# Chanuk-Yang/Deep_Continuous_Fusion_for_Multi-Sensor_3D_Object_Detection

Hardware: AMD Instinct MI355X
Metric: frames/sec (train step) 100k-pt LiDAR + 1242x375 RGB (higher is better)
Workload: dtype bf16; 1 GPU; cfg2: grid 32x704x800, 100000 pts/frame, 1242x375 RGB, ResNet-18 image stream, K=3 fusion x4 sites, eval-mode BN (reference F4), batch 2/GPU; global_batch=2, parallelism=dp1, loss_sampling=compat, conv_chain=False

## Files before the change

### deep_continuous_fusion_for_multi-sensor_3d_object_detection_amd/_hip.py

```python
import ctypes
import os
import subprocess

import numpy as np
import torch

_HERE = os.path.dirname(os.path.abspath(__file__))
LIB_PATH = os.environ.get("DCF_HIP_LIB") or os.path.join(_HERE, "libdcf_hip.so")
CSRC = os.path.join(_HERE, "csrc")

F32, BF16, F16 = 0, 1, 2
VOXEL_COMPAT, VOXEL_ACCUM, VOXEL_COMPAT_ROUNDS, VOXEL_OCCUPANCY = 0, 1, 2, 3
PROJ_COMPAT, PROJ_CORRECT = 0, 1

c_int, c_float, c_i64, c_size_t, c_void_p = ctypes.c_int, ctypes.c_float, ctypes.c_int64, ctypes.c_size_t, ctypes.c_void_p
P = c_void_p

SIGNATURES = {
    "dcf_last_error": (ctypes.c_char_p, []),
    "dcf_version": (c_int, []),
    "dcf_set_option": (c_int, [ctypes.c_char_p, ctypes.c_char_p]),
    "dcf_prof_enable": (c_int, [c_int]),
    "dcf_prof_reset": (c_int, []),
    "dcf_prof_calibrate": (c_int, [P, c_int]),
    "dcf_prof_read": (c_int, [P, P, P, P, c_int]),
    "dcf_prof_read2": (c_int, [P, P, P, P, P, c_int]),
    "dcf_compact_workspace_bytes": (c_size_t, [c_int]),
    "dcf_range_filter": (c_int, [P, c_int, P, P, P, P, P, P]),
    "dcf_voxelize_workspace_bytes": (c_size_t, [c_int, c_int, c_int]),
    "dcf_voxelize": (c_int, [P, c_int, P, P, c_int, c_int, c_int, c_int, P, P, P]),
    "dcf_voxelize_batch": (c_int, [P, P, c_int, P, P, c_int, c_int, c_int, P, P, P]),
    "dcf_voxelize_batch_nhwc": (c_int, [c_int, P, P, c_int, P, P, c_int, c_int, c_int, P, P, P]),
    "dcf_project_filter": (c_int, [P, c_int, P, P, c_float, c_float, c_int, P, P, P, P, P, P]),
    "dcf_project_filter_batch": (c_int, [P, P, c_int, P, P, c_float, c_float, c_int, P, P, c_int, P, P, P]),
    "dcf_knn_workspace_bytes": (c_size_t, [c_int, c_int, c_int]),
    "dcf_knn_bev": (c_int, [P, P, c_int, c_int, c_int, c_int, c_int, c_float, c_float, c_float, c_float, c_float, P, P, P]),
    "dcf_knn_bev_batch": (c_int, [P, P, c_int, c_int, c_int, c_int, c_int, c_int, c_float, c_float, c_float, c_float, c_float, P, P, c_size_t, P]),
    "dcf_knn_bev_sites": (c_int, [P, P, c_int, c_int, c_int, P, c_int, c_float, c_float, c_float, c_float, c_float, P]),
    "dcf_knn_bev_batch_shared": (c_int, [P, P, c_int, c_int, c_int, c_int, c_int, c_int, c_int, c_int, c_int, c_float, c_float, c_float, c_float, c_float, P, P, c_size_t, P, c_size_t, P]),
    "dcf_nchw_to_nhwc": (c_int, [c_int, P, P, c_int, c_int, c_int, c_int, P]),
    "dcf_nhwc_to_nchw": (c_int, [c_int, P, P, c_int, c_int, c_int, c_int, P]),
    "dcf_image_to_nhwc4": (c_int, [c_int, P, P, c_int, c_int, c_int, P]),
    "dcf_conv2d_fwd": (c_int, [c_int, P, P, P, P, P] + [c_int] * 12 + [P]),
    "dcf_conv2d_fwd_rowscale": (c_int, [c_int, P, P, P, P, P, P] + [c_int] * 12 + [P]),
    "dcf_conv2d_dgrad": (c_int, [c_int, P, P, P, P, P] + [c_int] * 11 + [P]),
    "dcf_conv2d_dgrad_halfres": (c_int, [c_int, P, P, P, P, P, P] + [c_int] * 11 + [P]),
    "dcf_conv3x3_chain_supported": (c_int, [c_int] * 6),
    "dcf_conv3x3_chain_workspace_bytes": (c_size_t, [c_int] * 6),
    "dcf_conv3x3_chain": (c_int, [c_int, P, c_int, c_int, c_int, c_int, c_int, c_int, P, P]),
    "dcf_fp8_act_scale": (c_int, [c_float, P]),
    "dcf_cast_fp8": (c_int, [c_int, P, P, P, P, c_i64, P]),
    "dcf_weight_prep_fp8": (c_int, [P, P, c_int, c_int, P, P, P, P, P, c_float, P]),
    "dcf_conv2d_fwd_fp8": (c_int, [c_int, P, P, P, P, P, P, P, P, P, P] + [c_int] * 12 + [P]),
    "dcf_conv2d_wgrad_splits": (c_int, [c_int] * 8),
    "dcf_conv2d_wgrad": (c_int, [c_int, P, P, P, P, c_int] + [c_int] * 11 + [P]),
    "dcf_conv2d_wgrad_groupable": (c_int, [c_int] * 10),
    "dcf_conv2d_wgrad_group": (c_int, [P, c_int, P]),
    "dcf_stem7x7_fwd": (c_int, [c_int, P, P, P, P] + [c_int] * 7 + [P]),
    "dcf_stem7x7_wgrad": (c_int, [c_int, P, P, P, P, c_int] + [c_int] * 6 + [P]),
    "dcf_weight_prep": (c_int, [c_int, P, c_int, P, P, P, P, c_float, P]),
    "dcf_wgrad_finalize": (c_int, [P, c_int, c_int, P, P, P, P, P, P, c_float, P]),
    "dcf_eval_score_filter": (c_int, [P, c_int, c_int, c_int, c_float, c_int, P, P, P]),
    "dcf_eval_nms_workspace_bytes": (c_size_t, [c_int]),
    "dcf_eval_nms": (c_int, [P, P, c_int, c_int, ctypes.c_double, P, P, P, P]),
    "dcf_eval_match": (c_int, [P, c_int, P, c_int, P, c_int, P, P]),
    "dcf_eval_rank_workspace_bytes": (c_size_t, [c_int, c_int, c_int]),
    "dcf_eval_rank_filter": (c_int, [P, c_int, c_int, c_int, c_float, c_int, P, P, P, P, P, P]),
    "dcf_eval_match_ranked_workspace_bytes": (c_size_t, [c_int, c_int]),
    "dcf_eval_match_ranked": (c_int, [P, P, P, c_int, P, c_int, P, c_int, P, P, P]),
    "dcf_eval_accumulate": (c_int, [P, P, P, P, P, c_int, P, c_int, P, P, c_i64, P, P]),
    "dcf_eval_ap_workspace_bytes": (c_size_t, [c_i64]),
    "dcf_eval_ap": (c_int, [P, P, P, c_i64, c_int, P, P, P, P]),
    "dcf_wgrad_finalize_rows": (c_int, [P, c_int, P, P, P, P, P, P, P, c_float, P]),
    "dcf_bn_workspace_bytes": (c_size_t, [c_int]),
    "dcf_bn_train_fwd": (c_int, [c_int, P, P, P, P, P, P, P, P, P, c_i64, c_int, c_float, c_float, c_int, P, P]),
    "dcf_bn_train_bwd": (c_int, [c_int, P, P, P, P, P, P, P, P, c_i64, c_int, P, P]),
    "dcf_relu_bwd_chansum": (c_int, [c_int, P, P, P, c_i64, c_int, c_int, P]),
    "dcf_resize_bilinear_fwd": (c_int, [c_int, P, P, P] + [c_int] * 7 + [P]),
    "dcf_resize_bilinear_bwd": (c_int, [c_int, P, P] + [c_int] * 7 + [P]),
    "dcf_maxpool3x3s2_fwd": (c_int, [c_int, P, P] + [c_int] * 6 + [P]),
    "dcf_maxpool3x3s2_bwd": (c_int, [c_int, P, P, P, P] + [c_int] * 6 + [P]),
    "dcf_maxpool3x3s2_fwd_idx": (c_int, [c_int, P, P, P] + [c_int] * 6 + [P]),
    "dcf_maxpool3x3s2_bwd_idx": (c_int, [c_int, P, P, P] + [c_int] * 6 + [P]),
    "dcf_head_fwd": (c_int, [c_int, P, c_int, P, P, c_int, c_int, c_int, P]),
    "dcf_head_bwd": (c_int, [c_int, P, c_int, P, P, P, P, c_int, c_int, c_int, P]),
    "dcf_point_sample_fwd": (c_int, [c_int, P, c_int, c_int, c_int, P, P, c_int, P, P]),
    "dcf_point_sample_bwd": (c_int, [c_int, P, c_int, c_int, c_int, P, P, c_int, P, P]),
    "dcf_point_sample_fwd_batch": (c_int, [c_int, P, c_int, c_int, c_int, P, c_i64, P, c_int, P, c_int, P]),
    "dcf_point_sample_bwd_batch": (c_int, [c_int, P, c_int, c_int, c_int, P, c_i64, P, c_int, P, c_int, P]),
    "dcf_fusion_gather_fwd_batch": (c_int, [c_int, P, c_i64, P, c_i64, P, c_int, c_int, c_int, c_int, c_float, c_float, c_float, c_float, P, P, c_int, P, P, c_int, P]),
    "dcf_fusion_gather_bwd_inv_batch": (c_int, [c_int, P, c_i64, P, c_i64, P, P, c_i64, P, P, c_int, c_int, c_int, c_int, c_float, c_float, c_float, c_float, P, P, c_int, P, P, P, P, P, c_int, P]),
    "dcf_fusion_gather_fwd": (c_int, [c_int, P, P, P, c_int, c_int, c_int, c_int, c_float, c_float, c_float, c_float, P, P, c_int, P, P, P]),
    "dcf_fusion_gather_bwd": (c_int, [c_int, P, P, P, c_int, c_int, c_int, c_int, c_float, c_float, c_float, c_float, P, P, c_int, P, P, P, P, P]),
    "dcf_fusion_invert_workspace_bytes": (c_size_t, [c_int, c_int]),
    "dcf_fusion_invert": (c_int, [P, c_int, c_int, c_int, P, P, P, P, P]),
    "dcf_fusion_gather_bwd_pts": (c_int, [c_int, P, P, P, c_int, P, P, c_int, c_int, c_int, c_int, c_float, c_float, c_float, c_float, P, P, c_int, P, P, P, P, P]),
    "dcf_fusion_gather_bwd_workspace_bytes": (c_size_t, [c_int]),
    "dcf_fusion_gather_bwd_direct_workspace_bytes": (c_size_t, [c_int, c_int, c_int]),
    "dcf_fusion_gather_bwd_direct_batch": (c_int, [c_int, P, c_i64, P, c_i64, P, P, c_i64, P, P, c_int, c_int, c_int, c_int, c_float, c_float, c_float, c_float, P, P, c_int, P, P, P, P, P, P, c_int, P]),
    "dcf_fusion_gather_bwd_inv": (c_int, [c_int, P, P, P, P, P, P, c_int, c_int, c_int, c_int, c_float, c_float, c_float, c_float, P, P, c_int, P, P, P, P, P, P]),
    "dcf_rowscale_bias_fwd": (c_int, [c_int, P, P, P, c_i64, c_int, P]),
    "dcf_rowscale_bias_bwd": (c_int, [c_int, P, P, P, c_i64, c_int, P]),
    "dcf_relu_mask_rowscale_bwd": (c_int, [c_int, P, P, P, P, P, c_i64, c_int, P]),
    "dcf_cast": (c_int, [c_int, P, c_int, P, c_i64, P]),
    "dcf_loss_fwd_bwd": (c_int, [P, c_i64, P, c_i64, P, P, P, c_int, c_int, c_float, c_int, P, P, c_i64, P, c_i64, P]),
    "dcf_loss_sample_rand": (ctypes.c_uint32, [ctypes.c_uint64, c_int, c_int, c_int, c_int]),
    "dcf_loss_sample_fwd_bwd": (c_int, [P, c_i64, P, c_i64, P, P, P, c_int, c_int, c_int, c_int, c_int, c_float, c_float, c_float, c_float, c_float,
                                        c_int, c_int, c_int, c_int, ctypes.c_uint64, c_float, c_int, P, P, c_i64, P, c_i64, P, P, P, P]),
    "dcf_inv_sort_segments": (c_int, [P, c_int, P, P, P]),
    "dcf_cam_invert_workspace_bytes": (c_size_t, [c_int, c_int, c_int]),
    "dcf_cam_invert": (c_int, [P, c_i64, P, c_int, c_int, c_int, c_int, P, P, P, P, P]),
    "dcf_point_sample_bwd_det": (c_int, [c_int, P, c_i64, c_int, c_int, c_int, P, c_i64, P, P, P, c_int, P]),
    "dcf_fusion_gather_bwd_det_workspace_bytes": (c_size_t, [c_int, c_int, c_int]),
    "dcf_fusion_gather_bwd_det": (c_int, [c_int, P, c_i64, P, c_i64, P, c_int, P, P, c_int, c_int, c_int, c_int, c_float, c_float, c_float, c_float,
                                          P, P, c_int, P, P, P, P, P, c_int, P]),
    "dcf_rowscale_bias_bwd_det_workspace_bytes": (c_size_t, [c_int]),
    "dcf_rowscale_bias_bwd_det": (c_int, [c_int, P, P, P, P, P, c_i64, c_int, P, P]),
    "dcf_rows_fold": (c_int, [P, c_int, c_int, P, P]),
    "dcf_loss_fwd_bwd_det": (c_int, [P, c_i64, P, c_i64, P, P, P, c_int, c_int, c_float, c_int, P, P, c_i64, P, c_i64, P, P]),
    "dcf_loss_sample_fwd_bwd_det": (c_int, [P, c_i64, P, c_i64, P, P, P, c_int, c_int, c_int, c_int, c_int, c_float, c_float, c_float, c_float, c_float,
                                            c_int, c_int, c_int, c_int, ctypes.c_uint64, c_float, c_int, P, P, c_i64, P, c_i64, P, P, P, P, P]),
    "dcf_loss_hard_workspace_bytes": (c_size_t, [c_int, c_int, c_int]),
    "dcf_loss_hard_fwd_bwd": (c_int, [P, c_i64, P, c_i64, P, P, P, c_int, c_int, c_int, c_int, c_int, c_float, c_float, c_float, c_float, c_float,
                                      c_int, c_int, c_int, c_int, ctypes.c_uint64, c_float, c_int, P, P, c_i64, P, c_i64, P, P, P, P, P]),
    "dcf_loss_hard_fwd_bwd_det": (c_int, [P, c_i64, P, c_i64, P, P, P, c_int, c_int, c_int, c_int, c_int, c_float, c_float, c_float, c_float, c_float,
                                          c_int, c_int, c_int, c_int, ctypes.c_uint64, c_float, c_int, P, P, c_i64, P, c_i64, P, P, P, P, P, P]),
    "dcf_adam_step": (c_int, [P, P, P, P, c_i64, c_float, c_float, c_float, c_float, c_int, c_float, P]),
    "dcf_grad_stats": (c_int, [P, c_i64, P, P]),
    "dcf_amp_update": (c_int, [P, c_float, c_int, ctypes.c_double, ctypes.c_double, c_int, c_float, c_float, c_float, c_float, P]),
    "dcf_adam_step_guarded": (c_int, [P, P, P, P, c_i64, c_float, c_float, c_float, P, P]),
}


class ConvParam(ctypes.Structure):
    _fields_ = [("w_off", c_i64), ("gamma_off", c_i64), ("beta_off", c_i64), ("mean_off", c_i64), ("var_off", c_i64),
                ("wfwd_off", c_i64), ("wdgrad_off", c_i64), ("shift_off", c_i64), ("slab_off", c_i64), ("gsum_off", c_i64),
                ("cout", ctypes.c_int32), ("cin", ctypes.c_int32), ("taps", ctypes.c_int32), ("cout_pad", ctypes.c_int32),
                ("nsplit", ctypes.c_int32), ("flags", ctypes.c_int32), ("pad0", ctypes.c_int32), ("pad1", ctypes.c_int32)]


F8_AMAX_STRIDE = 80


class F8Param(ctypes.Structure):
    _fields_ = [("w8_off", c_i64), ("wscale_off", c_i64)]


class WgradItem(ctypes.Structure):
    _fields_ = [("dtype", ctypes.c_int32), ("nsplit", ctypes.c_int32), ("x", c_void_p), ("gy", c_void_p), ("slabs", c_void_p),
                ("gsum", c_void_p), ("B", ctypes.c_int32), ("H", ctypes.c_int32), ("W", ctypes.c_int32), ("Cin", ctypes.c_int32),
                ("Cout", ctypes.c_int32), ("kh", ctypes.c_int32), ("kw", ctypes.c_int32), ("stride", ctypes.c_int32), ("pad", ctypes.c_int32),
                ("pad_", ctypes.c_int32)]


CHAIN_MAX_LAYERS = 24


class ChainLayer(ctypes.Structure):
    _fields_ = [("x", c_void_p), ("w", c_void_p), ("shift", c_void_p), ("res", c_void_p), ("mask", c_void_p), ("y", c_void_p),
                ("relu", ctypes.c_int32), ("pad_", ctypes.c_int32)]


class KnnMap(ctypes.Structure):
    _fields_ = [("idx", c_void_p), ("h", ctypes.c_int32), ("w", ctypes.c_int32)]


class KnnSite(ctypes.Structure):
    _fields_ = [("h", ctypes.c_int32), ("w", ctypes.c_int32), ("stride", ctypes.c_int32), ("fine", ctypes.c_int32), ("idx_out", c_void_p),
                ("ws", c_void_p), ("ws_stride_bytes", ctypes.c_size_t)]


AMP_PARTS = 1024


class AmpState(ctypes.Structure):
    _fields_ = [("scale_in", c_float), ("scale_next", c_float), ("growth_tracker", ctypes.c_int32), ("found_inf", ctypes.c_int32),
                ("applied_steps", c_i64), ("skipped_steps", c_i64), ("grad_norm", c_float), ("clip_coef", c_float),
                ("gscale", c_float), ("lr_over_bc1", c_float), ("inv_sqrt_bc2", c_float), ("pad_", ctypes.c_int32 * 3),
                ("part_sum", c_float * AMP_PARTS), ("part_flag", ctypes.c_int32 * AMP_PARTS)]


class DcfError(RuntimeError):
    pass


_LIB = None


def build(force=False):
    if force:
        subprocess.check_call(["make", "-s", "-C", CSRC, "clean"])
    subprocess.check_call(["make", "-s", "-j8", "-C", CSRC])
    return LIB_PATH


def lib():
    global _LIB
    if _LIB is None:
        if not os.path.exists(LIB_PATH):
            raise DcfError("libdcf_hip.so is not built (%s). Run __graft_entry__.build() / make -C %s; "
                           "there is no CPU fallback for the HIP hot path." % (LIB_PATH, CSRC))
        L = ctypes.CDLL(LIB_PATH)
        for name, (res, args) in SIGNATURES.items():
            fn = getattr(L, name)
            fn.restype = res
            fn.argtypes = args
        _LIB = L
    return _LIB


_Tensor = torch.Tensor
_Param = torch.nn.Parameter


def _ptr(t):
    tt = type(t)
    if tt is int or tt is float or t is None:
        return t
    if tt is _Tensor or tt is _Param:
        return t.data_ptr()
    if isinstance(t, torch.Tensor):
        return t.data_ptr()
    if isinstance(t, np.ndarray):
        return t.ctypes.data
    return t


_raw_stream = getattr(torch._C, "_cuda_getCurrentRawStream", None)
_get_device = torch._C._cuda_getDevice if hasattr(torch._C, "_cuda_getDevice") else None


def stream_ptr():
    if _raw_stream is not None:
        return _raw_stream(_get_device())
    return torch.cuda.current_stream().cuda_stream


_FN = {}
_NO_RAISE = ("dcf_version", "dcf_conv2d_wgrad_splits", "dcf_prof_read", "dcf_conv2d_wgrad_groupable", "dcf_conv3x3_chain_supported")


def call(name, *args):
    ent = _FN.get(name)
    if ent is None:
        fn = getattr(lib(), name)
        ent = _FN[name] = (fn, fn.restype is c_int and name not in _NO_RAISE)
    rc = ent[0](*[_ptr(a) for a in args])
    if rc != 0 and ent[1]:
# ... 50 lines not shown
```

### deep_continuous_fusion_for_multi-sensor_3d_object_detection_amd/csrc/geometry.hip

```cpp
#include <stdlib.h>
#include "dcf_common.h"

namespace {

struct Lim6 { float v[6]; };
struct Aff6 { float v[6]; };
struct Crt12 { float v[12]; };

__device__ __forceinline__ bool in_range(float x, float y, float z, const Lim6 &l)
{
    return x > l.v[0] && x < l.v[1] && y > l.v[2] && y < l.v[3] && z > l.v[4] && z < l.v[5];
}

constexpr int CP_THREADS = 256;
constexpr int CP_ITEMS = 4;
constexpr int CP_TILE = CP_THREADS * CP_ITEMS;

__device__ __forceinline__ int block_excl_scan(int v, int *total)
{
    __shared__ int wsum[4];
    const int lane = threadIdx.x & 63, wid = threadIdx.x >> 6;
    int inc = v;
#pragma unroll
    for (int o = 1; o < 64; o <<= 1) {
// ... 308 lines not shown
        for (int c = 0; c < 8; ++c) contrib[k][c] = 0.f;
    const int cell = (zl * L + xl) * W + yl;
#pragma unroll
    for (int oz = -1; oz <= 1; ++oz)
#pragma unroll
        for (int ox = -1; ox <= 1; ++ox)
#pragma unroll
            for (int oy = -1; oy <= 1; ++oy) {
                const int nc = cell + (oz * L + ox) * W + oy;
                if (nc < 0 || nc >= nvox) continue;
                const int j1 = last[nc];
                if (j1 <= 0) continue;
                const float *q = pts + 3 * (size_t)(j1 - 1);
                const float fx = __fadd_rn(__fmul_rn(q[0], aff.v[0]), aff.v[1]);
                const float fy = __fadd_rn(__fmul_rn(q[1], aff.v[2]), aff.v[3]);
                const float fz = __fadd_rn(__fmul_rn(q[2], aff.v[4]), aff.v[5]);
                const float dx = __fsub_rn(fx, (float)(int)fx), dy = __fsub_rn(fy, (float)(int)fy), dz = __fsub_rn(fz, (float)(int)fz);
                const float wxs[2] = {__fsub_rn(1.0f, dx), dx}, wys[2] = {__fsub_rn(1.0f, dy), dy}, wzs[2] = {__fsub_rn(1.0f, dz), dz};
#pragma unroll
                for (int k = 0; k < 8; ++k) {
                    const int ez = (k & 1) - oz, ex = ((k >> 1) & 1) - ox, ey = ((k >> 2) & 1) - oy;
                    if (ez < 0 || ez > 1 || ex < 0 || ex > 1 || ey < 0 || ey > 1) continue;
                    contrib[k][ez | (ex << 1) | (ey << 2)] = __fmul_rn(__fmul_rn(wxs[ex], wys[ey]), wzs[ez]);
                }
            }
#pragma unroll
    for (int k = 0; k < 8; ++k) {
        float sum = 0.f;
#pragma unroll
        for (int c = 0; c < 8; ++c) sum = __fadd_rn(sum, contrib[k][c]);
        const int v = cell + ((k & 1) * L + ((k >> 1) & 1)) * W + ((k >> 2) & 1);
        if (v >= nvox) continue;
        if (NHWC) {
            const int vz = v / (L * W), r = v - vz * (L * W);
            DT<TO>::st(grid + (size_t)r * Cz + vz, sum);
        } else {
            DT<TO>::st(grid + v, sum);
        }
    }
}

__global__ void __launch_bounds__(256) k_voxel_accum(const float *pts, int n, Lim6 lim, Aff6 aff, int L, int W, float *grid)
{
    const int i = blockIdx.x * blockDim.x + threadIdx.x;
    if (i >= n) return;
    const float x = pts[3 * i], y = pts[3 * i + 1], z = pts[3 * i + 2];
    if (!in_range(x, y, z, lim)) return;
    Corner8 c8;
    corners(x, y, z, aff, L, W, c8);
#pragma unroll
    for (int c = 0; c < 8; ++c) atomicAdd(&grid[c8.vox[c]], c8.w[c]);
}

__global__ void __launch_bounds__(256) k_voxel_occupancy(const float *pts, int n, Lim6 lim, Aff6 aff, int L, int W, float *grid)
{
    const int i = blockIdx.x * blockDim.x + threadIdx.x;
    if (i >= n) return;
    const float x = pts[3 * i], y = pts[3 * i + 1], z = pts[3 * i + 2];
    if (!in_range(x, y, z, lim)) return;
    Corner8 c8;
    corners(x, y, z, aff, L, W, c8);
    grid[c8.vox[0]] = 1.0f;
}

struct KnnGrid {
    int h, w, h8, w8, stride;
    float xs, xo, ys, yo;
    int fs_xyz, fs_cnt, fs_ws, fs_out;
};

__device__ __forceinline__ int cell_key(int ci, int cj, const KnnGrid &g)
{
    return (((ci >> 3) * g.w8 + (cj >> 3)) << 6) + ((ci & 7) << 3) + (cj & 7);
}

__device__ __forceinline__ void point_cell(float x, float y, const KnnGrid &g, int &ci, int &cj)
{
    const float fx = __fadd_rn(__fmul_rn(x, g.xs), g.xo), fy = __fadd_rn(__fmul_rn(y, g.ys), g.yo);
    ci = (int)floorf(fx / (float)g.stride);
    cj = (int)floorf(fy / (float)g.stride);
    ci = min(max(ci, 0), g.h - 1);
    cj = min(max(cj, 0), g.w - 1);
}

__global__ void __launch_bounds__(256) k_knn_hist(const float *xyz, const int *count, int n_max, KnnGrid g, int *cellcnt,
                                                  int *pkey)
{
    const int i = blockIdx.x * blockDim.x + threadIdx.x;
    xyz += (size_t)blockIdx.y * g.fs_xyz; count += blockIdx.y * g.fs_cnt; cellcnt += (size_t)blockIdx.y * g.fs_ws; pkey += (size_t)blockIdx.y * g.fs_ws;
    const int n = min(*count, n_max);
    if (i >= n) return;
    int ci, cj;
    point_cell(xyz[3 * i], xyz[3 * i + 1], g, ci, cj);
    const int key = cell_key(ci, cj, g);
    pkey[i] = key;
    atomicAdd(&cellcnt[key], 1);
}

__global__ void __launch_bounds__(CP_THREADS) k_scan_blocksum(const int *in, int n, int *blocksum, int fstride = 0)
{
    in += (size_t)blockIdx.y * fstride; blocksum += (size_t)blockIdx.y * fstride;
    const int base = blockIdx.x * CP_TILE + threadIdx.x * CP_ITEMS;
    int c = 0;
#pragma unroll
    for (int k = 0; k < CP_ITEMS; ++k)
        if (base + k < n) c += in[base + k];
    int tot;
    block_excl_scan(c, &tot);
    if (threadIdx.x == 0) blocksum[blockIdx.x] = tot;
}

__global__ void __launch_bounds__(CP_THREADS) k_scan_apply(const int *in, int n, const int *blockoff, int *out, int *cursor, int fstride = 0)
{
    in += (size_t)blockIdx.y * fstride; blockoff += (size_t)blockIdx.y * fstride; out += (size_t)blockIdx.y * fstride; cursor += (size_t)blockIdx.y * fstride;
    const int base = blockIdx.x * CP_TILE + threadIdx.x * CP_ITEMS;
    int v[CP_ITEMS];
    int c = 0;
#pragma unroll
    for (int k = 0; k < CP_ITEMS; ++k) {
        v[k] = (base + k < n) ? in[base + k] : 0;
        c += v[k];
    }
    int tot;
    int pos = blockoff[blockIdx.x] + block_excl_scan(c, &tot);
#pragma unroll
    for (int k = 0; k < CP_ITEMS; ++k) {
        if (base + k < n) {
            out[base + k] = pos;
            cursor[base + k] = pos;
            pos += v[k];
        }
    }
}

__global__ void __launch_bounds__(256) k_knn_fill(const float *xyz, const int *count, int n_max, const int *pkey, int *cursor,
                                                  float4 *sorted, int fs_xyz = 0, int fs_cnt = 0, int fs_ws = 0)
{
    xyz += (size_t)blockIdx.y * fs_xyz; count += blockIdx.y * fs_cnt; pkey += (size_t)blockIdx.y * fs_ws; cursor += (size_t)blockIdx.y * fs_ws;
    sorted = reinterpret_cast<float4 *>(reinterpret_cast<int *>(sorted) + (size_t)blockIdx.y * fs_ws);
    const int i = blockIdx.x * blockDim.x + threadIdx.x;
    const int n = min(*count, n_max);
    if (i >= n) return;
    const int pos = atomicAdd(&cursor[pkey[i]], 1);
    sorted[pos] = make_float4(xyz[3 * i], xyz[3 * i + 1], __int_as_float(i), 0.f);
}

#define DCF_MAX_KNN_SITES 4
struct KnnSortSites {
    KnnGrid g[DCF_MAX_KNN_SITES];
    int *ws[DCF_MAX_KNN_SITES];
    int nscan[DCF_MAX_KNN_SITES], nsb[DCF_MAX_KNN_SITES];
    int pkey_off[DCF_MAX_KNN_SITES], sorted_off[DCF_MAX_KNN_SITES];
    int n, B;
};

__global__ void __launch_bounds__(256) k_knn_zero_ms(KnnSortSites S)
{
    const int site = blockIdx.y / S.B, frame = blockIdx.y - site * S.B;
    int *p = S.ws[site] + (size_t)frame * S.g[site].fs_ws;
    const int n = S.nscan[site], n4 = n >> 2;
    int4 *row = reinterpret_cast<int4 *>(p);
    for (int i = blockIdx.x * blockDim.x + threadIdx.x; i < n4; i += gridDim.x * blockDim.x) row[i] = make_int4(0, 0, 0, 0);
    if (blockIdx.x == 0 && threadIdx.x < (n & 3)) p[(n4 << 2) + threadIdx.x] = 0;
}

__global__ void __launch_bounds__(256) k_knn_hist_ms(const float *xyz, const int *count, int n_max, KnnSortSites S)
{
    const int site = blockIdx.y / S.B, frame = blockIdx.y - site * S.B;
    const KnnGrid &g = S.g[site];
    const int i = blockIdx.x * blockDim.x + threadIdx.x;
    xyz += (size_t)frame * g.fs_xyz; count += frame * g.fs_cnt;
    int *cellcnt = S.ws[site] + (size_t)frame * g.fs_ws, *pkey = cellcnt + S.pkey_off[site];
    const int n = min(*count, n_max);
    if (i >= n) return;
    int ci, cj;
    point_cell(xyz[3 * i], xyz[3 * i + 1], g, ci, cj);
    const int key = cell_key(ci, cj, g);
    pkey[i] = key;
    atomicAdd(&cellcnt[key], 1);
}

__global__ void __launch_bounds__(CP_THREADS) k_scan_blocksum_ms(KnnSortSites S)
{
    const int site = blockIdx.y / S.B, frame = blockIdx.y - site * S.B;
    if ((int)blockIdx.x >= S.nsb[site]) return;
    const int n = S.nscan[site];
    const int *in = S.ws[site] + (size_t)frame * S.g[site].fs_ws;
    int *blocksum = const_cast<int *>(in) + 3 * n;
    const int base = blockIdx.x * CP_TILE + threadIdx.x * CP_ITEMS;
    int c = 0;
#pragma unroll
    for (int k = 0; k < CP_ITEMS; ++k)
        if (base + k < n) c += in[base + k];
    int tot;
    block_excl_scan(c, &tot);
    if (threadIdx.x == 0) blocksum[blockIdx.x] = tot;
}

__global__ void __launch_bounds__(CP_THREADS) k_compact_scan_ms(KnnSortSites S)
{
    const int site = blockIdx.y / S.B, frame = blockIdx.y - site * S.B;
    const int nb = S.nsb[site];
    int *blocksum = S.ws[site] + (size_t)frame * S.g[site].fs_ws + 3 * S.nscan[site];
    int carry = 0;
    for (int b0 = 0; b0 < nb; b0 += CP_THREADS) {
        int i = b0 + threadIdx.x;
        int v = i < nb ? blocksum[i] : 0;
        int tot;
        int ex = block_excl_scan(v, &tot);
        if (i < nb) blocksum[i] = carry + ex;
        carry += tot;
    }
    if (threadIdx.x == 0) blocksum[nb] = carry;
}

__global__ void __launch_bounds__(CP_THREADS) k_scan_apply_ms(KnnSortSites S)
{
    const int site = blockIdx.y / S.B, frame = blockIdx.y - site * S.B;
    if ((int)blockIdx.x >= S.nsb[site]) return;
    const int n = S.nscan[site];
    const int *in = S.ws[site] + (size_t)frame * S.g[site].fs_ws;
    int *out = const_cast<int *>(in) + n, *cursor = out + n;
    const int *blockoff = cursor + n;
    const int base = blockIdx.x * CP_TILE + threadIdx.x * CP_ITEMS;
    int v[CP_ITEMS];
    int c = 0;
#pragma unroll
    for (int k = 0; k < CP_ITEMS; ++k) {
        v[k] = (base + k < n) ? in[base + k] : 0;
        c += v[k];
    }
    int tot;
    int pos = blockoff[blockIdx.x] + block_excl_scan(c, &tot);
#pragma unroll
    for (int k = 0; k < CP_ITEMS; ++k) {
        if (base + k < n) {
            out[base + k] = pos;
            cursor[base + k] = pos;
            pos += v[k];
        }
    }
}

__global__ void __launch_bounds__(256) k_knn_fill_ms(const float *xyz, const int *count, int n_max, KnnSortSites S)
{
    const int site = blockIdx.y / S.B, frame = blockIdx.y - site * S.B;
    const KnnGrid &g = S.g[site];
    xyz += (size_t)frame * g.fs_xyz; count += frame * g.fs_cnt;
    int *ws = S.ws[site] + (size_t)frame * g.fs_ws;
    const int *pkey = ws + S.pkey_off[site];
    int *cursor = ws + 2 * S.nscan[site];
    float4 *sorted = reinterpret_cast<float4 *>(ws + S.sorted_off[site]);
    const int i = blockIdx.x * blockDim.x + threadIdx.x;
    const int n = min(*count, n_max);
    if (i >= n) return;
    const int pos = atomicAdd(&cursor[pkey[i]], 1);
    sorted[pos] = make_float4(xyz[3 * i], xyz[3 * i + 1], __int_as_float(i), 0.f);
}

template <int K>
struct TopK {
    float d[K];
    int id[K];
    __device__ __forceinline__ void clear()
    {
#pragma unroll
        for (int q = 0; q < K; ++q) { d[q] = 3.0e38f; id[q] = 0x7fffffff; }
    }
    __device__ __forceinline__ float kth() const { return d[K - 1]; }
    __device__ __forceinline__ bool full() const { return id[K - 1] != 0x7fffffff; }
    __device__ __forceinline__ int count() const
    {
        int c = 0;
#pragma unroll
        for (int q = 0; q < K; ++q) c += id[q] != 0x7fffffff;
        return c;
    }
    static __device__ __forceinline__ unsigned long long key(float dd, int ii)
    {
        return ((unsigned long long)__float_as_uint(dd) << 32) | (unsigned)ii;
    }
    __device__ __forceinline__ void insert(float dd, int ii)
    {
        unsigned long long x = key(dd, ii);
#pragma unroll
        for (int q = 0; q < K; ++q) {
            const unsigned long long kq = key(d[q], id[q]);
            const bool lt = x < kq;
            const unsigned long long lo = lt ? x : kq;
            x = lt ? kq : x;
            d[q] = __uint_as_float((unsigned)(lo >> 32));
            id[q] = (int)(unsigned)lo;
        }
    }
    __device__ __forceinline__ void insert_unique(unsigned long long x)
    {
#pragma unroll
        for (int q = 0; q < K; ++q) {
            const unsigned long long kq = key(d[q], id[q]);
            if (x == kq) x = ~0ull;
            const bool lt = x < kq;
            const unsigned long long lo = lt ? x : kq;
            x = lt ? kq : x;
            d[q] = __uint_as_float((unsigned)(lo >> 32));
            id[q] = (int)(unsigned)lo;
        }
    }
};

#ifdef KNN_STAMP
#define KNN_STAMP_TILES 4096
__device__ long long g_knn_stamps[KNN_STAMP_TILES][16];
#define KNN_ST(k, v) do { if (blockIdx.y == 0 && tile < KNN_STAMP_TILES && lane == 0 && wv == 0) g_knn_stamps[tile][k] = (v); } while (0)
#define KNN_CNT(var, n) (var) += (n)
#define KNN_T(k) KNN_ST(k, __builtin_amdgcn_s_memtime() - st_t0)
#else
#define KNN_ST(k, v) do { } while (0)
#define KNN_CNT(var, n) do { } while (0)
#define KNN_T(k) do { } while (0)
#endif

constexpr int KNN_MERGE_POINTS = 256;
template <int K, int NW>
__device__ __forceinline__ void knn_search_tile(const int *count, int n_max, const KnnGrid &g, const int *cellstart,
                                                const float4 *sorted, float rmax2, int *out, const int tile, const int wv)
{
    count += blockIdx.y * g.fs_cnt; cellstart += (size_t)blockIdx.y * g.fs_ws; out += (size_t)blockIdx.y * g.fs_out;
    sorted = reinterpret_cast<const float4 *>(reinterpret_cast<const int *>(sorted) + (size_t)blockIdx.y * g.fs_ws);
    const int lane = threadIdx.x & 63;
    const int TI = tile / g.w8, TJ = tile - TI * g.w8;
    const int i = TI * 8 + (lane >> 3), j = TJ * 8 + (lane & 7);
    const bool inside = (i < g.h) && (j < g.w);
    __shared__ unsigned long long s_keys[NW][K][64];
    const float s = (float)g.stride;
    const float X = __fdiv_rn(__fsub_rn(__fmul_rn((float)i + 0.5f, s), g.xo), g.xs);
    const float Y = __fdiv_rn(__fsub_rn(__fmul_rn((float)j + 0.5f, s), g.yo), g.ys);
    const float cwx = s / g.xs, cwy = s / g.ys;
    const float cwmin = fminf(cwx, cwy);
    const int n = min(*count, n_max);

    TopK<K> top;
    top.clear();
    bool done = !inside;
#ifdef KNN_STAMP
    long long st_pts = 0, st_rings = 0, st_blocks = 0;
    const long long st_t0 = __builtin_amdgcn_s_memtime();
#endif

    const float d2lim = rmax2 >= 0.0f ? rmax2 : __int_as_float(0x7f800000);
    const float4 nopoint = make_float4(__int_as_float(0x7fc00000), __int_as_float(0x7fc00000), 0.f, 0.f);
    auto offer = [&](const float4 &mine, int n, bool take) {
        const float lim = take ? d2lim : -1.0f;
        for (int u0 = wv; u0 < n; u0 += 4 * NW) {
#pragma unroll
            for (int v = 0; v < 4; ++v) {
                const int u = u0 + NW * v;
                const float qx = __int_as_float(__builtin_amdgcn_readlane(__float_as_int(mine.x), u));
                const float qy = __int_as_float(__builtin_amdgcn_readlane(__float_as_int(mine.y), u));
                const int qi = __builtin_amdgcn_readlane(__float_as_int(mine.z), u);
                const float dx = __fsub_rn(qx, X), dy = __fsub_rn(qy, Y);
                const float d2 = __fadd_rn(__fmul_rn(dx, dx), __fmul_rn(dy, dy));
                top.insert(d2 <= lim ? d2 : __int_as_float(0x7f800000), qi);
            }
        }
    };
    auto merge = [&]() {
        if constexpr (NW > 1) {
#pragma unroll
            for (int q = 0; q < K; ++q) s_keys[wv][q][lane] = TopK<K>::key(top.d[q], top.id[q]);
            __syncthreads();
#pragma unroll
            for (int o = 1; o < NW; ++o) {
#pragma unroll
                for (int q = 0; q < K; ++q) top.insert_unique(s_keys[(wv + o) % NW][q][lane]);
            }
            __syncthreads();
        }
    };
    auto scan_range = [&](int b, int e, bool take) {
        KNN_CNT(st_pts, e - b);
        for (int p0 = b; p0 < e; p0 += 64) {
            const int n = min(64, e - p0);
            const float4 mine = lane < n ? sorted[p0 + lane] : nopoint;
            offer(mine, n, take);
        }
    };

    KNN_T(8);
    if (n > 0) {
        const int H8 = g.h8 * 8, W8 = g.w8 * 8;
        {
            const int row = lane / 3, seg = lane - row * 3;
            const int ci = TI * 8 - 2 + row;
            int c0 = TJ * 8 + (seg == 0 ? -2 : (seg == 1 ? 0 : 8));
            int c1 = TJ * 8 + (seg == 0 ? -1 : (seg == 1 ? 7 : 9));
            c0 = max(c0, 0); c1 = min(c1, W8 - 1);
            int ps = 0, pe = 0;
            if (lane < 36 && ci >= 0 && ci <= H8 - 1 && c0 <= c1) {
                ps = cellstart[cell_key(ci, c0, g)];
                pe = cellstart[cell_key(ci, c1, g) + 1];
            }
            const int len = pe - ps;
            int inc = len;
#ifdef KNN_STAMP
            if (__any(len > 1 << 30)) return;
            KNN_T(9);
#endif
#pragma unroll
            for (int o = 1; o < 64; o <<= 1) {
                const int v = __shfl_up(inc, o, 64);
                if (lane >= o) inc += v;
            }
            const int total = __builtin_amdgcn_readlane(inc, 63);
            const int exc = inc - len;
            KNN_ST(2, (long long)total);
            for (int base = 0; base < total; base += 64) {
                const int t = base + lane;
                int lo = 0, hi = 63;
#pragma unroll
                for (int it = 0; it < 6; ++it) {
                    const int mid = (lo + hi) >> 1;
                    const bool right = __shfl(inc, mid, 64) <= t;
                    lo = right ? mid + 1 : lo;
                    hi = right ? hi : mid;
                }
                const int src = __shfl(ps, lo, 64) + (t - __shfl(exc, lo, 64));
                const int n = min(64, total - base);
                const float4 mine = lane < n ? sorted[src] : nopoint;
#ifdef KNN_STAMP
                if (base == 0) {
                    KNN_T(10);
                    if (__any(mine.z == 123456.f)) return;
                    KNN_T(11);
                }
#endif
                offer(mine, n, !done);
            }
        }
        merge();
        {
            const float bound = 2.5f * cwmin - 1e-3f;
            if (!done && top.full() && top.kth() < bound * bound) done = true;
            if (rmax2 >= 0.0f && bound > 0.f && bound * bound > rmax2) done = true;
        }
        KNN_ST(0, __builtin_amdgcn_s_memtime() - st_t0);
#ifdef KNN_STAMP
        { const long long left = __popcll(__ballot(!done)); KNN_ST(6, left); }
#endif
        if (!__all(done)) {
            if (!done) top.clear();
            const int Rmax = max(g.h8, g.w8);
            for (int R = 0; R <= Rmax; ++R) {
                const int nblk = R == 0 ? 1 : 8 * R;
                for (int t0 = 0; t0 < nblk; t0 += 64) {
                    const int t = t0 + lane;
                    int a = 0, b = 0;
                    if (R > 0) {
                        if (t < 2 * R + 1) { a = -R; b = -R + t; }
                        else if (t < 4 * R + 2) { a = R; b = -R + (t - (2 * R + 1)); }
                        else if (t < 6 * R + 1) { b = -R; a = -R + 1 + (t - (4 * R + 2)); }
                        else { b = R; a = -R + 1 + (t - (6 * R + 1)); }
                    }
                    const int bi = TI + a, bj = TJ + b;
                    int ps = 0, pe = 0;
                    if (t < nblk && bi >= 0 && bi < g.h8 && bj >= 0 && bj < g.w8) {
                        const int k0 = (bi * g.w8 + bj) << 6;
                        ps = cellstart[k0];
                        pe = cellstart[k0 + 64];
                    }
                    unsigned long long live = __ballot(pe > ps);
                    while (live) {
                        const int l = __ffsll((long long)live) - 1;
                        live &= live - 1;
                        const int cbi = __builtin_amdgcn_readlane(bi, l), cbj = __builtin_amdgcn_readlane(bj, l);
                        const int cps = __builtin_amdgcn_readlane(ps, l), cpe = __builtin_amdgcn_readlane(pe, l);
                        bool visit = !done;
                        if (visit && top.full()) {
                            const float lox = ((float)(cbi * 8) * s - g.xo) / g.xs, hix = ((float)(cbi * 8 + 8) * s - g.xo) / g.xs;
                            const float loy = ((float)(cbj * 8) * s - g.yo) / g.ys, hiy = ((float)(cbj * 8 + 8) * s - g.yo) / g.ys;
                            const float ddx = fmaxf(0.f, fmaxf(lox - X, X - hix) - 1e-3f);
                            const float ddy = fmaxf(0.f, fmaxf(loy - Y, Y - hiy) - 1e-3f);
                            visit = (ddx * ddx + ddy * ddy) <= top.kth();
                        }
                        if (__any(visit)) { KNN_CNT(st_blocks, 1); scan_range(cps, cpe, visit); }
                        if (cpe - cps > KNN_MERGE_POINTS) merge();
                    }
                }
                merge();
                KNN_CNT(st_rings, 1);
                const float bound = (8.0f * (float)R + 0.5f) * cwmin - 1e-3f;
                if (!done && top.full() && top.kth() < bound * bound) done = true;
                if (rmax2 >= 0.0f && bound > 0.f && bound * bound > rmax2) done = true;
                if (__all(done)) break;
            }
        }
    }
#ifdef KNN_STAMP
    KNN_ST(1, __builtin_amdgcn_s_memtime() - st_t0);
    KNN_ST(3, st_pts); KNN_ST(4, st_rings); KNN_ST(5, st_blocks);
#endif
    if (inside) {
        const int hw = g.h * g.w, pix = i * g.w + j;
#pragma unroll
        for (int q = 0; q < K; ++q) out[q * hw + pix] = top.id[q] != 0x7fffffff ? top.id[q] : -1;
    }
}

template <int K, int NW>
__global__ void __launch_bounds__(64 * NW) k_knn_search(const int *count, int n_max, KnnGrid g, const int *cellstart,
                                                       const float4 *sorted, float rmax2, int *out)
{
    knn_search_tile<K, NW>(count, n_max, g, cellstart, sorted, rmax2, out, blockIdx.x, __builtin_amdgcn_readfirstlane(threadIdx.x >> 6));
}

template <int K>
__device__ __forceinline__ void wave_merge(const TopK<K> &mine, float (&gd)[K], int (&gi)[K], int &gcnt)
{
    TopK<K> t = mine;
    gcnt = 0;
#pragma unroll
    for (int q = 0; q < K; ++q) {
        float d = t.d[0];
        int id = t.id[0];
#pragma unroll
        for (int o = 1; o < 64; o <<= 1) {
            const float od = __shfl_xor(d, o, 64);
            const int oi = __shfl_xor(id, o, 64);
            if (od < d || (od == d && oi < id)) { d = od; id = oi; }
        }
        gd[q] = d; gi[q] = id;
        if (id != 0x7fffffff) ++gcnt;
        if (t.id[0] == id && id != 0x7fffffff) {
#pragma unroll
            for (int k = 0; k + 1 < K; ++k) { t.d[k] = t.d[k + 1]; t.id[k] = t.id[k + 1]; }
            t.d[K - 1] = 3.0e38f; t.id[K - 1] = 0x7fffffff;
        }
    }
}

template <int K>
__device__ __forceinline__ void knn_search_wave(const int *count, int n_max, const KnnGrid &g, const int *cellstart,
                                                const float4 *sorted, float rmax2, int *out, const int bx)
{
    count += blockIdx.y * g.fs_cnt; cellstart += (size_t)blockIdx.y * g.fs_ws; out += (size_t)blockIdx.y * g.fs_out;
    sorted = reinterpret_cast<const float4 *>(reinterpret_cast<const int *>(sorted) + (size_t)blockIdx.y * g.fs_ws);
    const int lane = threadIdx.x & 63;
    const int pix = __builtin_amdgcn_readfirstlane(bx * 4 + (threadIdx.x >> 6));
    const int hw = g.h * g.w;
    if (pix >= hw) return;
    const int i = pix / g.w, j = pix - i * g.w;
    const float s = (float)g.stride;
    const float X = __fdiv_rn(__fsub_rn(__fmul_rn((float)i + 0.5f, s), g.xo), g.xs);
    const float Y = __fdiv_rn(__fsub_rn(__fmul_rn((float)j + 0.5f, s), g.yo), g.ys);
    const float cwmin = fminf(s / g.xs, s / g.ys);
    const int n = min(*count, n_max);

    TopK<K> top;
    top.clear();
    float gd[K];
    int gi[K];
    int gcnt = 0;
#pragma unroll
    for (int q = 0; q < K; ++q) { gd[q] = 3.0e38f; gi[q] = 0x7fffffff; }

    auto scan_range = [&](int b, int e) {
        for (int p = b + lane; p < e; p += 64) {
            const float4 q = sorted[p];
            const float dx = __fsub_rn(q.x, X), dy = __fsub_rn(q.y, Y);
            const float d2 = __fadd_rn(__fmul_rn(dx, dx), __fmul_rn(dy, dy));
            if (!(rmax2 >= 0.0f && d2 > rmax2)) top.insert(d2, __float_as_int(q.z));
        }
    };

    bool done = (n == 0);
    if (!done) {
        const int H8 = g.h8 * 8, W8 = g.w8 * 8;
        {
            const int row = lane >> 1, part = lane & 1;
            const int ci = i - 2 + row;
            const int cbeg = max(j - 2, 0), cend = min(j + 2, W8 - 1);
            const int split = min(cend, (cbeg | 7));
            const int c0 = part == 0 ? cbeg : split + 1;
            const int c1 = part == 0 ? split : cend;
            int ps = 0, pe = 0;
            if (lane < 10 && ci >= 0 && ci <= H8 - 1 && c0 <= c1) {
                ps = cellstart[cell_key(ci, c0, g)];
                pe = cellstart[cell_key(ci, c1, g) + 1];
            }
            unsigned long long live = __ballot(pe > ps);
            while (live) {
                const int l = __ffsll((long long)live) - 1;
                live &= live - 1;
                scan_range(__builtin_amdgcn_readlane(ps, l), __builtin_amdgcn_readlane(pe, l));
            }
        }
        wave_merge<K>(top, gd, gi, gcnt);
        const float bound = 2.5f * cwmin - 1e-3f;
        if (gcnt >= K && gd[K - 1] < bound * bound) done = true;
        if (rmax2 >= 0.0f && bound > 0.f && bound * bound > rmax2) done = true;
    }
    if (!done) {
        top.clear();
        gcnt = 0;
#pragma unroll
        for (int q = 0; q < K; ++q) { gd[q] = 3.0e38f; gi[q] = 0x7fffffff; }
        const int I = i >> 3, J = j >> 3;
        const int Rmax = max(g.h8, g.w8);
        for (int R = 0; R <= Rmax && !done; ++R) {
            const int nblk = R == 0 ? 1 : 8 * R;
            for (int t0 = 0; t0 < nblk; t0 += 64) {
                const int t = t0 + lane;
                int a = 0, b = 0;
                if (R > 0) {
                    if (t < 2 * R + 1) { a = -R; b = -R + t; }
                    else if (t < 4 * R + 2) { a = R; b = -R + (t - (2 * R + 1)); }
                    else if (t < 6 * R + 1) { b = -R; a = -R + 1 + (t - (4 * R + 2)); }
                    else { b = R; a = -R + 1 + (t - (6 * R + 1)); }
                }
                const int bi = I + a, bj = J + b;
                int ps = 0, pe = 0;
                if (t < nblk && bi >= 0 && bi < g.h8 && bj >= 0 && bj < g.w8) {
                    const int k0 = (bi * g.w8 + bj) << 6;
                    ps = cellstart[k0];
                    pe = cellstart[k0 + 64];
                }
                unsigned long long live = __ballot(pe > ps);
                while (live) {
                    const int l = __ffsll((long long)live) - 1;
                    live &= live - 1;
                    const int cbi = __builtin_amdgcn_readlane(bi, l), cbj = __builtin_amdgcn_readlane(bj, l);
                    const int cps = __builtin_amdgcn_readlane(ps, l), cpe = __builtin_amdgcn_readlane(pe, l);
                    bool visit = true;
                    if (gcnt >= K) {
                        const float lox = ((float)(cbi * 8) * s - g.xo) / g.xs, hix = ((float)(cbi * 8 + 8) * s - g.xo) / g.xs;
                        const float loy = ((float)(cbj * 8) * s - g.yo) / g.ys, hiy = ((float)(cbj * 8 + 8) * s - g.yo) / g.ys;
                        const float ddx = fmaxf(0.f, fmaxf(lox - X, X - hix) - 1e-3f);
                        const float ddy = fmaxf(0.f, fmaxf(loy - Y, Y - hiy) - 1e-3f);
                        visit = (ddx * ddx + ddy * ddy) <= gd[K - 1];
                    }
                    if (visit) scan_range(cps, cpe);
                }
            }
            wave_merge<K>(top, gd, gi, gcnt);
            const float bound = (8.0f * (float)R + 0.5f) * cwmin - 1e-3f;
            if (gcnt >= K && gd[K - 1] < bound * bound) done = true;
            if (rmax2 >= 0.0f && bound > 0.f && bound * bound > rmax2) done = true;
        }
    }
    if (lane == 0) {
#pragma unroll
        for (int q = 0; q < K; ++q) out[q * hw + pix] = (q < gcnt) ? gi[q] : -1;
    }
}

template <int K>
__global__ void __launch_bounds__(256) k_knn_search_wave(const int *count, int n_max, KnnGrid g, const int *cellstart,
                                                         const float4 *sorted, float rmax2, int *out)
{
    knn_search_wave<K>(count, n_max, g, cellstart, sorted, rmax2, out, blockIdx.x);
}

constexpr int KNN_FINE_MIN_POINTS = 192;

__device__ __forceinline__ float open_edge_distance(const KnnGrid &gf, float X, float Y, int i0, int i1, int j0, int j1)
{
    const float s = (float)gf.stride;
    float b = 3.0e38f;
    if (i0 > 0) b = fminf(b, X - ((float)i0 * s - gf.xo) / gf.xs);
    if (i1 < gf.h - 1) b = fminf(b, ((float)(i1 + 1) * s - gf.xo) / gf.xs - X);
    if (j0 > 0) b = fminf(b, Y - ((float)j0 * s - gf.yo) / gf.ys);
    if (j1 < gf.w - 1) b = fminf(b, ((float)(j1 + 1) * s - gf.yo) / gf.ys - Y);
    return b - 1e-3f;
}

template <int K>
__device__ __forceinline__ void knn_search_fine(const int *count, int n_max, const KnnGrid &g, const KnnGrid &gf, const int *cellstart_c,
                                                const float4 *sorted_c, const int *cellstart, const float4 *sorted, float rmax2,
                                                int *out, int dense_min, const int bx)
{
    count += blockIdx.y * g.fs_cnt; out += (size_t)blockIdx.y * g.fs_out;
    cellstart_c += (size_t)blockIdx.y * g.fs_ws;
    sorted_c = reinterpret_cast<const float4 *>(reinterpret_cast<const int *>(sorted_c) + (size_t)blockIdx.y * g.fs_ws);
    cellstart += (size_t)blockIdx.y * gf.fs_ws;
    sorted = reinterpret_cast<const float4 *>(reinterpret_cast<const int *>(sorted) + (size_t)blockIdx.y * gf.fs_ws);
    const int lane = threadIdx.x & 63;
    const int pix = __builtin_amdgcn_readfirstlane(bx * 4 + (threadIdx.x >> 6));
    const int hw = g.h * g.w;
    if (pix >= hw) return;
    const int i = pix / g.w, j = pix - i * g.w;
    const float s = (float)g.stride;
    const float X = __fdiv_rn(__fsub_rn(__fmul_rn((float)i + 0.5f, s), g.xo), g.xs);
    const float Y = __fdiv_rn(__fsub_rn(__fmul_rn((float)j + 0.5f, s), g.yo), g.ys);
    const int n = min(*count, n_max);
    int ci, cj;
    point_cell(X, Y, gf, ci, cj);

    TopK<K> top;
    top.clear();
    float gd[K];
    int gi[K];
    int gcnt = 0;
#pragma unroll
    for (int q = 0; q < K; ++q) { gd[q] = 3.0e38f; gi[q] = 0x7fffffff; }
    auto scan_own = [&](int b, int e) {
        for (int p = b; p < e; ++p) {
            const float4 q = sorted[p];
            const float dx = __fsub_rn(q.x, X), dy = __fsub_rn(q.y, Y);
            const float d2 = __fadd_rn(__fmul_rn(dx, dx), __fmul_rn(dy, dy));
            if (!(rmax2 >= 0.0f && d2 > rmax2)) top.insert(d2, __float_as_int(q.z));
        }
    };
    auto scan_range = [&](int b, int e) {
        for (int p = b + lane; p < e; p += 64) {
            const float4 q = sorted_c[p];
            const float dx = __fsub_rn(q.x, X), dy = __fsub_rn(q.y, Y);
            const float d2 = __fadd_rn(__fmul_rn(dx, dx), __fmul_rn(dy, dy));
            if (!(rmax2 >= 0.0f && d2 > rmax2)) top.insert(d2, __float_as_int(q.z));
        }
    };
    bool done = (n == 0);
    bool dense = false;
    if (!done) {
        const int H8 = g.h8 * 8, W8 = g.w8 * 8;
        const int row = lane >> 1, part = lane & 1;
        const int wi = i - 2 + row;
        const int cbeg = max(j - 2, 0), cend = min(j + 2, W8 - 1);
        const int split = min(cend, (cbeg | 7));
        const int c0 = part == 0 ? cbeg : split + 1;
        const int c1 = part == 0 ? split : cend;
        int ps = 0, pe = 0;
        if (lane < 10 && wi >= 0 && wi <= H8 - 1 && c0 <= c1) {
            ps = cellstart_c[cell_key(wi, c0, g)];
            pe = cellstart_c[cell_key(wi, c1, g) + 1];
        }
        const int total = wave_sum_i(pe - ps);
        dense = total > dense_min;
        if (!dense) {
            unsigned long long live = __ballot(pe > ps);
            while (live) {
                const int l = __ffsll((long long)live) - 1;
                live &= live - 1;
                scan_range(__builtin_amdgcn_readlane(ps, l), __builtin_amdgcn_readlane(pe, l));
            }
            wave_merge<K>(top, gd, gi, gcnt);
            const float cw = fminf(s / g.xs, s / g.ys);
            const float bound = 2.5f * cw - 1e-3f;
            if (gcnt >= K && gd[K - 1] < bound * bound) done = true;
            if (rmax2 >= 0.0f && bound > 0.f && bound * bound > rmax2) done = true;
        }
    }
    int rprev = -1;
    for (int r = 2; r <= 8 && !done && dense; r += 2) {
        const int side = 2 * r + 1, ncell = side * side;
        for (int t0 = 0; t0 < ncell; t0 += 64) {
            const int t = t0 + lane;
            const int a = t / side - r, b = t - (t / side) * side - r;
            const int fi = ci + a, fj = cj + b;
            if (t < ncell && max(abs(a), abs(b)) > rprev && fi >= 0 && fi < gf.h && fj >= 0 && fj < gf.w) {
                const int key = cell_key(fi, fj, gf);
                scan_own(cellstart[key], cellstart[key + 1]);
            }
        }
        rprev = r;
        wave_merge<K>(top, gd, gi, gcnt);
        const float bound = open_edge_distance(gf, X, Y, ci - r, ci + r, cj - r, cj + r);
        if (gcnt >= K && bound > 0.f && gd[K - 1] < bound * bound) done = true;
        if (rmax2 >= 0.0f && bound > 0.f && bound * bound > rmax2) done = true;
    }
    if (!done) {
        top.clear();
        gcnt = 0;
#pragma unroll
        for (int q = 0; q < K; ++q) { gd[q] = 3.0e38f; gi[q] = 0x7fffffff; }
        const float cwmin = fminf(s / g.xs, s / g.ys);
        const int I = i >> 3, J = j >> 3;
        const int Rmax = max(g.h8, g.w8);
        for (int R = 0; R <= Rmax && !done; ++R) {
            const int nblk = R == 0 ? 1 : 8 * R;
            for (int t0 = 0; t0 < nblk; t0 += 64) {
                const int t = t0 + lane;
                int a = 0, b = 0;
                if (R > 0) {
                    if (t < 2 * R + 1) { a = -R; b = -R + t; }
                    else if (t < 4 * R + 2) { a = R; b = -R + (t - (2 * R + 1)); }
                    else if (t < 6 * R + 1) { b = -R; a = -R + 1 + (t - (4 * R + 2)); }
                    else { b = R; a = -R + 1 + (t - (6 * R + 1)); }
                }
                const int bi = I + a, bj = J + b;
                int ps = 0, pe = 0;
                if (t < nblk && bi >= 0 && bi < g.h8 && bj >= 0 && bj < g.w8) {
                    const int k0 = (bi * g.w8 + bj) << 6;
                    ps = cellstart_c[k0];
                    pe = cellstart_c[k0 + 64];
                }
                unsigned long long live = __ballot(pe > ps);
                while (live) {
                    const int l = __ffsll((long long)live) - 1;
                    live &= live - 1;
                    const int cbi = __builtin_amdgcn_readlane(bi, l), cbj = __builtin_amdgcn_readlane(bj, l);
                    const int cps = __builtin_amdgcn_readlane(ps, l), cpe = __builtin_amdgcn_readlane(pe, l);
                    bool visit = true;
                    if (gcnt >= K) {
                        const float lox = ((float)(cbi * 8) * s - g.xo) / g.xs, hix = ((float)(cbi * 8 + 8) * s - g.xo) / g.xs;
                        const float loy = ((float)(cbj * 8) * s - g.yo) / g.ys, hiy = ((float)(cbj * 8 + 8) * s - g.yo) / g.ys;
                        const float ddx = fmaxf(0.f, fmaxf(lox - X, X - hix) - 1e-3f);
                        const float ddy = fmaxf(0.f, fmaxf(loy - Y, Y - hiy) - 1e-3f);
                        visit = (ddx * ddx + ddy * ddy) <= gd[K - 1];
                    }
                    if (visit) scan_range(cps, cpe);
                }
            }
            wave_merge<K>(top, gd, gi, gcnt);
            const float bound = (8.0f * (float)R + 0.5f) * cwmin - 1e-3f;
            if (gcnt >= K && gd[K - 1] < bound * bound) done = true;
            if (rmax2 >= 0.0f && bound > 0.f && bound * bound > rmax2) done = true;
        }
    }
    if (lane == 0) {
#pragma unroll
        for (int q = 0; q < K; ++q) out[q * hw + pix] = (q < gcnt) ? gi[q] : -1;
    }
}

template <int K>
__global__ void __launch_bounds__(256) k_knn_search_fine(const int *count, int n_max, KnnGrid g, KnnGrid gf, const int *cellstart_c,
                                                         const float4 *sorted_c, const int *cellstart, const float4 *sorted, float rmax2,
                                                         int *out, int dense_min)
{
    knn_search_fine<K>(count, n_max, g, gf, cellstart_c, sorted_c, cellstart, sorted, rmax2, out, dense_min, blockIdx.x);
}

struct KnnSearchSites {
    KnnGrid g[DCF_MAX_KNN_SITES], gf[DCF_MAX_KNN_SITES];
    const int *cellstart[DCF_MAX_KNN_SITES], *cellstart_f[DCF_MAX_KNN_SITES];
    const float4 *sorted[DCF_MAX_KNN_SITES], *sorted_f[DCF_MAX_KNN_SITES];
    int *out[DCF_MAX_KNN_SITES];
    int kind[DCF_MAX_KNN_SITES];
    int first[DCF_MAX_KNN_SITES + 1];
    int n, dense_min;
};

template <int K>
__global__ void __launch_bounds__(256) k_knn_search_ms(const int *count, int n_max, KnnSearchSites S, float rmax2)
{
    int i = 0;
#pragma unroll
    for (int k = 1; k < DCF_MAX_KNN_SITES; ++k) i += (k < S.n && (int)blockIdx.x >= S.first[k]);
    const int lb = (int)blockIdx.x - S.first[i];
    const int wave = __builtin_amdgcn_readfirstlane(threadIdx.x >> 6);
    const KnnGrid &g = S.g[i];
    const int kind = S.kind[i];
    if (kind == 0) {
        const int tile = lb * 4 + wave;
        if (tile >= g.h8 * g.w8) return;
        knn_search_tile<K, 1>(count, n_max, g, S.cellstart[i], S.sorted[i], rmax2, S.out[i], tile, 0);
    } else if (kind == 1) {
        knn_search_tile<K, 4>(count, n_max, g, S.cellstart[i], S.sorted[i], rmax2, S.out[i], lb, wave);
    } else if (kind == 2) {
        knn_search_wave<K>(count, n_max, g, S.cellstart[i], S.sorted[i], rmax2, S.out[i], lb);
    } else {
        knn_search_fine<K>(count, n_max, g, S.gf[i], S.cellstart[i], S.sorted[i], S.cellstart_f[i], S.sorted_f[i], rmax2, S.out[i], S.dense_min, lb);
    }
}

struct InvMaps {
    const int *idx[DCF_MAX_KNN_MAPS];
    int first[DCF_MAX_KNN_MAPS + 1];
    int hw[DCF_MAX_KNN_MAPS], w[DCF_MAX_KNN_MAPS];
    int n;
};

__device__ __forceinline__ int inv_map_of(const InvMaps &m, int e)
{
    int g = 0;
#pragma unroll
    for (int i = 1; i < DCF_MAX_KNN_MAPS; ++i) g += (i < m.n && e >= m.first[i]);
    return g;
}

struct InvRun { int head, len; };
__device__ __forceinline__ InvRun inv_run(int key, int lane)
{
    const int prev = __shfl_up(key, 1, 64);
    const unsigned long long heads = __ballot(lane == 0 || key != prev);
    const unsigned long long below = heads & ((2ull << lane) - 1ull);
    InvRun r;
    r.head = 63 - __clzll(below);
    const unsigned long long above = lane == 63 ? 0ull : (heads >> (lane + 1));
    r.len = (above ? lane + 1 + (__ffsll((long long)above) - 1) : 64) - r.head;
    return r;
}

__global__ void __launch_bounds__(256) k_zero_rows(int *p, int n, int64_t stride)
{
    int4 *row = reinterpret_cast<int4 *>(p + blockIdx.y * stride);
    const int n4 = n >> 2;
    for (int i = blockIdx.x * blockDim.x + threadIdx.x; i < n4; i += gridDim.x * blockDim.x) row[i] = make_int4(0, 0, 0, 0);
    if (blockIdx.x == 0 && threadIdx.x < (n & 3)) p[blockIdx.y * stride + (n4 << 2) + threadIdx.x] = 0;
}

__device__ __forceinline__ int inv_load(const InvMaps &m, int e, int &g)
{
    const int e0 = blockIdx.x * blockDim.x;
    const int gA = __builtin_amdgcn_readfirstlane(inv_map_of(m, e0));
    const int gB = __builtin_amdgcn_readfirstlane(inv_map_of(m, min(e0 + (int)blockDim.x, m.first[m.n]) - 1));
    if (gA == gB) {
        g = gA;
        return m.idx[gA][e - m.first[gA]];
    }
    g = inv_map_of(m, e);
    return m.idx[g][e - m.first[g]];
}

__global__ void __launch_bounds__(256) k_inv_hist(InvMaps m, int n_max, int *cnt)
{
    const int e = blockIdx.x * blockDim.x + threadIdx.x;
    const int lane = threadIdx.x & 63;
    int key = -1;
    if (e < m.first[m.n]) {
        int g;
        const int id = inv_load(m, e, g);
        if (id >= 0 && id < n_max) key = g * (n_max + 1) + id;
    }
    const InvRun r = inv_run(key, lane);
    if (key >= 0 && r.head == lane) atomicAdd(&cnt[key], r.len);
}

__global__ void __launch_bounds__(256) k_inv_fill(InvMaps m, int n_max, int *cursor, int *ent_pix, int *ent_pt)
{
    const int e = blockIdx.x * blockDim.x + threadIdx.x;
    const int lane = threadIdx.x & 63;
    int key = -1, g = 0, id = 0;
    if (e < m.first[m.n]) {
        id = inv_load(m, e, g);
        if (id >= 0 && id < n_max) key = g * (n_max + 1) + id;
    }
    const InvRun r = inv_run(key, lane);
    int base = 0;
    if (key >= 0 && r.head == lane) base = atomicAdd(&cursor[key], r.len);
    base = __shfl(base, r.head, 64);
    if (key < 0) return;
    const int pos = base + (lane - r.head);
    const int p = (e - m.first[g]) % m.hw[g];
    ent_pix[pos] = ((p / m.w[g]) << 16) | (p % m.w[g]);
    ent_pt[pos] = id;
}

}

extern "C" size_t dcf_compact_workspace_bytes(int n) { return sizeof(int) * (size_t)(cdiv(n > 0 ? n : 1, CP_TILE) + 8); }

extern "C" int dcf_range_filter(const float *pts, int n, const float *lim, float *out_pts, int32_t *out_src,
                                int32_t *count_dev, void *ws, dcf_stream_t stream)
{
    DCF_REQUIRE(n >= 0 && lim && count_dev && ws, "dcf_range_filter: bad arguments");
    hipStream_t s = S(stream);
    if (n == 0) { DCF_HIP(hipMemsetAsync(count_dev, 0, sizeof(int), s)); return DCF_OK; }
    RangePred p;
    memcpy(p.lim.v, lim, sizeof(p.lim.v));
    int nb = cdiv(n, CP_TILE);
    int *bs = (int *)ws;
    DCF_LAUNCH_B("compact_count", (double)n * 12.0, s, hipLaunchKernelGGL(k_compact_count<RangePred>, dim3(nb), dim3(CP_THREADS), 0, s, pts, n, p, bs));
    DCF_LAUNCH("compact_scan", s, hipLaunchKernelGGL(k_compact_scan, dim3(1), dim3(CP_THREADS), 0, s, bs, nb, count_dev));
    DCF_LAUNCH_B("compact_scatter", (double)n * (12.0 + 16.0), s, hipLaunchKernelGGL((k_compact_scatter<RangePred, false>), dim3(nb), dim3(CP_THREADS), 0, s, pts, n, p, bs,
                                                         (float *)nullptr, out_pts, out_src));
    return DCF_OK;
}

extern "C" int dcf_project_filter(const float *pts, int n, const float *lim, const float *crt, float ulim, float vlim,
                                  int mode, float *uv_out, float *xyz_out, int32_t *src_out, int32_t *count_dev,
                                  void *ws, dcf_stream_t stream)
{
    DCF_REQUIRE(n >= 0 && lim && crt && count_dev && ws && uv_out && xyz_out, "dcf_project_filter: bad arguments");
    hipStream_t s = S(stream);
    if (n == 0) { DCF_HIP(hipMemsetAsync(count_dev, 0, sizeof(int), s)); return DCF_OK; }
    ProjPred p;
    memcpy(p.lim.v, lim, sizeof(p.lim.v));
    memcpy(p.c.v, crt, sizeof(p.c.v));
    p.ulim = ulim; p.vlim = vlim; p.mode = mode;
    int nb = cdiv(n, CP_TILE);
    int *bs = (int *)ws;
    DCF_LAUNCH_B("project_count", (double)n * 12.0, s, hipLaunchKernelGGL(k_compact_count<ProjPred>, dim3(nb), dim3(CP_THREADS), 0, s, pts, n, p, bs));
    DCF_LAUNCH("compact_scan", s, hipLaunchKernelGGL(k_compact_scan, dim3(1), dim3(CP_THREADS), 0, s, bs, nb, count_dev));
    DCF_LAUNCH_B("project_scatter", (double)n * (12.0 + 20.0), s, hipLaunchKernelGGL((k_compact_scatter<ProjPred, true>), dim3(nb), dim3(CP_THREADS), 0, s, pts, n, p, bs,
                                                         uv_out, xyz_out, src_out));
    return DCF_OK;
}

extern "C" int dcf_project_filter_batch(const float *const *pts, const int *n, int B, const float *lim, const float *crt, float ulim, float vlim,
                                        int mode, float *uv_out, float *xyz_out, int rows, int32_t *count_dev, void *ws, dcf_stream_t stream)
{
    const char *who = "dcf_project_filter_batch";
    DCF_REQUIRE(pts && n && lim && crt && count_dev && ws && uv_out && xyz_out, "%s: bad arguments", who);
    DCF_REQUIRE(B >= 1 && B <= DCF_PROJ_BATCH_MAX, "%s: 1..%d frames per call", who, DCF_PROJ_BATCH_MAX);
    hipStream_t s = S(stream);
    ProjBatch pb;
    int nmax = 0;
    for (int b = 0; b < DCF_PROJ_BATCH_MAX; ++b) {
        pb.pts[b] = b < B ? pts[b] : nullptr;
        pb.n[b] = b < B ? n[b] : 0;
        DCF_REQUIRE(b >= B || (n[b] >= 0 && n[b] <= rows && (n[b] == 0 || pts[b])), "%s: frame %d: bad point count / null points", who, b);
        memcpy(pb.c[b].v, crt + 12 * (b < B ? b : 0), sizeof(pb.c[b].v));
        if (b < B && n[b] > nmax) nmax = n[b];
    }
    if (nmax == 0) { DCF_HIP(hipMemsetAsync(count_dev, 0, sizeof(int) * B, s)); return DCF_OK; }
    Lim6 l;
    memcpy(l.v, lim, sizeof(l.v));
    const int nb = cdiv(nmax, CP_TILE);
    const int bstride = (int)(dcf_compact_workspace_bytes(nmax) / sizeof(int));
    int *bs = (int *)ws;
    DCF_LAUNCH_B("project_count", (double)nmax * B * 12.0, s, hipLaunchKernelGGL(k_proj_count_b, dim3(nb, B), dim3(CP_THREADS), 0, s, pb, l, ulim, vlim, mode, bs, bstride));
    DCF_LAUNCH("compact_scan", s, hipLaunchKernelGGL(k_proj_scan_b, dim3(1, B), dim3(CP_THREADS), 0, s, bs, nb, bstride, count_dev));
    DCF_LAUNCH_B("project_scatter", (double)nmax * B * (12.0 + 20.0), s, hipLaunchKernelGGL(k_proj_scatter_b, dim3(nb, B), dim3(CP_THREADS), 0, s, pb, l, ulim, vlim, mode, bs, bstride,
                                                                                    uv_out, xyz_out, rows));
    return DCF_OK;
}

extern "C" size_t dcf_voxelize_workspace_bytes(int Cz, int L, int W) { return sizeof(int) * 2 * (size_t)Cz * L * W; }


extern "C" int dcf_voxelize(const float *pts, int n, const float *lim, const float *aff, int Cz, int L, int W,
                            int mode, float *grid, void *owner_ws, dcf_stream_t stream)
{
    DCF_REQUIRE(n >= 0 && lim && aff && grid && Cz > 0 && L > 0 && W > 0, "dcf_voxelize: bad arguments");
    DCF_REQUIRE((int64_t)Cz * L * W < (1ll << 31), "dcf_voxelize: grid too large for int32 voxel ids");
    hipStream_t s = S(stream);
    const int nvox = Cz * L * W;
    DCF_HIP(hipMemsetAsync(grid, 0, sizeof(float) * (size_t)nvox, s));
    if (n == 0) return DCF_OK;
    Lim6 l; Aff6 a;
    memcpy(l.v, lim, sizeof(l.v));
    memcpy(a.v, aff, sizeof(a.v));
    const int nb = cdiv(n, 256);
    if (mode == DCF_VOXEL_COMPAT) {
        DCF_REQUIRE(owner_ws != nullptr, "dcf_voxelize: compat mode needs the zeroed owner workspace");
        VoxBatch vb;
        for (int b = 0; b < DCF_MAX_VOXEL_BATCH; ++b) { vb.pts[b] = b == 0 ? pts : nullptr; vb.n[b] = b == 0 ? n : 0; }
        const dim3 g1(nb, 1);
        DCF_LAUNCH("voxel_cell_claim", s, hipLaunchKernelGGL(k_voxel_cell_claim, g1, dim3(256), 0, s, vb, l, a, L, W, nvox, (int *)owner_ws, 0));
        DCF_LAUNCH("voxel_cell_gather", s, hipLaunchKernelGGL((k_voxel_cell_gather<float, false>), g1, dim3(256), 0, s, vb, l, a, Cz, L, W, nvox, grid, (const int *)owner_ws));
        DCF_LAUNCH("voxel_cell_claim", s, hipLaunchKernelGGL(k_voxel_cell_claim, g1, dim3(256), 0, s, vb, l, a, L, W, nvox, (int *)owner_ws, 1));
    } else if (mode == DCF_VOXEL_COMPAT_ROUNDS) {
        DCF_REQUIRE(owner_ws != nullptr, "dcf_voxelize: compat mode needs the zeroed owner workspace");
        for (int r = 0; r <= 8; ++r)
            DCF_LAUNCH("voxel_compat_round", s, hipLaunchKernelGGL(k_voxel_compat_round, dim3(nb), dim3(256), 0, s, pts, n, l, a, L, W, nvox, r,
                                                                   grid, (int *)owner_ws));
    } else if (mode == DCF_VOXEL_ACCUM) {
        DCF_LAUNCH("voxel_accum", s, hipLaunchKernelGGL(k_voxel_accum, dim3(nb), dim3(256), 0, s, pts, n, l, a, L, W, grid));
    } else if (mode == DCF_VOXEL_OCCUPANCY) {
        DCF_LAUNCH("voxel_occupancy", s, hipLaunchKernelGGL(k_voxel_occupancy, dim3(nb), dim3(256), 0, s, pts, n, l, a, L, W, grid));
    } else {
        dcf_set_error("dcf_voxelize: unknown mode %d", mode);
        return DCF_EINVAL;
    }
    return DCF_OK;
}

static int voxelize_batch_impl(const char *who, int dtype, bool nhwc, const float *const *pts, const int *n, int B, const float *lim, const float *aff,
                               int Cz, int L, int W, void *grids, void *owner_ws, hipStream_t s)
{
    DCF_REQUIRE(pts && n && lim && aff && grids && owner_ws && Cz > 0 && L > 0 && W > 0, "%s: bad arguments", who);
    DCF_REQUIRE(B >= 1 && B <= DCF_MAX_VOXEL_BATCH, "%s: 1..%d frames per call", who, DCF_MAX_VOXEL_BATCH);
    DCF_REQUIRE((int64_t)Cz * L * W < (1ll << 31), "%s: grid too large for int32 voxel ids", who);
    const int nvox = Cz * L * W;
    const size_t es = dtype == DCF_F32 ? 4 : 2;
    DCF_HIP(hipMemsetAsync(grids, 0, es * (size_t)nvox * B, s));
    VoxBatch vb;
    int nmax = 0;
    for (int b = 0; b < DCF_MAX_VOXEL_BATCH; ++b) {
        vb.pts[b] = b < B ? pts[b] : nullptr;
        vb.n[b] = b < B ? n[b] : 0;
        DCF_REQUIRE(b >= B || (n[b] >= 0 && (n[b] == 0 || pts[b])), "%s: frame %d: null points", who, b);
        if (b < B && n[b] > nmax) nmax = n[b];
    }
    if (nmax == 0) return DCF_OK;
    Lim6 l; Aff6 a;
    memcpy(l.v, lim, sizeof(l.v));
    memcpy(a.v, aff, sizeof(a.v));
    const dim3 grid(cdiv(nmax, 256), B);
    DCF_LAUNCH_B("voxel_cell_claim", (double)nmax * B * 16.0, s, hipLaunchKernelGGL(k_voxel_cell_claim, grid, dim3(256), 0, s, vb, l, a, L, W, nvox, (int *)owner_ws, 0));
    if (!nhwc) {
        DCF_LAUNCH_B("voxel_cell_gather", (double)nmax * B * (12.0 + 27 * 4.0 + 8 * 4.0), s, hipLaunchKernelGGL((k_voxel_cell_gather<float, false>), grid, dim3(256), 0, s, vb, l, a, Cz, L, W, nvox, (float *)grids, (const int *)owner_ws));
    } else {
        DCF_DISPATCH_DTYPE(dtype, { DCF_LAUNCH_B("voxel_cell_gather", (double)nmax * B * (12.0 + 27 * 4.0 + 8.0 * sizeof(T)), s, hipLaunchKernelGGL((k_voxel_cell_gather<T, true>), grid, dim3(256), 0, s, vb, l, a, Cz, L, W, nvox, (T *)grids, (const int *)owner_ws)); })
    }
    DCF_LAUNCH_B("voxel_cell_claim", (double)nmax * B * 16.0, s, hipLaunchKernelGGL(k_voxel_cell_claim, grid, dim3(256), 0, s, vb, l, a, L, W, nvox, (int *)owner_ws, 1));
    return DCF_OK;
}

extern "C" int dcf_voxelize_batch(const float *const *pts, const int *n, int B, const float *lim, const float *aff, int Cz, int L, int W,
                                  float *grids, void *owner_ws, dcf_stream_t stream)
{
    return voxelize_batch_impl("dcf_voxelize_batch", DCF_F32, false, pts, n, B, lim, aff, Cz, L, W, grids, owner_ws, S(stream));
}

extern "C" int dcf_voxelize_batch_nhwc(int dtype, const float *const *pts, const int *n, int B, const float *lim, const float *aff, int Cz, int L,
                                       int W, void *x_nhwc, void *owner_ws, dcf_stream_t stream)
{
    DCF_REQUIRE(dtype == DCF_F32 || dtype == DCF_BF16 || dtype == DCF_F16, "dcf_voxelize_batch_nhwc: unsupported dtype %d", dtype);
    return voxelize_batch_impl("dcf_voxelize_batch_nhwc", dtype, true, pts, n, B, lim, aff, Cz, L, W, x_nhwc, owner_ws, S(stream));
}

static inline void knn_dims(int h, int w, int &h8, int &w8, int &ncell) { h8 = (h + 7) / 8; w8 = (w + 7) / 8; ncell = h8 * w8 * 64; }

extern "C" size_t dcf_knn_workspace_bytes(int n_max, int h, int w)
{
    int h8, w8, ncell;
    knn_dims(h, w, h8, w8, ncell);
    size_t ints = 3 * (size_t)(ncell + 1) + (size_t)cdiv(ncell + 1, CP_TILE) + 8 + (size_t)n_max;
    ints = (ints + 3) & ~(size_t)3;
    return ints * sizeof(int) + sizeof(float4) * (size_t)n_max + 64;
}

struct KnnFine {
    int h, w, stride;
    const void *ws;
    size_t ws_stride_bytes;
};

struct KnnSearchPlan {
    KnnGrid g, gf;
    const int *cellstart, *cellstart_f;
    const float4 *sorted, *sorted_f;
    int kind;
    int tile_waves, dense_min;
};

static KnnSearchPlan knn_search_plan(const KnnGrid &g, int B, int n_max, int K, const int *cellstart, const float4 *sorted, const KnnFine *fine, bool merged)
{
    KnnSearchPlan pl;
    pl.g = g; pl.gf = g; pl.cellstart = cellstart; pl.sorted = sorted; pl.cellstart_f = nullptr; pl.sorted_f = nullptr;
    pl.tile_waves = 1; pl.dense_min = KNN_FINE_MIN_POINTS;
    static DcfOpt force_o("KNN_KERNEL"); const char *force = force_o.str();
    const bool per_wave = force && force[0] == 'w' ? true : (force && force[0] == 't' ? false : (g.h * g.w <= 20000));
    static DcfOpt tw_o("KNN_TILE_WAVES"); const char *tw = tw_o.str();
    pl.tile_waves = tw && (tw[0] == '1' || tw[0] == '2' || tw[0] == '4') ? tw[0] - '0' : (!merged && g.h8 * g.w8 * B <= 1500 ? 4 : 1);
    if (fine) {
        KnnGrid gf = g;
        gf.h = fine->h; gf.w = fine->w; gf.stride = fine->stride;
        int ncf;
        knn_dims(fine->h, fine->w, gf.h8, gf.w8, ncf);
        gf.fs_ws = B > 1 ? (int)(fine->ws_stride_bytes / 4) : 0;
        const int nscf = ncf + 1, nsbf = cdiv(nscf, CP_TILE);
        size_t intsf = 3 * (size_t)nscf + (size_t)nsbf + 8 + (size_t)n_max;
        intsf = (intsf + 3) & ~(size_t)3;
        static DcfOpt dm_o("KNN_FINE_MIN"); const char *dm = dm_o.str();
        pl.gf = gf;
        pl.cellstart_f = (const int *)fine->ws + nscf;
        pl.sorted_f = (const float4 *)((const char *)fine->ws + intsf * sizeof(int));
        pl.dense_min = dm ? atoi(dm) : KNN_FINE_MIN_POINTS;
        pl.kind = 3;
    } else if (per_wave) pl.kind = 2;
    else pl.kind = pl.tile_waves == 4 ? 1 : 0;
    (void)K;
    return pl;
}

static int knn_bev_impl(const char *who, const float *xyz, const int32_t *count_dev, int B, int n_max, int K, int h, int w, int stride,
                        float xs, float xo, float ys, float yo, float rmax2, int32_t *idx_out, void *ws, size_t ws_stride_bytes, hipStream_t s,
                        const KnnFine *fine = nullptr, bool presorted = false, KnnSearchPlan *defer = nullptr)
{
    DCF_REQUIRE(xyz && count_dev && idx_out && ws, "%s: null pointer", who);
    DCF_REQUIRE(K >= 1 && K <= 8, "%s: K must be 1..8 (got %d)", who, K);
    DCF_REQUIRE(h > 0 && w > 0 && stride > 0 && n_max >= 0 && B >= 1 && B <= 65535, "%s: bad dims", who);
    DCF_REQUIRE(B == 1 || (ws_stride_bytes % 16 == 0 && ws_stride_bytes >= dcf_knn_workspace_bytes(n_max, h, w) && ws_stride_bytes / 4 < (1ull << 31)),
                "%s: workspace stride must be a multiple of 16 bytes and hold one frame's workspace", who);
    KnnGrid g;
    g.h = h; g.w = w; g.stride = stride; g.xs = xs; g.xo = xo; g.ys = ys; g.yo = yo;
    g.fs_xyz = B > 1 ? n_max * 3 : 0; g.fs_cnt = B > 1 ? 1 : 0; g.fs_ws = B > 1 ? (int)(ws_stride_bytes / 4) : 0; g.fs_out = B > 1 ? K * h * w : 0;
    int ncell;
    knn_dims(h, w, g.h8, g.w8, ncell);
    const int nscan = ncell + 1;
    const int nsb = cdiv(nscan, CP_TILE);
    int *cellcnt = (int *)ws;
    int *cellstart = cellcnt + nscan;
    int *cursor = cellstart + nscan;
    int *blocksum = cursor + nscan;
    int *pkey = blocksum + nsb + 8;
    size_t ints = 3 * (size_t)nscan + (size_t)nsb + 8 + (size_t)n_max;
    ints = (ints + 3) & ~(size_t)3;
    float4 *sorted = (float4 *)((char *)ws + ints * sizeof(int));
    const double fB = (double)B;
    if (!presorted) {
        if (B == 1) DCF_HIP(hipMemsetAsync(cellcnt, 0, sizeof(int) * (size_t)nscan, s));
        else if ((ws_stride_bytes & 15) == 0 && ((uintptr_t)cellcnt & 15) == 0)
            DCF_LAUNCH_B("knn_zero", (double)B * nscan * 4.0, s, hipLaunchKernelGGL(k_zero_rows, dim3(std::min(cdiv(nscan, 1024), 256), B), dim3(256), 0, s, cellcnt, nscan, (int64_t)(ws_stride_bytes / 4)));
        else DCF_HIP(hipMemset2DAsync(cellcnt, ws_stride_bytes, 0, sizeof(int) * (size_t)nscan, B, s));
        if (n_max > 0) {
            const int nb = cdiv(n_max, 256);
            DCF_LAUNCH_B("knn_hist", fB * n_max * 16.0, s, hipLaunchKernelGGL(k_knn_hist, dim3(nb, B), dim3(256), 0, s, xyz, count_dev, n_max, g, cellcnt, pkey));
        }
        int *total = blocksum + nsb;
        DCF_LAUNCH("scan_blocksum", s, hipLaunchKernelGGL(k_scan_blocksum, dim3(nsb, B), dim3(CP_THREADS), 0, s, cellcnt, nscan, blocksum, g.fs_ws));
        DCF_LAUNCH("compact_scan", s, hipLaunchKernelGGL(k_compact_scan, dim3(1, B), dim3(CP_THREADS), 0, s, blocksum, nsb, total, g.fs_ws));
        DCF_LAUNCH("scan_apply", s, hipLaunchKernelGGL(k_scan_apply, dim3(nsb, B), dim3(CP_THREADS), 0, s, cellcnt, nscan, blocksum, cellstart, cursor, g.fs_ws));
        if (n_max > 0) {
            const int nb = cdiv(n_max, 256);
            DCF_LAUNCH_B("knn_fill", fB * n_max * (12.0 + 4.0 + 16.0), s, hipLaunchKernelGGL(k_knn_fill, dim3(nb, B), dim3(256), 0, s, xyz, count_dev, n_max, pkey, cursor, sorted, g.fs_xyz, g.fs_cnt, g.fs_ws));
        }
    }
    const KnnSearchPlan pl = knn_search_plan(g, B, n_max, K, cellstart, sorted, fine, defer != nullptr);
    if (defer) { *defer = pl; return DCF_OK; }
    const int nbp = g.h8 * g.w8;
    const int nbw = cdiv(h * w, 4);
    if (pl.kind == 3) {
#define KNN_FCASE(KK)                                                                                                                       \
    case KK:                                                                                                                                \
        DCF_LAUNCH_B("knn_search_fine", fB * ((double)h * w * K * 4.0 + (double)n_max * 16.0), s,                                           \
                     hipLaunchKernelGGL(k_knn_search_fine<KK>, dim3(nbw, B), dim3(256), 0, s, count_dev, n_max, g, pl.gf, cellstart, sorted,   \
                                        pl.cellstart_f, pl.sorted_f, rmax2, idx_out, pl.dense_min));                                        \
        break;
        switch (K) {
            KNN_FCASE(1) KNN_FCASE(2) KNN_FCASE(3) KNN_FCASE(4) KNN_FCASE(5) KNN_FCASE(6) KNN_FCASE(7) KNN_FCASE(8)
        }
#undef KNN_FCASE
        return DCF_OK;
    }
#define KNN_CASE(KK)                                                                                                     \
    case KK:                                                                                                             \
        if (pl.kind == 2)                                                                                                \
            DCF_LAUNCH_B("knn_search_wave", fB * ((double)h * w * K * 4.0 + (double)n_max * 16.0), s, hipLaunchKernelGGL(k_knn_search_wave<KK>, dim3(nbw, B), dim3(256), 0, s, count_dev, n_max, g, \
                                                                cellstart, sorted, rmax2, idx_out));                     \
        else if (pl.tile_waves == 4)                                                                                     \
            DCF_LAUNCH_B("knn_search", fB * ((double)h * w * K * 4.0 + (double)n_max * 16.0), s, hipLaunchKernelGGL((k_knn_search<KK, 4>), dim3(nbp, B), dim3(256), 0, s, count_dev, n_max, g, \
                                                           cellstart, sorted, rmax2, idx_out));                          \
        else if (pl.tile_waves == 2)                                                                                     \
            DCF_LAUNCH_B("knn_search", fB * ((double)h * w * K * 4.0 + (double)n_max * 16.0), s, hipLaunchKernelGGL((k_knn_search<KK, 2>), dim3(nbp, B), dim3(128), 0, s, count_dev, n_max, g, \
                                                           cellstart, sorted, rmax2, idx_out));                          \
        else                                                                                                             \
            DCF_LAUNCH_B("knn_search", fB * ((double)h * w * K * 4.0 + (double)n_max * 16.0), s, hipLaunchKernelGGL((k_knn_search<KK, 1>), dim3(nbp, B), dim3(64), 0, s, count_dev, n_max, g, \
                                                           cellstart, sorted, rmax2, idx_out));                          \
        break;
    switch (K) {
        KNN_CASE(1) KNN_CASE(2) KNN_CASE(3) KNN_CASE(4) KNN_CASE(5) KNN_CASE(6) KNN_CASE(7) KNN_CASE(8)
    }
#undef KNN_CASE
    return DCF_OK;
}

extern "C" int dcf_knn_bev(const float *xyz, const int32_t *count_dev, int n_max, int K, int h, int w, int stride,
                           float xs, float xo, float ys, float yo, float rmax2, int32_t *idx_out, void *ws,
                           dcf_stream_t stream)
{
    return knn_bev_impl("dcf_knn_bev", xyz, count_dev, 1, n_max, K, h, w, stride, xs, xo, ys, yo, rmax2, idx_out, ws, 0, S(stream));
}

extern "C" int dcf_knn_bev_batch(const float *xyz, const int32_t *count_dev, int B, int n_max, int K, int h, int w, int stride,
                                 float xs, float xo, float ys, float yo, float rmax2, int32_t *idx_out, void *ws, size_t ws_stride_bytes,
                                 dcf_stream_t stream)
{
    return knn_bev_impl("dcf_knn_bev_batch", xyz, count_dev, B, n_max, K, h, w, stride, xs, xo, ys, yo, rmax2, idx_out, ws, ws_stride_bytes, S(stream));
}

extern "C" int dcf_knn_bev_batch_shared(const float *xyz, const int32_t *count_dev, int B, int n_max, int K, int h, int w, int stride,
                                        int fine_h, int fine_w, int fine_stride, float xs, float xo, float ys, float yo, float rmax2,
                                        int32_t *idx_out, void *ws, size_t ws_stride_bytes, const void *ws_fine, size_t ws_fine_stride_bytes,
                                        dcf_stream_t stream)
{
    const char *who = "dcf_knn_bev_batch_shared";
    DCF_REQUIRE(ws_fine && fine_h > 0 && fine_w > 0 && fine_stride > 0, "%s: bad fine-site arguments", who);
    DCF_REQUIRE(stride % fine_stride == 0 && h * stride <= fine_h * fine_stride && w * stride <= fine_w * fine_stride,
                "%s: the coarse site must lie on the fine site's grid", who);
    DCF_REQUIRE(B == 1 || (ws_fine_stride_bytes % 16 == 0 && ws_fine_stride_bytes >= dcf_knn_workspace_bytes(n_max, fine_h, fine_w) &&
                           ws_fine_stride_bytes / 4 < (1ull << 31)), "%s: fine workspace stride must be that of the fine site's call", who);
    const KnnFine fine = {fine_h, fine_w, fine_stride, ws_fine, ws_fine_stride_bytes};
    return knn_bev_impl(who, xyz, count_dev, B, n_max, K, h, w, stride, xs, xo, ys, yo, rmax2, idx_out, ws, ws_stride_bytes, S(stream), &fine);
}

extern "C" int dcf_knn_bev_sites(const float *xyz, const int32_t *count_dev, int B, int n_max, int K, const dcf_knn_site *sites, int nsites,
                                 float xs, float xo, float ys, float yo, float rmax2, dcf_stream_t stream)
{
    const char *who = "dcf_knn_bev_sites";
    DCF_REQUIRE(xyz && count_dev && sites && nsites >= 1 && nsites <= DCF_MAX_KNN_SITES, "%s: 1..%d sites", who, DCF_MAX_KNN_SITES);
    DCF_REQUIRE(K >= 1 && K <= 8 && n_max >= 0 && B >= 1 && B * nsites <= 65535, "%s: bad dims", who);
    hipStream_t s = S(stream);
    KnnSortSites ss;
    ss.n = nsites; ss.B = B;
    int max_nsb = 1, max_nscan = 1;
    for (int i = 0; i < DCF_MAX_KNN_SITES; ++i) {
        const dcf_knn_site &t = sites[i < nsites ? i : 0];
        DCF_REQUIRE(t.idx_out && t.ws && t.h > 0 && t.w > 0 && t.stride > 0, "%s: site %d: bad arguments", who, i);
        DCF_REQUIRE(((uintptr_t)t.ws & 15) == 0 && t.ws_stride_bytes % 16 == 0 && t.ws_stride_bytes >= dcf_knn_workspace_bytes(n_max, t.h, t.w) &&
                    t.ws_stride_bytes / 4 < (1ull << 31), "%s: site %d: workspace must be 16-byte aligned, its stride a multiple of 16 bytes that holds one frame's workspace", who, i);
        DCF_REQUIRE(t.fine < i && t.fine >= -1, "%s: site %d: `fine` must name an earlier site of the call (or -1)", who, i);
        KnnGrid &g = ss.g[i];
        g.h = t.h; g.w = t.w; g.stride = t.stride; g.xs = xs; g.xo = xo; g.ys = ys; g.yo = yo;
        g.fs_xyz = B > 1 ? n_max * 3 : 0; g.fs_cnt = B > 1 ? 1 : 0; g.fs_ws = B > 1 ? (int)(t.ws_stride_bytes / 4) : 0; g.fs_out = B > 1 ? K * t.h * t.w : 0;
        int ncell;
        knn_dims(t.h, t.w, g.h8, g.w8, ncell);
        ss.ws[i] = (int *)t.ws;
        ss.nscan[i] = ncell + 1;
        ss.nsb[i] = cdiv(ncell + 1, CP_TILE);
        ss.pkey_off[i] = 3 * ss.nscan[i] + ss.nsb[i] + 8;
        size_t ints = 3 * (size_t)ss.nscan[i] + (size_t)ss.nsb[i] + 8 + (size_t)n_max;
        ints = (ints + 3) & ~(size_t)3;
        ss.sorted_off[i] = (int)ints;
        if (i < nsites) { max_nsb = std::max(max_nsb, ss.nsb[i]); max_nscan = std::max(max_nscan, ss.nscan[i]); }
    }
    const int gy = nsites * B;
    DCF_LAUNCH_B("knn_zero", (double)B * max_nscan * 4.0, s, hipLaunchKernelGGL(k_knn_zero_ms, dim3(std::min(cdiv(max_nscan, 1024), 256), gy), dim3(256), 0, s, ss));
    if (n_max > 0)
        DCF_LAUNCH_B("knn_hist", (double)gy * n_max * 16.0, s, hipLaunchKernelGGL(k_knn_hist_ms, dim3(cdiv(n_max, 256), gy), dim3(256), 0, s, xyz, count_dev, n_max, ss));
    DCF_LAUNCH("scan_blocksum", s, hipLaunchKernelGGL(k_scan_blocksum_ms, dim3(max_nsb, gy), dim3(CP_THREADS), 0, s, ss));
    DCF_LAUNCH("compact_scan", s, hipLaunchKernelGGL(k_compact_scan_ms, dim3(1, gy), dim3(CP_THREADS), 0, s, ss));
    DCF_LAUNCH("scan_apply", s, hipLaunchKernelGGL(k_scan_apply_ms, dim3(max_nsb, gy), dim3(CP_THREADS), 0, s, ss));
    if (n_max > 0)
        DCF_LAUNCH_B("knn_fill", (double)gy * n_max * (12.0 + 4.0 + 16.0), s, hipLaunchKernelGGL(k_knn_fill_ms, dim3(cdiv(n_max, 256), gy), dim3(256), 0, s, xyz, count_dev, n_max, ss));
    static DcfOpt ms_o("KNN_MERGED_SEARCH"); const char *ms = ms_o.str();
    const bool merged = !(ms && ms[0] == '0');
    KnnSearchSites S;
    S.n = nsites; S.dense_min = KNN_FINE_MIN_POINTS;
    int blocks = 0;
    double bytes = 0.0;
    for (int i = 0; i < nsites; ++i) {
        const dcf_knn_site &t = sites[i];
        KnnFine fine;
        if (t.fine >= 0) {
            const dcf_knn_site &f = sites[t.fine];
            DCF_REQUIRE(t.stride % f.stride == 0 && t.h * t.stride <= f.h * f.stride && t.w * t.stride <= f.w * f.stride,
                        "%s: site %d must lie on the grid of its fine site", who, i);
            fine = {f.h, f.w, f.stride, f.ws, f.ws_stride_bytes};
        }
        KnnSearchPlan pl;
        int rc = knn_bev_impl(who, xyz, count_dev, B, n_max, K, t.h, t.w, t.stride, xs, xo, ys, yo, rmax2, t.idx_out, t.ws, t.ws_stride_bytes, s,
                              t.fine >= 0 ? &fine : nullptr, true, merged ? &pl : nullptr);
        if (rc) return rc;
        if (!merged) continue;
        S.g[i] = pl.g; S.gf[i] = pl.gf; S.cellstart[i] = pl.cellstart; S.sorted[i] = pl.sorted; S.cellstart_f[i] = pl.cellstart_f;
        S.sorted_f[i] = pl.sorted_f; S.out[i] = t.idx_out; S.kind[i] = pl.kind; S.dense_min = pl.dense_min;
        S.first[i] = blocks;
        const int tiles = pl.g.h8 * pl.g.w8;
        blocks += pl.kind == 0 ? cdiv(tiles, 4) : (pl.kind == 1 ? tiles : cdiv(t.h * t.w, 4));
        bytes += (double)B * ((double)t.h * t.w * K * 4.0 + (double)n_max * 16.0);
    }
    if (!merged) return DCF_OK;
    for (int i = nsites; i < DCF_MAX_KNN_SITES; ++i) {
        S.g[i] = S.g[0]; S.gf[i] = S.gf[0]; S.cellstart[i] = S.cellstart[0]; S.sorted[i] = S.sorted[0]; S.cellstart_f[i] = S.cellstart_f[0];
        S.sorted_f[i] = S.sorted_f[0]; S.out[i] = S.out[0]; S.kind[i] = S.kind[0];
    }
    for (int i = nsites; i <= DCF_MAX_KNN_SITES; ++i) S.first[i] = blocks;
#define KNN_MCASE(KK)                                                                                                                  \
    case KK:                                                                                                                           \
        DCF_LAUNCH_B("knn_search_sites", bytes, s, hipLaunchKernelGGL(k_knn_search_ms<KK>, dim3(blocks, B), dim3(256), 0, s, count_dev, n_max, S, rmax2)); \
        break;
    switch (K) {
        KNN_MCASE(1) KNN_MCASE(2) KNN_MCASE(3) KNN_MCASE(4) KNN_MCASE(5) KNN_MCASE(6) KNN_MCASE(7) KNN_MCASE(8)
    }
#undef KNN_MCASE
    return DCF_OK;
}

extern "C" size_t dcf_fusion_invert_workspace_bytes(int n_max, int nmaps)
{
    const size_t nscan = (size_t)nmaps * (n_max + 1);
    return sizeof(int) * (2 * nscan + (size_t)cdiv(nscan, CP_TILE) + 8);
}

extern "C" int dcf_fusion_invert(const dcf_knn_map *maps, int nmaps, int K, int n_max, int32_t *start, int32_t *ent_pix, int32_t *ent_pt,
                                 void *ws, dcf_stream_t stream)
{
    DCF_REQUIRE(maps && start && ent_pix && ent_pt && ws && K >= 1 && n_max >= 1, "dcf_fusion_invert: bad arguments");
    DCF_REQUIRE(nmaps >= 1 && nmaps <= DCF_MAX_KNN_MAPS, "dcf_fusion_invert: 1..%d maps per call", DCF_MAX_KNN_MAPS);
    InvMaps m;
    m.n = nmaps;
    int64_t tot = 0;
    for (int i = 0; i < DCF_MAX_KNN_MAPS; ++i) {
        m.idx[i] = nullptr; m.hw[i] = 1; m.w[i] = 1; m.first[i] = (int)tot;
        if (i < nmaps) {
            DCF_REQUIRE(maps[i].idx && maps[i].h >= 1 && maps[i].w >= 1 && maps[i].h < 65536 && maps[i].w < 65536,
                        "dcf_fusion_invert: map %d: null or pixel coordinates beyond 16 bits", i);
            m.idx[i] = maps[i].idx; m.hw[i] = maps[i].h * maps[i].w; m.w[i] = maps[i].w;
            tot += (int64_t)K * m.hw[i];
        }
    }
    m.first[DCF_MAX_KNN_MAPS] = (int)tot;
    for (int i = nmaps; i <= DCF_MAX_KNN_MAPS; ++i) m.first[i] = (int)tot;
    DCF_REQUIRE(tot < (1ll << 31), "dcf_fusion_invert: too many pairs");
    hipStream_t s = S(stream);
    const int total = (int)tot, nscan = nmaps * (n_max + 1), nsb = cdiv(nscan, CP_TILE);
    int *cnt = (int *)ws, *cursor = cnt + nscan, *blocksum = cursor + nscan, *totp = blocksum + nsb;
    DCF_HIP(hipMemsetAsync(cnt, 0, sizeof(int) * (size_t)nscan, s));
    DCF_LAUNCH_B("inv_hist", (double)total * 4.0, s, hipLaunchKernelGGL(k_inv_hist, dim3(cdiv(total, 256)), dim3(256), 0, s, m, n_max, cnt));
    DCF_LAUNCH("scan_blocksum", s, hipLaunchKernelGGL(k_scan_blocksum, dim3(nsb), dim3(CP_THREADS), 0, s, cnt, nscan, blocksum));
    DCF_LAUNCH("compact_scan", s, hipLaunchKernelGGL(k_compact_scan, dim3(1), dim3(CP_THREADS), 0, s, blocksum, nsb, totp));
    DCF_LAUNCH("scan_apply", s, hipLaunchKernelGGL(k_scan_apply, dim3(nsb), dim3(CP_THREADS), 0, s, cnt, nscan, blocksum, start, cursor));
    DCF_LAUNCH_B("inv_fill", (double)total * 12.0, s, hipLaunchKernelGGL(k_inv_fill, dim3(cdiv(total, 256)), dim3(256), 0, s, m, n_max, cursor, ent_pix, ent_pt));
    return DCF_OK;
}

#ifdef KNN_STAMP
extern "C" int dcf_knn_stamps_read(long long *dst, int *dims)
{
    dims[0] = KNN_STAMP_TILES; dims[1] = 16;
    DCF_HIP(hipMemcpyFromSymbol(dst, HIP_SYMBOL(g_knn_stamps), sizeof(long long) * KNN_STAMP_TILES * 16));
    return DCF_OK;
}
#endif
```

### deep_continuous_fusion_for_multi-sensor_3d_object_detection_amd/model.py

```python
import math
import os

import numpy as np
import torch
import torch.nn as nn

from . import _hip as H
from .engine import ParamTable, Plan, StackPlan


class AnchorBoundingBoxFeature(nn.Module):

    def __init__(self, config):
        super(AnchorBoundingBoxFeature, self).__init__()
        self.config = config
        a = config["anchor_bbox_feature"]
        self.f_height = int(config["voxel_length"] / a["reduced_scale"])
        self.f_width = int(config["voxel_width"] / a["reduced_scale"])
        self.width, self.length, self.height = a["width"], a["length"], a["height"]

    def forward(self):
        h, w, c = self.f_height, self.f_width, self.config
        xs = torch.linspace(c["lidar_x_min"], c["lidar_x_max"], h).view(h, 1).expand(h, w)
        ys = torch.linspace(c["lidar_y_min"], c["lidar_y_max"], w).view(1, w).expand(h, w)
# ... 262 lines not shown
                if len(shape) >= 2:
                    bound = 1.0 / math.sqrt(float(np.prod(shape[1:])))
                    p.uniform_(-bound, bound)
            for (key, shape, off, n, layout), p in zip(self._table.entries, self._param_list):
                leaf = key.split(".")[-1]
                if len(shape) == 1 and leaf == "weight":
                    p.fill_(1.0)
                elif len(shape) == 1 and "fusion" in key:
                    p.uniform_(-0.05, 0.05)
                if zero_init_last and "fusion" in key and ".fc2." in key:
                    p.zero_()
            for key, shape, off, n in self._buf_meta:
                self._bufflat[off:off + n].fill_(1.0 if key.endswith("running_var") else 0.0)

    def _apply(self, fn, recurse=True):
        new_flat = fn(self._flat)
        if new_flat.dtype != torch.float32:
            raise TypeError("master parameters stay fp32; choose the compute dtype with config['dtype']")
        if new_flat.device == self._flat.device:
            return self
        self._flat = new_flat.contiguous()
        self._gradflat = torch.zeros_like(self._flat)
        self._bufflat = fn(self._bufflat).contiguous()
        for p, (shape, off, n, layout) in zip(self._param_list, self._param_meta):
            p.data = ParamTable.view(self._flat, shape, off, n, layout)
            p.grad = None
        for key, shape, off, n in self._buf_meta:
            node, leaf = self._resolve(key)
            node._buffers[leaf] = self._bufflat[off:off + n].view(shape)
        self._nbtflat = fn(self._nbtflat).contiguous()
        for i, key in enumerate(self._nbt_keys):
            node, leaf = self._resolve(key)
            node._buffers[leaf] = self._nbtflat[i]
        self._on_moved()
        return self

    @property
    def _nbt(self):
        out = []
        for key in self._nbt_keys:
            node, leaf = self._resolve(key)
            out.append(node._buffers[leaf])
        return out

    def _bind_grads(self):
        for p, (shape, off, n, layout) in zip(self._param_list, self._param_meta):
            p.grad = ParamTable.view(self._gradflat, shape, off, n, layout)

    @property
    def flat_params(self):
        return self._flat

    @property
    def flat_grads(self):
        return self._gradflat


class ObjectDetection_DCF(_FlatParamModule):
    def __init__(self, config):
        super(ObjectDetection_DCF, self).__init__()
        self.config = config
        fu = dict(config.get("fusion") or {})
        self.fusion_enabled = bool(fu.get("enabled", False))
        self.K = int(fu.get("K", 3))
        self.r_max = fu.get("r_max", None)
        self.cf = int(fu.get("image_channels", 64))
        dt = config.get("dtype", "f32")
        self.fp8 = dt in ("fp8", "f8", "e4m3")
        self.dtype = H.dtype_code("bf16" if self.fp8 else dt)
        self.bn_mode = config.get("bn_mode", "eval")
        if self.bn_mode not in ("eval", "train", "module"):
            raise ValueError("bn_mode must be eval, train or module (got %r)" % (self.bn_mode,))
        stream = fu.get("image_stream", "resnet18")
        from .engine import IMAGE_ARCHS
        if self.fusion_enabled and stream not in IMAGE_ARCHS:
            raise NotImplementedError("image_stream=%r (one of %s)" % (stream, sorted(IMAGE_ARCHS)))
        self.deterministic = parse_deterministic_config(config)
        hg = config.get("hip_graphs", False)
        self.use_graphs = "auto" if str(hg).lower() == "auto" else bool(hg)
        self._graphs = None
        self._plan = Plan(config, with_image=self.fusion_enabled, cf=self.cf, image_arch=str(fu.get("image_stream", "resnet18")))
        self._backend = None
        if self.deterministic and self.fusion_enabled:
            bad = [f["cb"] for f in self._plan.fusion if f["cb"] not in DET_CHANNELS]
            if bad:
                raise ValueError("deterministic: true needs fusion sites of %s channels (got %s)" % (list(DET_CHANNELS), bad))
        self._build_parameters()
        self.reset_parameters(zero_init_last=bool(fu.get("zero_init_last", False)))
        from .ops import GridSpec
        self._grid = GridSpec(config)

    def _on_moved(self):
        self._backend = None
        self._graphs = None
        self._plan._anc_key = None

    def set_grid(self, voxel_length, voxel_width):
        L, W = int(voxel_length), int(voxel_width)
        if (L, W) == (self.config["voxel_length"], self.config["voxel_width"]):
            return
        if L % 16 or W % 16:
            raise ValueError("voxel_length and voxel_width must be multiples of 16 (FPN add, model.py:151)")
        cfg = dict(self.config, voxel_length=L, voxel_width=W)
        from .ops import GridSpec
        grid = GridSpec(cfg)
        self.config = cfg
        self._plan.cfg = cfg
        self._plan._anc_key = None
        self._grid = grid
        self._graphs = None

    def load_state_dict(self, state_dict, strict=True):
        sd = {(k[7:] if k.startswith("module.") else k): v for k, v in state_dict.items()}
        return super(ObjectDetection_DCF, self).load_state_dict(sd, strict=strict)

    def _ensure_backend(self, device):
        if self._backend is None or self._backend.dev != device:
            if device.type != "cuda":
                raise H.DcfError("ObjectDetection_DCF runs on the HIP device only: move the module with .cuda() "
                                 "(no CPU fallback exists for the hot path)")
            from .backend_hip import HipBackend
            self._backend = HipBackend(self._plan, self._flat, self._gradflat, self._bufflat, self.dtype,
                                       fp8_min_cin=int(self.config.get("fp8_min_cin", 128)) if self.fp8 else 0,
                                       fp8_min_blocks=int(self.config.get("fp8_min_blocks", 512)))
            self._backend.deterministic = self.deterministic
            if self.config.get("conv_chain") is not None:
                self._backend.chain_enabled = bool(self.config["conv_chain"])
        return self._backend

    KNN_SHARED_MAX_PIXELS = 20000
    knn_shared = True
    knn_merged = os.environ.get("DCF_KNN_MERGED", "1") != "0"

    def fusion_geometry(self, points, uv, n_valid, bufs=None):
        from . import ops
        B = points.shape[0]
        dev = points.device
        cnt = n_valid.to(device=dev, dtype=torch.int32).contiguous() if isinstance(n_valid, torch.Tensor) else \
            torch.tensor([int(v) for v in n_valid], dtype=torch.int32, device=dev)
        L, W = self.config["voxel_length"], self.config["voxel_width"]
        idx = []
        batched = points.is_contiguous() and cnt.is_contiguous()
        if batched and self.knn_shared and self.knn_merged:
            sites, first = [], None
            for si in range(1, 5):
                s = 2 ** si
                h, w = L // s, W // s
                out = bufs["idx"][si - 1] if bufs is not None else torch.empty((B, self.K, h, w), dtype=torch.int32, device=dev)
                ws = bufs["ws"][si - 1] if bufs is not None else torch.empty((B, ops.knn_ws_stride(points.shape[1], h, w)), dtype=torch.uint8, device=dev)
                fine = first if (first is not None and h * w <= self.KNN_SHARED_MAX_PIXELS) else -1
                if first is None:
                    first = si - 1
                sites.append((h, w, s, fine, ws, out))
            idx = ops.knn_bev_sites(points, cnt, self.K, sites, self._grid.aff, self.r_max)
            return dict(xyz=points.contiguous(), uv=uv.contiguous(), cnt=cnt, idx=idx, aff=self._grid.aff)
        fine = None
        for si in range(1, 5):
            s = 2 ** si
            h, w = L // s, W // s
            if bufs is not None:
                site = bufs["idx"][si - 1]
            else:
                site = torch.empty((B, self.K, h, w), dtype=torch.int32, device=dev)
            ws = None if bufs is None else bufs["ws"][si - 1]
            if batched and fine is not None and h * w <= self.KNN_SHARED_MAX_PIXELS and self.knn_shared:
                ops.knn_bev_batch_shared(points, cnt, self.K, h, w, s, fine[:3], fine[3], self._grid.aff, self.r_max, ws=ws, out=site)
            elif batched and (B > 1 or self.knn_shared):
                if ws is None:
                    ws = torch.empty((B, ops.knn_ws_stride(points.shape[1], h, w)), dtype=torch.uint8, device=dev)
                ops.knn_bev_batch(points, cnt, self.K, h, w, s, self._grid.aff, self.r_max, ws=ws, out=site)
                if fine is None:
                    fine = (h, w, s, ws)
            else:
                for b in range(B):
                    ops.knn_bev(points[b], cnt[b:b + 1], self.K, h, w, s, self._grid.aff, self.r_max, ws=None if ws is None else ws[0], out=site[b])
            idx.append(site)
        return dict(xyz=points.contiguous(), uv=uv.contiguous(), cnt=cnt, idx=idx, aff=self._grid.aff)

    def fusion_buffers(self, B, n_max, device):
        from . import ops
        L, W = self.config["voxel_length"], self.config["voxel_width"]
        idx, ws = [], []
        for si in range(1, 5):
            s = 2 ** si
            idx.append(torch.empty((B, self.K, L // s, W // s), dtype=torch.int32, device=device))
            ws.append(torch.empty((B, ops.knn_ws_stride(n_max, L // s, W // s)), dtype=torch.uint8, device=device))
        maps = [t[b] for t in idx for b in range(B)]
        ns, ne, nw = ops.fusion_invert_sizes(maps, n_max)
        inv = (torch.empty((ns,), dtype=torch.int32, device=device), torch.empty((2, ne), dtype=torch.int32, device=device),
               torch.empty((nw,), dtype=torch.uint8, device=device))
        out = dict(idx=idx, ws=ws, inv=inv)
        if self.deterministic:
            out["inv_scratch"] = torch.empty((ne,), dtype=torch.int32, device=device)
            Hf, Wf = self._cam_hw()
            out["cam"] = ops.cam_invert_buffers(B, n_max, Hf, Wf, device)
        return out

    def _cam_hw(self):
        Hi, Wi = int(self.config["image_height"]), int(self.config["image_width"])
        return ((Hi + 1) // 2 + 1) // 2, ((Wi + 1) // 2 + 1) // 2

    def fusion_inverse(self, geom, bufs=None):
        from . import ops
        from .engine import FUSION_INV
        if FUSION_INV == "0":
            return geom
        n_max = geom["xyz"].shape[1]
        maps = [t[b] for t in geom["idx"] for b in range(t.shape[0])]
        if self.deterministic:
            geom["inv"] = ops.fusion_invert_sorted(maps, n_max, out=None if bufs is None else bufs["inv"],
                                                   scratch=None if bufs is None else bufs["inv_scratch"])
            Hf, Wf = self._cam_hw()
            geom["cam_inv"] = ops.cam_invert(geom["uv"], geom["cnt"], n_max, Hf, Wf, out=None if bufs is None else bufs["cam"])
        else:
            geom["inv"] = ops.fusion_invert(maps, n_max, out=None if bufs is None else bufs["inv"])
        geom["inv_nmax"] = n_max
        return geom

    def forward(self, x_lidar, x_image, points=None, uv=None, n_valid=None, geom=None):
        K = self._ensure_backend(x_lidar.device)
        if not self.fusion_enabled:
            if geom is not None and geom.get("voxel_event") is not None:
                torch.cuda.current_stream().wait_event(geom["voxel_event"])
            geom = None
        elif geom is None and points is not None:
            geom = self.fusion_geometry(points, uv, n_valid)
            if torch.is_grad_enabled():
                self.fusion_inverse(geom)
        bn_train = self.bn_mode == "train" or (self.bn_mode == "module" and self.training)
        if K.set_bn_mode(bn_train):
            self._graphs = None
        if bn_train:
            self._nbtflat += 1
        need = torch.is_grad_enabled() and self._param_list[0].requires_grad
        if self.graphs_wanted(x_lidar.shape[0]) and need and not self._profiling():
            if self._graphs is None:
                self._graphs = _StepGraphs(self)
            if self._graphs.misses > self._graphs.MAX_MISSES and not self._graphs.disabled:
                import warnings
                warnings.warn("hip_graphs: more than %d input signatures captured -- falling back to eager launches" % self._graphs.MAX_MISSES)
                self._graphs.disabled = True
                self._graphs.sets.clear()
            if not self._graphs.disabled:
                return _RunGraphs.apply(self._param_list[0], self, x_lidar, x_image, geom)
        K.prepare()
        return _RunPlan.apply(self._param_list[0], self, x_lidar, x_image, geom, need)

    def graphs_wanted(self, batch):
        if self.use_graphs == "auto":
            import torch.distributed as dist
            multi = dist.is_available() and dist.is_initialized() and dist.get_world_size() > 1
            return batch == 1 and not multi
        return bool(self.use_graphs)

    graphs_off = False

    def _profiling(self):
        return self.graphs_off


class _RunStack(torch.autograd.Function):

    @staticmethod
    def forward(ctx, x, token, module, need):
        ctx.module, ctx.saved_graph = module, need
        outs = module._plan.forward(module._backend, x, save=need)
        module._fwd_serial = ctx.serial = getattr(module, "_fwd_serial", 0) + 1
        return tuple(outs)

    @staticmethod
    def backward(ctx, *gouts):
        m = ctx.module
        if not ctx.saved_graph:
            raise RuntimeError("backward through a forward that ran without saving activations")
        if ctx.serial != m._fwd_serial:
            raise RuntimeError("backward of a stale forward: this module keeps the activations of its LAST forward only "
                               "(call backward before the next forward; gradients are overwritten, not accumulated)")
        gx = m._plan.backward(m._backend, list(gouts))
        m._bind_grads()
        return gx, None, None, None


class _ResidualStack(_FlatParamModule):
    dtype = "f32"
    bn_mode = "module"

    def _setup(self, stages, taps, dtype=None, bn_mode=None):
        if dtype is not None:
            self.dtype = dtype
        if bn_mode is not None:
            self.bn_mode = bn_mode
        self._plan = StackPlan(stages, taps)
        self._backend = None
        self._build_parameters()
        self.reset_parameters()

    def _ensure_backend(self, device):
        if self._backend is None or self._backend.dev != device:
            if device.type != "cuda":
                raise H.DcfError("%s runs on the HIP device only: move the module with .cuda() (no CPU fallback exists "
                                 "for the hot path)" % type(self).__name__)
            from .backend_hip import HipBackend
            self._backend = HipBackend(self._plan, self._flat, self._gradflat, self._bufflat, H.dtype_code(self.dtype))
        return self._backend

    def _run(self, x):
        K = self._ensure_backend(x.device)
        bn_train = self.bn_mode == "train" or (self.bn_mode == "module" and self.training)
        K.set_bn_mode(bn_train)
        if bn_train:
            self._nbtflat += 1
        need = torch.is_grad_enabled() and (self._param_list[0].requires_grad or x.requires_grad)
        K.prepare()
        return _RunStack.apply(x.contiguous(), self._param_list[0], self, need)


class ResidualBlock(_ResidualStack):

    def __init__(self, in_channels, out_channels, dtype=None, bn_mode=None):
        super(ResidualBlock, self).__init__()
        self.in_channels, self.out_channels = in_channels, out_channels
        self._setup([[("", in_channels, out_channels)]], [0], dtype, bn_mode)

    @property
    def should_apply_shortcut(self):
        return self.in_channels != self.out_channels

    def forward(self, x):
        return self._run(x)[0]


class ResidualBlockModule(_ResidualStack):

    def __init__(self, first_in_channel, last_out_channel, num_resblock, dtype=None, bn_mode=None):
        super(ResidualBlockModule, self).__init__()
        blocks = [("sequential.resblock_%d." % i, first_in_channel if i == 0 else last_out_channel, last_out_channel)
                  for i in range(num_resblock)]
        self._setup([blocks], [0], dtype, bn_mode)

    def forward(self, x):
        return self._run(x)[0]


class ResnetCustomed(_ResidualStack):

    def __init__(self, out_feature=(32, 64, 128, 192, 256), num_res_block=(1, 2, 4, 6, 6), dtype=None, bn_mode=None):
        super(ResnetCustomed, self).__init__()
        stages = []
        for k in range(5):
            cin = out_feature[0] if k == 0 else out_feature[k - 1]
            stages.append([("layer%d.sequential.resblock_%d." % (k + 1, i), cin if i == 0 else out_feature[k], out_feature[k])
                           for i in range(num_res_block[k])])
        self._setup(stages, [4, 3, 2], dtype, bn_mode)

    def forward(self, x):
        x4, x3, x2 = self._run(x)
        return x4, x3, x2


class OffsettoBbox(nn.Module):

    def __init__(self, config):
        super(OffsettoBbox, self).__init__()
        self.anchor_bbox_feature = AnchorBoundingBoxFeature(config)

    def forward(self, x):
        from . import ops
        B, C, h, w = x.shape
# ... 34 lines not shown
```

### deep_continuous_fusion_for_multi-sensor_3d_object_detection_amd/ops.py

```python
import ctypes

import numpy as np
import torch

from . import _hip as H


def _chk(t, name):
    if not (isinstance(t, torch.Tensor) and t.is_cuda and t.is_contiguous()):
        raise H.DcfError("%s must be a contiguous CUDA tensor" % name)
    return t


def conv_out_size(n, k, s, p):
    return (n + 2 * p - k) // s + 1


def nchw_to_nhwc(x, dtype):
    B, C, Hh, W = x.shape
    _chk(x, "x")
    y = torch.empty((B, Hh, W, C), dtype=H.torch_dtype(dtype), device=x.device)
    H.call("dcf_nchw_to_nhwc", dtype, x, y, B, C, Hh, W, H.stream_ptr())
    return y

# ... 269 lines not shown
def adam_step_guarded(params, grads, m, v, beta1, beta2, eps, state):
    H.call("dcf_adam_step_guarded", params, grads, m, v, params.numel(), beta1, beta2, eps, state.raw, H.stream_ptr())


class GridSpec(object):

    def __init__(self, cfg):
        L, W, Cz = cfg["voxel_length"], cfg["voxel_width"], cfg["voxel_channel"]
        self.dims = (Cz, L, W)
        self.xs = int(L / (cfg["lidar_x_max"] - cfg["lidar_x_min"]))
        self.ys = int(W / (cfg["lidar_y_max"] - cfg["lidar_y_min"]))
        self.zs = int(Cz / (cfg["lidar_z_max"] - cfg["lidar_z_min"]))
        self.xo = int(-cfg["lidar_x_min"] * self.xs)
        self.yo = int(-cfg["lidar_y_min"] * self.ys)
        self.zo = int(-cfg["lidar_z_min"] * self.zs)
        d = cfg["delta"]
        self.lim = np.array([cfg["lidar_x_min"], cfg["lidar_x_max"] - d, cfg["lidar_y_min"], cfg["lidar_y_max"] - d,
                             cfg["lidar_z_min"], cfg["lidar_z_max"] - d], dtype=np.float64).astype(np.float32)
        self.aff = np.array([self.xs, self.xo, self.ys, self.yo, self.zs, self.zo], dtype=np.float32)
        self.image_height = cfg["image_height"]
        self.image_width = cfg["image_width"]


def range_filter(pts, lim):
    n = pts.shape[0]
    dev = pts.device
    out = torch.empty((max(n, 1), 3), dtype=torch.float32, device=dev)
    src = torch.empty((max(n, 1),), dtype=torch.int32, device=dev)
    cnt = torch.zeros((1,), dtype=torch.int32, device=dev)
    ws = torch.empty((H.lib().dcf_compact_workspace_bytes(n),), dtype=torch.uint8, device=dev)
    H.call("dcf_range_filter", _chk(pts, "pts"), n, H.host_f32(lim), out, src, cnt, ws, H.stream_ptr())
    return out, src, cnt


def voxelize(pts, lim, aff, dims, mode=H.VOXEL_COMPAT, owner_ws=None, out=None):
    Cz, L, W = dims
    dev = pts.device
    grid = torch.empty((Cz, L, W), dtype=torch.float32, device=dev) if out is None else _chk(out, "out")
    if mode in (H.VOXEL_COMPAT, H.VOXEL_COMPAT_ROUNDS) and owner_ws is None:
        owner_ws = torch.zeros((2, Cz * L * W), dtype=torch.int32, device=dev)
    H.call("dcf_voxelize", _chk(pts, "pts"), pts.shape[0], H.host_f32(lim), H.host_f32(aff), Cz, L, W, mode, grid, owner_ws,
           H.stream_ptr())
    return grid


def voxelize_batch(pts_list, lim, aff, dims, owner_ws, out):
    Cz, L, W = dims
    B = len(pts_list)
    ptrs = (ctypes.c_void_p * B)(*[_chk(p, "pts").data_ptr() for p in pts_list])
    ns = (ctypes.c_int * B)(*[p.shape[0] for p in pts_list])
    H.call("dcf_voxelize_batch", ctypes.addressof(ptrs), ctypes.addressof(ns), B, H.host_f32(lim), H.host_f32(aff), Cz, L, W, _chk(out, "out"),
           owner_ws, H.stream_ptr())
    return out


def voxelize_batch_nhwc(dtype, pts_list, lim, aff, dims, owner_ws, out):
    Cz, L, W = dims
    B = len(pts_list)
    ptrs = (ctypes.c_void_p * B)(*[_chk(p, "pts").data_ptr() for p in pts_list])
    ns = (ctypes.c_int * B)(*[p.shape[0] for p in pts_list])
    H.call("dcf_voxelize_batch_nhwc", dtype, ctypes.addressof(ptrs), ctypes.addressof(ns), B, H.host_f32(lim), H.host_f32(aff), Cz, L, W,
           _chk(out, "out"), owner_ws, H.stream_ptr())
    return out


def project_filter(pts, lim, crt, ulim, vlim, mode=H.PROJ_COMPAT, n_out=None, want_src=False, out=None):
    n = pts.shape[0]
    dev = pts.device
    n_out = n if n_out is None else n_out
    if n_out < n:
        raise H.DcfError("project_filter: output rows (%d) < input points (%d)" % (n_out, n))
    if out is not None:
        uv, xyz, cnt = out
        if uv.shape[0] < n or xyz.shape[0] < n or not (uv.is_contiguous() and xyz.is_contiguous()):
            raise H.DcfError("project_filter: out tensors must be contiguous with at least %d rows" % n)
    else:
        uv = torch.zeros((max(n_out, 1), 2), dtype=torch.float32, device=dev)
        xyz = torch.zeros((max(n_out, 1), 3), dtype=torch.float32, device=dev)
        cnt = torch.zeros((1,), dtype=torch.int32, device=dev)
    src = torch.empty((max(n, 1),), dtype=torch.int32, device=dev) if want_src else None
    ws = torch.empty((H.lib().dcf_compact_workspace_bytes(n),), dtype=torch.uint8, device=dev)
    H.call("dcf_project_filter", _chk(pts, "pts"), n, H.host_f32(lim), H.host_f32(crt).reshape(-1), float(ulim), float(vlim), mode,
           uv, xyz, src, cnt, ws, H.stream_ptr())
    return uv, xyz, cnt, src


def project_filter_batch(pts_list, lim, crts, ulim, vlim, mode, uv_all, xyz_all, cnt_all, ws=None):
    import ctypes
    B = len(pts_list)
    rows = xyz_all.shape[1]
    ns = [int(p.shape[0]) for p in pts_list]
    if max(ns) > rows or uv_all.shape[1] != rows or not (uv_all.is_contiguous() and xyz_all.is_contiguous() and cnt_all.is_contiguous()):
        raise H.DcfError("project_filter_batch: contiguous outputs with at least %d rows per frame" % max(ns))
    ptrs = (ctypes.c_void_p * B)(*[_chk(p, "pts").data_ptr() if p.shape[0] else None for p in pts_list])
    cnts = (ctypes.c_int32 * B)(*ns)
    crt = np.ascontiguousarray(np.asarray(crts, dtype=np.float32).reshape(B, 12))
    need = B * H.lib().dcf_compact_workspace_bytes(max(max(ns), 1))
    if ws is None or ws.numel() < need:
        ws = torch.empty((need,), dtype=torch.uint8, device=xyz_all.device)
    H.call("dcf_project_filter_batch", ctypes.addressof(ptrs), ctypes.addressof(cnts), B, H.host_f32(lim), crt, float(ulim), float(vlim), int(mode),
           uv_all, xyz_all, rows, cnt_all, ws, H.stream_ptr())
    return ws


def knn_bev(xyz, cnt, K, h, w, stride, aff, rmax=None, ws=None, out=None):
    n_max = xyz.shape[0]
    dev = xyz.device
    idx = torch.empty((K, h, w), dtype=torch.int32, device=dev) if out is None else _chk(out, "out")
    if ws is None:
        ws = torch.empty((H.lib().dcf_knn_workspace_bytes(n_max, h, w),), dtype=torch.uint8, device=dev)
    r2 = -1.0 if rmax is None else float(np.float32(rmax) * np.float32(rmax))
    H.call("dcf_knn_bev", _chk(xyz, "xyz"), cnt, n_max, K, h, w, stride, float(aff[0]), float(aff[1]), float(aff[2]), float(aff[3]),
           r2, idx, ws, H.stream_ptr())
    return idx


def knn_ws_stride(n_max, h, w):
    return (H.lib().dcf_knn_workspace_bytes(n_max, h, w) + 255) // 256 * 256


def knn_bev_batch(xyz, cnt, K, h, w, stride, aff, rmax=None, ws=None, out=None):
    B, n_max = xyz.shape[0], xyz.shape[1]
    dev = xyz.device
    st = knn_ws_stride(n_max, h, w)
    idx = torch.empty((B, K, h, w), dtype=torch.int32, device=dev) if out is None else _chk(out, "out")
    if ws is None:
        ws = torch.empty((B, st), dtype=torch.uint8, device=dev)
    if ws.shape[0] < B or ws.stride(0) != st:
        raise H.DcfError("knn_bev_batch: workspace must be [B, %d] bytes" % st)
    r2 = -1.0 if rmax is None else float(np.float32(rmax) * np.float32(rmax))
    H.call("dcf_knn_bev_batch", _chk(xyz, "xyz"), _chk(cnt, "cnt"), B, n_max, K, h, w, stride, float(aff[0]), float(aff[1]), float(aff[2]), float(aff[3]),
           r2, idx, ws, st, H.stream_ptr())
    return idx


def knn_bev_batch_shared(xyz, cnt, K, h, w, stride, fine, ws_fine, aff, rmax=None, ws=None, out=None):
    B, n_max = xyz.shape[0], xyz.shape[1]
    fh, fw, fs = fine
    stf = knn_ws_stride(n_max, fh, fw)
    if ws_fine.shape[0] < B or ws_fine.stride(0) != stf:
        raise H.DcfError("knn_bev_batch_shared: the fine site's workspace must be [B, %d] bytes" % stf)
    st = knn_ws_stride(n_max, h, w)
    if ws is None:
        ws = torch.empty((B, st), dtype=torch.uint8, device=xyz.device)
    if ws.shape[0] < B or ws.stride(0) != st:
        raise H.DcfError("knn_bev_batch_shared: workspace must be [B, %d] bytes" % st)
    idx = torch.empty((B, K, h, w), dtype=torch.int32, device=xyz.device) if out is None else _chk(out, "out")
    r2 = -1.0 if rmax is None else float(np.float32(rmax) * np.float32(rmax))
    H.call("dcf_knn_bev_batch_shared", _chk(xyz, "xyz"), _chk(cnt, "cnt"), B, n_max, K, h, w, stride, fh, fw, fs, float(aff[0]), float(aff[1]),
           float(aff[2]), float(aff[3]), r2, idx, ws, st, ws_fine, stf, H.stream_ptr())
    return idx


def knn_bev_sites(xyz, cnt, K, sites, aff, rmax=None):
    B, n_max = xyz.shape[0], xyz.shape[1]
    arr = (H.KnnSite * len(sites))()
    for i, (h, w, stride, fine, ws, out) in enumerate(sites):
        st = knn_ws_stride(n_max, h, w)
        if ws.shape[0] < B or ws.stride(0) != st or ws.dtype != torch.uint8:
            raise H.DcfError("knn_bev_sites: site %d: workspace must be uint8 [B, %d]" % (i, st))
        if tuple(out.shape) != (B, K, h, w) or out.dtype != torch.int32 or not out.is_contiguous():
            raise H.DcfError("knn_bev_sites: site %d: out must be a contiguous int32 [B, K, h, w]" % i)
        arr[i] = H.KnnSite(h, w, stride, fine, out.data_ptr(), ws.data_ptr(), st)
    r2 = -1.0 if rmax is None else float(np.float32(rmax) * np.float32(rmax))
    H.call("dcf_knn_bev_sites", _chk(xyz, "xyz"), _chk(cnt, "cnt"), B, n_max, K, ctypes.addressof(arr), len(sites), float(aff[0]), float(aff[1]),
           float(aff[2]), float(aff[3]), r2, H.stream_ptr())
    return [t[5] for t in sites]


def point_sample_fwd(dtype, fmap, uv, cnt, n_max, out=None):
    Hf, Wf, Cf = fmap.shape
    fp = (torch.empty if n_max > 0 else torch.zeros)((max(n_max, 1), Cf), dtype=fmap.dtype, device=fmap.device) if out is None else _chk(out, "out")
    H.call("dcf_point_sample_fwd", dtype, fmap, Hf, Wf, Cf, uv, cnt, n_max, fp, H.stream_ptr())
    return fp


def point_sample_bwd(dtype, gfp, uv, cnt, n_max, gfmap):
    Hf, Wf, Cf = gfmap.shape
    H.call("dcf_point_sample_bwd", dtype, gfp, Hf, Wf, Cf, uv, cnt, n_max, gfmap, H.stream_ptr())
    return gfmap


def point_sample_fwd_batch(dtype, fmap, uv, cnt, n_max, out):
    B, Hf, Wf, Cf = fmap.shape
    H.call("dcf_point_sample_fwd_batch", dtype, _chk(fmap, "fmap"), Hf, Wf, Cf, _chk(uv, "uv"), uv.stride(0), cnt, n_max, _chk(out, "out"), B, H.stream_ptr())
    return out


def point_sample_bwd_batch(dtype, gfp, uv, cnt, n_max, gfmap):
    B, Hf, Wf, Cf = gfmap.shape
    H.call("dcf_point_sample_bwd_batch", dtype, _chk(gfp, "gfp"), Hf, Wf, Cf, _chk(uv, "uv"), uv.stride(0), cnt, n_max, _chk(gfmap, "gfmap"), B, H.stream_ptr())
    return gfmap


def fusion_gather_fwd_batch(dtype, P, xyz, idx, stride, aff, w1d, b1, hsum, cnt):
    B, K, h, w = idx.shape
    Cb = P.shape[2]
    H.call("dcf_fusion_gather_fwd_batch", dtype, _chk(P, "P"), P.shape[1], _chk(xyz, "xyz"), xyz.stride(0), _chk(idx, "idx"), K, h, w, stride,
           float(aff[0]), float(aff[1]), float(aff[2]), float(aff[3]), w1d, b1, Cb, _chk(hsum, "hsum"), _chk(cnt, "cnt"), B, H.stream_ptr())
    return hsum, cnt


def fusion_gather_bwd_inv_batch(dtype, P, xyz, inv, n_max, g0, khw, stride, aff, w1d, b1, ghsum, gP, gw1d, gb1, ws=None):
    start, ent = inv
    B, rows, Cb = P.shape
    seg = start[g0 * (n_max + 1):]
    H.call("dcf_fusion_gather_bwd_inv_batch", dtype, _chk(P, "P"), rows, _chk(xyz, "xyz"), xyz.stride(0), seg, seg[n_max:], n_max + 1, ent[0], ent[1],
           khw[0] * khw[1] * khw[2], khw[1], khw[2], stride, float(aff[0]), float(aff[1]), float(aff[2]), float(aff[3]), w1d, b1, Cb,
           _chk(ghsum, "ghsum"), _chk(gP, "gP"), gw1d, gb1, ws, B, H.stream_ptr())


_DWS_BYTES = {}


def fusion_bwd_direct_workspace(device, max_entries, Cb, B):
    return torch.zeros((max(H.lib().dcf_fusion_gather_bwd_direct_workspace_bytes(max_entries, Cb, B) // 4, 1),), dtype=torch.float32, device=device)


def fusion_gather_bwd_direct_batch(dtype, P, xyz, inv, n_max, g0, khw, stride, aff, w1d, b1, ghsum, gP, gw1d, gb1, ws, dws):
    start, ent = inv
    B, rows, Cb = P.shape
    me = khw[0] * khw[1] * khw[2]
    if gP.dtype != P.dtype or gP.shape != P.shape:
        raise H.DcfError("fusion_gather_bwd_direct_batch: gP must look like P")
    need = _DWS_BYTES.get((me, Cb, B))
    if need is None:
        need = _DWS_BYTES[(me, Cb, B)] = H.lib().dcf_fusion_gather_bwd_direct_workspace_bytes(me, Cb, B)
    if dws.numel() * 4 < need:
        raise H.DcfError("fusion_gather_bwd_direct_batch: workspace too small")
    seg = start.data_ptr() + 4 * g0 * (n_max + 1)
    H.call("dcf_fusion_gather_bwd_direct_batch", dtype, _chk(P, "P"), rows, _chk(xyz, "xyz"), xyz.stride(0), seg, seg + 4 * n_max, n_max + 1,
           ent.data_ptr(), ent.data_ptr() + 4 * ent.stride(0), me, khw[1], khw[2], stride, float(aff[0]), float(aff[1]), float(aff[2]), float(aff[3]),
           w1d, b1, Cb, _chk(ghsum, "ghsum"), _chk(gP, "gP"), gw1d, gb1, ws, dws, B, H.stream_ptr())


def fusion_gather_fwd(dtype, P, xyz, idx, stride, aff, w1d, b1, out=None):
    K, h, w = idx.shape
    Cb = P.shape[1]
    if out is not None:
        hsum, cnt = _chk(out[0], "hsum"), _chk(out[1], "cnt")
    else:
        hsum = torch.empty((h, w, Cb), dtype=P.dtype, device=P.device)
        cnt = torch.empty((h * w,), dtype=torch.float32, device=P.device)
    H.call("dcf_fusion_gather_fwd", dtype, P, xyz, idx, K, h, w, stride, float(aff[0]), float(aff[1]), float(aff[2]), float(aff[3]),
           w1d, b1, Cb, hsum, cnt, H.stream_ptr())
    return hsum, cnt


def fusion_gather_bwd(dtype, P, xyz, idx, stride, aff, w1d, b1, ghsum, gP, gw1d, gb1):
    K, h, w = idx.shape
    Cb = P.shape[1]
    H.call("dcf_fusion_gather_bwd", dtype, P, xyz, idx, K, h, w, stride, float(aff[0]), float(aff[1]), float(aff[2]), float(aff[3]),
           w1d, b1, Cb, ghsum, gP, gw1d, gb1, H.stream_ptr())


def fusion_invert_sizes(maps, n_max):
    return len(maps) * (n_max + 1), sum(t.numel() for t in maps), H.lib().dcf_fusion_invert_workspace_bytes(n_max, len(maps))


def fusion_invert(maps, n_max, out=None):
    K = maps[0].shape[0]
    dev = maps[0].device
    tab = (H.KnnMap * len(maps))()
    total = 0
    for i, t in enumerate(maps):
        assert t.dtype == torch.int32 and t.is_contiguous() and t.shape[0] == K
        tab[i] = H.KnnMap(t.data_ptr(), t.shape[1], t.shape[2])
        total += t.numel()
    if out is not None:
        start, ent, ws = out
    else:
        start = torch.empty((len(maps) * (n_max + 1),), dtype=torch.int32, device=dev)
        ent = torch.empty((2, total), dtype=torch.int32, device=dev)
        ws = torch.empty((H.lib().dcf_fusion_invert_workspace_bytes(n_max, len(maps)),), dtype=torch.uint8, device=dev)
    H.call("dcf_fusion_invert", ctypes.addressof(tab), len(maps), K, n_max, start, ent[0], ent[1], ws, H.stream_ptr())
    return start, ent


def fusion_bwd_workspace(device, Cb=256):
    return torch.zeros((H.lib().dcf_fusion_gather_bwd_workspace_bytes(Cb) // 4,), dtype=torch.float32, device=device)


def fusion_gather_bwd_inv(dtype, P, xyz, inv, n_max, g, khw, stride, aff, w1d, b1, ghsum, gP, gw1d, gb1, ws=None):
    start, ent = inv
    Cb = P.shape[1]
    seg = start[g * (n_max + 1):]
    if ws is not None and ws.numel() * 4 < H.lib().dcf_fusion_gather_bwd_workspace_bytes(Cb):
        raise H.DcfError("fusion_gather_bwd_inv: workspace too small for %d channels" % Cb)
    H.call("dcf_fusion_gather_bwd_inv", dtype, P, xyz, seg, seg[n_max:], ent[0], ent[1], khw[0] * khw[1] * khw[2], khw[1], khw[2], stride,
           float(aff[0]), float(aff[1]), float(aff[2]), float(aff[3]), w1d, b1, Cb, ghsum, gP, gw1d, gb1, ws, H.stream_ptr())


def rowscale_bias_fwd(dtype, y, cnt, b2):
    C = y.shape[-1]
    H.call("dcf_rowscale_bias_fwd", dtype, y, cnt, b2, y.numel() // C, C, H.stream_ptr())
    return y


def rowscale_bias_bwd(dtype, gy, cnt, gb2):
    C = gy.shape[-1]
    H.call("dcf_rowscale_bias_bwd", dtype, gy, cnt, gb2, gy.numel() // C, C, H.stream_ptr())


def relu_mask_rowscale_bwd(dtype, gy, y, cnt, gb2):
    C = gy.shape[-1]
    gout = torch.empty_like(gy)
    H.call("dcf_relu_mask_rowscale_bwd", dtype, _chk(gy, "gy"), _chk(y, "y"), cnt, gout, gb2, gy.numel() // C, C, H.stream_ptr())
    return gout


def fusion_gather_bwd_pts(dtype, P, xyz, inv, n_max, g, khw, stride, aff, w1d, b1, ghsum, gP, gw1d, gb1):
    start, ent = inv
    Cb = P.shape[1]
    seg = start[g * (n_max + 1):]
    H.call("dcf_fusion_gather_bwd_pts", dtype, P, xyz, seg, P.shape[0], ent[0], ent[1], khw[0] * khw[1] * khw[2], khw[1], khw[2], stride,
           float(aff[0]), float(aff[1]), float(aff[2]), float(aff[3]), w1d, b1, Cb, ghsum, gP, gw1d, gb1, H.stream_ptr())


def inv_sort_segments(start, keys, scratch=None, nseg=None):
    if scratch is None:
        scratch = torch.empty_like(keys)
    if scratch.numel() < keys.numel() or scratch.dtype != torch.int32 or keys.dtype != torch.int32 or start.dtype != torch.int32:
        raise H.DcfError("inv_sort_segments: int32 tensors, scratch as long as keys")
    H.call("dcf_inv_sort_segments", _chk(start, "start"), start.numel() - 1 if nseg is None else int(nseg), _chk(keys, "keys"), scratch, H.stream_ptr())
    return keys


def fusion_invert_sorted(maps, n_max, out=None, scratch=None):
    start, ent = fusion_invert(maps, n_max, out=out)
    inv_sort_segments(start, ent[0], scratch)
    return start, ent


def cam_invert_buffers(B, n_max, Hf, Wf, device):
    i32 = dict(dtype=torch.int32, device=device)
    return (torch.empty((B * (Hf * Wf + 1),), **i32), torch.empty((max(B * 4 * n_max, 1),), **i32), torch.empty((max(B * 4 * n_max, 1),), **i32),
            torch.empty((H.lib().dcf_cam_invert_workspace_bytes(Hf, Wf, B),), dtype=torch.uint8, device=device))


def cam_invert(uv, cnt, n_max, Hf, Wf, out=None):
    B = uv.shape[0]
    start, ent, scratch, ws = out if out is not None else cam_invert_buffers(B, n_max, Hf, Wf, uv.device)
    if start.numel() < B * (Hf * Wf + 1) or ent.numel() < B * 4 * n_max or scratch.numel() < B * 4 * n_max:
        raise H.DcfError("cam_invert: buffers too small")
    H.call("dcf_cam_invert", _chk(uv, "uv"), uv.stride(0), _chk(cnt, "cnt"), n_max, Hf, Wf, B, start, ent, scratch, ws, H.stream_ptr())
    return start, ent, (Hf, Wf)


def point_sample_bwd_det(dtype, gfp, uv, cam_inv, gfmap):
    B, Hf, Wf, Cf = gfmap.shape
    start, ent, hw = cam_inv
    if tuple(hw) != (Hf, Wf) or gfmap.dtype != torch.float32:
        raise H.DcfError("point_sample_bwd_det: the camera-pixel map was built for a %s map, the gradient is %s" % (tuple(hw), (Hf, Wf)))
    H.call("dcf_point_sample_bwd_det", dtype, _chk(gfp, "gfp"), gfp.shape[1], Hf, Wf, Cf, _chk(uv, "uv"), uv.stride(0), start, ent, _chk(gfmap, "gfmap"), B,
           H.stream_ptr())
    return gfmap


def fusion_bwd_det_workspace(device, max_entries, Cb, B):
    return torch.empty((max(H.lib().dcf_fusion_gather_bwd_det_workspace_bytes(max_entries, Cb, B) // 4, 1),), dtype=torch.float32, device=device)


def fusion_gather_bwd_det(dtype, P, xyz, inv, n_max, g0, khw, stride, aff, w1d, b1, ghsum, gP, gw1d, gb1, ws):
    start, ent = inv
    B, rows, Cb = P.shape
    me = khw[0] * khw[1] * khw[2]
    if gP.dtype != P.dtype or gP.shape != P.shape:
        raise H.DcfError("fusion_gather_bwd_det: gP must look like P")
    if ws.numel() * 4 < H.lib().dcf_fusion_gather_bwd_det_workspace_bytes(me, Cb, B):
        raise H.DcfError("fusion_gather_bwd_det: workspace too small")
    seg = start.data_ptr() + 4 * g0 * (n_max + 1)
    H.call("dcf_fusion_gather_bwd_det", dtype, _chk(P, "P"), rows, _chk(xyz, "xyz"), xyz.stride(0), seg, n_max, ent.data_ptr(),
           ent.data_ptr() + 4 * ent.stride(0), me, khw[1], khw[2], stride, float(aff[0]), float(aff[1]), float(aff[2]), float(aff[3]),
           w1d, b1, Cb, _chk(ghsum, "ghsum"), _chk(gP, "gP"), gw1d, gb1, ws, B, H.stream_ptr())


def rowscale_bias_det_workspace(device, C):
    return torch.empty((H.lib().dcf_rowscale_bias_bwd_det_workspace_bytes(C) // 4,), dtype=torch.float32, device=device)


def rowscale_bias_bwd_det(dtype, gy, cnt, gb2, ws, y=None):
    C = gy.shape[-1]
    gout = None if y is None else torch.empty_like(gy)
    H.call("dcf_rowscale_bias_bwd_det", dtype, _chk(gy, "gy"), None if y is None else _chk(y, "y"), cnt, gout, gb2, gy.numel() // C, C, ws, H.stream_ptr())
    return gout


EVAL_NMS_CAP = 4096


def eval_score_filter(pred, threshold, cap=EVAL_NMS_CAP):
    B, C, h, w = pred.shape
    if C != 32 or pred.dtype != torch.float32:
        raise H.DcfError("eval_score_filter: pred must be the model output [B,32,h,w] fp32")
    pred = _chk(pred.contiguous(), "pred")
    boxes = torch.zeros((B, cap, 7), dtype=torch.float32, device=pred.device)
    count = torch.zeros((B,), dtype=torch.int32, device=pred.device)
    H.call("dcf_eval_score_filter", pred, B, h, w, float(threshold), cap, boxes, count, H.stream_ptr())
    return boxes, count


def eval_nms(boxes, mode, iou_threshold=0.01, count=None):
    n = boxes.shape[0]
    if n > EVAL_NMS_CAP:
        raise H.DcfError("eval_nms: at most %d boxes per call (got %d)" % (EVAL_NMS_CAP, n))
    boxes = _chk(boxes.float().contiguous(), "boxes")
    keep = torch.zeros((max(n, 1),), dtype=torch.int32, device=boxes.device)
    nkeep = torch.zeros((1,), dtype=torch.int32, device=boxes.device)
    ws = torch.empty((H.lib().dcf_eval_nms_workspace_bytes(max(n, 1)),), dtype=torch.uint8, device=boxes.device)
    H.call("dcf_eval_nms", boxes, count, n, {"sat": 0, "iou": 1, "bev": 2}[mode], float(iou_threshold), keep, nkeep, ws, H.stream_ptr())
    return keep[:n], nkeep


def eval_match(pred_boxes, ref_boxes, thresholds, tp):
    n = pred_boxes.shape[0]
    if n == 0:
        return tp
    H.call("dcf_eval_match", _chk(pred_boxes.float().contiguous(), "pred_boxes"), n, _chk(ref_boxes.float().contiguous(), "ref_boxes"),
           ref_boxes.shape[0], thresholds, thresholds.shape[0], tp, H.stream_ptr())
    return tp


def eval_rank_filter(pred, threshold, cap=EVAL_NMS_CAP):
    B, C, h, w = pred.shape
    if C != 32 or pred.dtype != torch.float32:
        raise H.DcfError("eval_rank_filter: pred must be the model output [B,32,h,w] fp32")
    if not 0 < cap <= EVAL_NMS_CAP:
        raise H.DcfError("eval_rank_filter: cap must be in 1..%d (got %d)" % (EVAL_NMS_CAP, cap))
    pred = _chk(pred.contiguous(), "pred")
    dev = pred.device
    boxes = torch.zeros((B, cap, 7), dtype=torch.float32, device=dev)
    scores = torch.zeros((B, cap), dtype=torch.float32, device=dev)
    count = torch.zeros((B,), dtype=torch.int32, device=dev)
    total = torch.zeros((B,), dtype=torch.int32, device=dev)
    ws = torch.empty((H.lib().dcf_eval_rank_workspace_bytes(B, h, w),), dtype=torch.uint8, device=dev)
    H.call("dcf_eval_rank_filter", pred, B, h, w, float(threshold), cap, boxes, scores, count, total, ws, H.stream_ptr())
    return boxes, scores, count, total


def eval_match_ranked(boxes, keep, count, ref_boxes, thresholds):
    n, R = boxes.shape[0], ref_boxes.shape[0]
    tpmask = torch.zeros((max(n, 1),), dtype=torch.int32, device=boxes.device)
    if n == 0:
        return tpmask[:0]
    ws = torch.empty((H.lib().dcf_eval_match_ranked_workspace_bytes(n, R),), dtype=torch.uint8, device=boxes.device)
    H.call("dcf_eval_match_ranked", _chk(boxes, "boxes"), _chk(keep, "keep"), count, n, _chk(ref_boxes, "ref_boxes") if R else None, R,
           thresholds, thresholds.shape[0], tpmask, ws, H.stream_ptr())
    return tpmask


def eval_accumulate(scores, tpmask, keep, count, total, ref_boxes, acc_scores, acc_tpmask, state):
    n, R = scores.shape[0], ref_boxes.shape[0]
    H.call("dcf_eval_accumulate", _chk(scores, "scores"), _chk(tpmask, "tpmask"), _chk(keep, "keep"), count, total, n,
           _chk(ref_boxes, "ref_boxes") if R else None, R, acc_scores, acc_tpmask, acc_scores.shape[0], state, H.stream_ptr())


def eval_ap(acc_scores, acc_tpmask, state, nthr):
    cap = acc_scores.shape[0]
    ap = torch.zeros((nthr,), dtype=torch.float64, device=acc_scores.device)
    tp = torch.zeros((nthr,), dtype=torch.int64, device=acc_scores.device)
    ws = torch.empty((H.lib().dcf_eval_ap_workspace_bytes(cap),), dtype=torch.uint8, device=acc_scores.device)
    H.call("dcf_eval_ap", _chk(acc_scores, "acc_scores"), _chk(acc_tpmask, "acc_tpmask"), _chk(state, "state"), cap, nthr, ap, tp, ws, H.stream_ptr())
    return ap, tp
```

### include/dcf_hip.h

```cpp
#ifndef DCF_HIP_H
#define DCF_HIP_H

#include <stddef.h>
#include <stdint.h>

#ifdef __cplusplus
extern "C" {
#endif

typedef void *dcf_stream_t;

enum { DCF_OK = 0, DCF_EINVAL = -1, DCF_ELAUNCH = -2, DCF_EUNSUPPORTED = -3 };
enum { DCF_F32 = 0, DCF_BF16 = 1, DCF_F16 = 2 };
enum { DCF_VOXEL_COMPAT = 0, DCF_VOXEL_ACCUM = 1, DCF_VOXEL_COMPAT_ROUNDS = 2,
       DCF_VOXEL_OCCUPANCY = 3  };
enum { DCF_PROJ_COMPAT = 0, DCF_PROJ_CORRECT = 1 };

const char *dcf_last_error(void);
int dcf_version(void);
int dcf_set_option(const char *name, const char *value);
int dcf_prof_enable(int on);
int dcf_prof_reset(void);
int dcf_prof_calibrate(dcf_stream_t stream, int n);
int dcf_prof_read(char *names , double *total_ms, int64_t *calls, double *work, int cap);
int dcf_prof_read2(char *names, double *total_ms, int64_t *calls, double *work, double *bytes, int cap);


size_t dcf_compact_workspace_bytes(int n);
int dcf_range_filter(const float *pts, int n, const float *lim, float *out_pts, int32_t *out_src,
                     int32_t *count_dev, void *ws, dcf_stream_t stream);

size_t dcf_voxelize_workspace_bytes(int Cz, int L, int W);
int dcf_voxelize(const float *pts, int n, const float *lim, const float *aff, int Cz, int L, int W,
                 int mode, float *grid, void *owner_ws, dcf_stream_t stream);
#define DCF_MAX_VOXEL_BATCH 8
int dcf_voxelize_batch(const float *const *pts, const int *n, int B, const float *lim, const float *aff, int Cz, int L, int W,
                       float *grids, void *owner_ws, dcf_stream_t stream);
int dcf_voxelize_batch_nhwc(int dtype, const float *const *pts, const int *n, int B, const float *lim, const float *aff, int Cz, int L,
                            int W, void *x_nhwc, void *owner_ws, dcf_stream_t stream);

int dcf_project_filter(const float *pts, int n, const float *lim, const float *crt, float ulim, float vlim,
                       int mode, float *uv_out, float *xyz_out, int32_t *src_out, int32_t *count_dev,
                       void *ws, dcf_stream_t stream);
int dcf_project_filter_batch(const float *const *pts, const int *n, int B, const float *lim, const float *crt, float ulim, float vlim,
                             int mode, float *uv_out, float *xyz_out, int rows, int32_t *count_dev, void *ws, dcf_stream_t stream);

size_t dcf_knn_workspace_bytes(int n_max, int h, int w);
int dcf_knn_bev(const float *xyz, const int32_t *count_dev, int n_max, int K, int h, int w, int stride,
                float xs, float xo, float ys, float yo, float rmax2, int32_t *idx_out, void *ws,
                dcf_stream_t stream);
int dcf_knn_bev_batch(const float *xyz, const int32_t *count_dev, int B, int n_max, int K, int h, int w, int stride,
                      float xs, float xo, float ys, float yo, float rmax2, int32_t *idx_out, void *ws, size_t ws_stride_bytes,
                      dcf_stream_t stream);

int dcf_knn_bev_batch_shared(const float *xyz, const int32_t *count_dev, int B, int n_max, int K, int h, int w, int stride,
                             int fine_h, int fine_w, int fine_stride, float xs, float xo, float ys, float yo, float rmax2,
                             int32_t *idx_out, void *ws, size_t ws_stride_bytes, const void *ws_fine, size_t ws_fine_stride_bytes,
                             dcf_stream_t stream);

typedef struct { int32_t h, w, stride, fine; int32_t *idx_out; void *ws; size_t ws_stride_bytes; } dcf_knn_site;
int dcf_knn_bev_sites(const float *xyz, const int32_t *count_dev, int B, int n_max, int K, const dcf_knn_site *sites, int nsites,
                      float xs, float xo, float ys, float yo, float rmax2, dcf_stream_t stream);

#define DCF_MAX_KNN_MAPS 32
typedef struct { const int32_t *idx; int32_t h, w; } dcf_knn_map;
size_t dcf_fusion_invert_workspace_bytes(int n_max, int nmaps);
int dcf_fusion_invert(const dcf_knn_map *maps, int nmaps, int K, int n_max, int32_t *start, int32_t *ent_pix, int32_t *ent_pt,
                      void *ws, dcf_stream_t stream);

int dcf_nchw_to_nhwc(int dtype, const float *x, void *y, int B, int C, int H, int W, dcf_stream_t stream);
int dcf_nhwc_to_nchw(int dtype, const void *x, float *y, int B, int C, int H, int W, dcf_stream_t stream);
int dcf_image_to_nhwc4(int dtype, const uint8_t *img, void *y, int B, int H, int W, dcf_stream_t stream);

int dcf_conv2d_fwd(int dtype, const void *x, const void *w, const float *shift, const void *res, void *y,
                   int B, int H, int W, int Cin, int Ho, int Wo, int Cout, int kh, int kw, int stride, int pad,
                   int relu, dcf_stream_t stream);
int dcf_conv2d_fwd_rowscale(int dtype, const void *x, const void *w, const float *shift, const float *rowscale, const void *res,
                            void *y, int B, int H, int W, int Cin, int Ho, int Wo, int Cout, int kh, int kw, int stride, int pad,
                            int relu, dcf_stream_t stream);
int dcf_conv2d_dgrad(int dtype, const void *gy, const void *wt, const void *res, const void *mask, void *gx,
                     int B, int H, int W, int Cin, int Ho, int Wo, int Cout, int kh, int kw, int stride, int pad,
                     dcf_stream_t stream);
int dcf_conv2d_dgrad_halfres(int dtype, const void *gy, const void *wt, const void *res, const void *resq,
                             const void *mask, void *gx, int B, int H, int W, int Cin, int Ho, int Wo, int Cout,
                             int kh, int kw, int stride, int pad, dcf_stream_t stream);
#define DCF_CHAIN_MAX_LAYERS 24
typedef struct {
    const void *x, *w;
    const float *shift;
    const void *res, *mask;
    void *y;
    int32_t relu, pad_;
} dcf_chain_layer;
int dcf_conv3x3_chain_supported(int dtype, int B, int H, int W, int C, int nlayers);
size_t dcf_conv3x3_chain_workspace_bytes(int dtype, int B, int H, int W, int C, int nlayers);
int dcf_conv3x3_chain(int dtype, const dcf_chain_layer *layers, int nlayers, int B, int H, int W, int C, int flip,
                      void *ws, dcf_stream_t stream);
int dcf_conv2d_wgrad_splits(int B, int Ho, int Wo, int Cin, int Cout, int kh, int kw, int stride);
int dcf_conv2d_wgrad(int dtype, const void *x, const void *gy, float *slabs, float *gsum, int nsplit,
                     int B, int H, int W, int Cin, int Ho, int Wo, int Cout, int kh, int kw, int stride, int pad,
                     dcf_stream_t stream);
typedef struct {
    int32_t dtype, nsplit;
    const void *x, *gy;
    float *slabs, *gsum;
    int32_t B, H, W, Cin, Cout, kh, kw, stride, pad, pad_;
} dcf_wgrad_item;
int dcf_conv2d_wgrad_groupable(int dtype, int B, int H, int W, int Cin, int Cout, int kh, int kw, int stride, int pad);
int dcf_conv2d_wgrad_group(const dcf_wgrad_item *items, int n, dcf_stream_t stream);
int dcf_stem7x7_fwd(int dtype, const void *img4, const void *w, const float *shift, void *y,
                    int B, int H, int W, int Ho, int Wo, int Cout, int relu, dcf_stream_t stream);
int dcf_stem7x7_wgrad(int dtype, const void *img4, const void *gy, float *slabs, float *gsum, int nsplit,
                      int B, int H, int W, int Ho, int Wo, int Cout, dcf_stream_t stream);

typedef struct dcf_conv_param {
    int64_t w_off;
    int64_t gamma_off;
    int64_t beta_off;
    int64_t mean_off;
    int64_t var_off;
    int64_t wfwd_off;
    int64_t wdgrad_off;
    int64_t shift_off;
    int64_t slab_off;
    int64_t gsum_off;
    int32_t cout, cin, taps, cout_pad;
    int32_t nsplit, flags, pad0, pad1;
} dcf_conv_param;
int dcf_weight_prep(int dtype, const dcf_conv_param *table, int nconv, const float *params, const float *buffers,
                    void *warena, float *ssarena, float eps, dcf_stream_t stream);
int dcf_wgrad_finalize(const dcf_conv_param *table, int nconv, int max_cout, const float *params, const float *buffers,
                       const float *ssarena, const float *slabs, const float *gsum, float *grads, float eps,
                       dcf_stream_t stream);
int dcf_wgrad_finalize_rows(const dcf_conv_param *table, int nconv, const int32_t *cout_host, const float *params, const float *buffers,
                            const float *ssarena, const float *slabs, const float *gsum, float *grads, float eps,
                            dcf_stream_t stream);

int dcf_fp8_act_scale(float amax, float *scale);
int dcf_cast_fp8(int dtype, const void *x, void *x8, const float *amax_prev, float *amax_cur, int64_t n, dcf_stream_t stream);
#define DCF_F8_AMAX_STRIDE 80
typedef struct dcf_f8_param {
    int64_t w8_off;
    int64_t wscale_off;
} dcf_f8_param;
int dcf_weight_prep_fp8(const dcf_conv_param *table, const dcf_f8_param *f8table, int nconv, int max_cout_pad, const float *params,
                        const float *buffers, void *w8arena, float *wsarena, float *amax, float eps, dcf_stream_t stream);
int dcf_conv2d_fwd_fp8(int out_dtype, const void *x8, const void *w8, const float *wscale, const float *xamax, const float *shift,
                       const void *res, void *y, void *y8, const float *y8amax, float *y8cur, int B, int H, int W, int Cin,
                       int Ho, int Wo, int Cout, int kh, int kw, int stride, int pad, int relu, dcf_stream_t stream);

int dcf_relu_bwd_chansum(int dtype, void *gy, const void *y, float *gsum, int64_t npix, int C, int relu,
                         dcf_stream_t stream);
int dcf_resize_bilinear_fwd(int dtype, const void *x, const void *add, void *y, int B, int Hi, int Wi, int Ho, int Wo,
                            int C, int align_corners, dcf_stream_t stream);
int dcf_resize_bilinear_bwd(int dtype, const void *gy, void *gx, int B, int Hi, int Wi, int Ho, int Wo, int C,
                            int align_corners, dcf_stream_t stream);
int dcf_maxpool3x3s2_fwd(int dtype, const void *x, void *y, int B, int H, int W, int Ho, int Wo, int C,
                         dcf_stream_t stream);
int dcf_maxpool3x3s2_bwd(int dtype, const void *x, const void *y, const void *gy, void *gx, int B, int H, int W,
                         int Ho, int Wo, int C, dcf_stream_t stream);
int dcf_maxpool3x3s2_fwd_idx(int dtype, const void *x, void *y, uint32_t *idx, int B, int H, int W, int Ho, int Wo, int C,
                             dcf_stream_t stream);
int dcf_maxpool3x3s2_bwd_idx(int dtype, const uint32_t *idx, const void *gy, void *gx, int B, int H, int W, int Ho, int Wo, int C,
                             dcf_stream_t stream);
int dcf_head_fwd(int dtype, const void *head, int Cp, const float *anchors, float *pred, int B, int h, int w,
                 dcf_stream_t stream);
int dcf_head_bwd(int dtype, const void *head, int Cp, const float *anchors, const float *pred, const float *gpred,
                 void *ghead, int B, int h, int w, dcf_stream_t stream);

size_t dcf_bn_workspace_bytes(int C);
int dcf_bn_train_fwd(int dtype, const void *x, const float *gamma, const float *beta, const void *res, void *y,
                     float *mean, float *invstd, float *running_mean, float *running_var, int64_t npix, int C,
                     float eps, float momentum, int relu, void *ws, dcf_stream_t stream);
int dcf_bn_train_bwd(int dtype, const void *g, const void *x, const float *mean, const float *invstd, const float *gamma,
                     float *dgamma, float *dbeta, void *dx, int64_t npix, int C, void *ws, dcf_stream_t stream);

int dcf_point_sample_fwd(int dtype, const void *fmap, int Hf, int Wf, int Cf, const float *uv, const int32_t *count_dev,
                         int n_max, void *fp, dcf_stream_t stream);
int dcf_point_sample_bwd(int dtype, const void *gfp, int Hf, int Wf, int Cf, const float *uv, const int32_t *count_dev,
                         int n_max, float *gfmap, dcf_stream_t stream);
int dcf_point_sample_fwd_batch(int dtype, const void *fmap, int Hf, int Wf, int Cf, const float *uv, int64_t uv_fstride,
                               const int32_t *count_dev, int n_max, void *fp, int B, dcf_stream_t stream);
int dcf_point_sample_bwd_batch(int dtype, const void *gfp, int Hf, int Wf, int Cf, const float *uv, int64_t uv_fstride,
                               const int32_t *count_dev, int n_max, float *gfmap, int B, dcf_stream_t stream);
int dcf_fusion_gather_fwd(int dtype, const void *P, const float *xyz, const int32_t *idx, int K, int h, int w,
                          int stride, float xs, float xo, float ys, float yo, const float *w1d, const float *b1,
                          int Cb, void *hsum, float *cnt, dcf_stream_t stream);
int dcf_fusion_gather_fwd_batch(int dtype, const void *P, int64_t p_rows, const float *xyz, int64_t xyz_fstride, const int32_t *idx,
                                int K, int h, int w, int stride, float xs, float xo, float ys, float yo, const float *w1d,
                                const float *b1, int Cb, void *hsum, float *cnt, int B, dcf_stream_t stream);
int dcf_fusion_gather_bwd(int dtype, const void *P, const float *xyz, const int32_t *idx, int K, int h, int w,
                          int stride, float xs, float xo, float ys, float yo, const float *w1d, const float *b1,
                          int Cb, const void *ghsum, float *gP, float *gw1d, float *gb1, dcf_stream_t stream);
int dcf_rowscale_bias_fwd(int dtype, void *y, const float *cnt, const float *b2, int64_t npix, int C, dcf_stream_t stream);
int dcf_rowscale_bias_bwd(int dtype, const void *gy, const float *cnt, float *gb2, int64_t npix, int C, dcf_stream_t stream);
int dcf_relu_mask_rowscale_bwd(int dtype, const void *gy, const void *y, const float *cnt, void *gout, float *gb2, int64_t npix, int C,
                               dcf_stream_t stream);
int dcf_cast(int dtype_src, const void *src, int dtype_dst, void *dst, int64_t n, dcf_stream_t stream);

int dcf_adam_step(float *params, const float *grads, float *m, float *v, int64_t n, float lr, float beta1,
                  float beta2, float eps, int step, float gscale, dcf_stream_t stream);

#define DCF_AMP_PARTS 1024
typedef struct dcf_amp_state {
    float scale_in, scale_next;
    int32_t growth_tracker, found_inf;
    int64_t applied_steps, skipped_steps;
    float grad_norm, clip_coef;
    float gscale, lr_over_bc1, inv_sqrt_bc2;
    int32_t pad_[3];
    float part_sum[DCF_AMP_PARTS];
    int32_t part_flag[DCF_AMP_PARTS];
} dcf_amp_state;
int dcf_grad_stats(const float *grads, int64_t n, dcf_amp_state *state, dcf_stream_t stream);
int dcf_amp_update(dcf_amp_state *state, float gscale_host, int dynamic, double growth_factor, double backoff_factor,
                   int growth_interval, float max_norm, float lr, float beta1, float beta2, dcf_stream_t stream);
int dcf_adam_step_guarded(float *params, const float *grads, float *m, float *v, int64_t n, float beta1, float beta2, float eps,
                          const dcf_amp_state *state, dcf_stream_t stream);

size_t dcf_fusion_gather_bwd_workspace_bytes(int Cb);
int dcf_fusion_gather_bwd_inv(int dtype, const void *P, const float *xyz, const int32_t *e_begin, const int32_t *e_end,
// ... 97 lines not shown
```

Before: 365.4 frames/s.

## Fuse inverse-map histogram into KNN search and stage candidate points in LDS

The KNN sites search now atomically accumulates per-point reference counts into the fusion-invert workspace, so the later invert pass can skip its memset and histogram kernel. It also adds an LDS staging path: when a tile's candidate set fits in 256 points, points are copied to shared memory and each pixel scans only its own 5x5 cell window using prefix-summed cell counts. This trades an extra standalone kernel and redundant distance tests for atomics in the search kernel, a larger shared-memory footprint, and more complex control flow.

```diff
diff --git a/deep_continuous_fusion_for_multi-sensor_3d_object_detection_amd/_hip.py b/deep_continuous_fusion_for_multi-sensor_3d_object_detection_amd/_hip.py
--- a/deep_continuous_fusion_for_multi-sensor_3d_object_detection_amd/_hip.py
+++ b/deep_continuous_fusion_for_multi-sensor_3d_object_detection_amd/_hip.py
@@ -37,6 +37,7 @@
     "dcf_knn_bev": (c_int, [P, P, c_int, c_int, c_int, c_int, c_int, c_float, c_float, c_float, c_float, c_float, P, P, P]),
     "dcf_knn_bev_batch": (c_int, [P, P, c_int, c_int, c_int, c_int, c_int, c_int, c_float, c_float, c_float, c_float, c_float, P, P, c_size_t, P]),
     "dcf_knn_bev_sites": (c_int, [P, P, c_int, c_int, c_int, P, c_int, c_float, c_float, c_float, c_float, c_float, P]),
+    "dcf_knn_bev_sites_counted": (c_int, [P, P, c_int, c_int, c_int, P, c_int, c_float, c_float, c_float, c_float, c_float, P, P]),
     "dcf_knn_bev_batch_shared": (c_int, [P, P, c_int, c_int, c_int, c_int, c_int, c_int, c_int, c_int, c_int, c_float, c_float, c_float, c_float, c_float, P, P, c_size_t, P, c_size_t, P]),
     "dcf_nchw_to_nhwc": (c_int, [c_int, P, P, c_int, c_int, c_int, c_int, P]),
     "dcf_nhwc_to_nchw": (c_int, [c_int, P, P, c_int, c_int, c_int, c_int, P]),
@@ -94,6 +95,7 @@
     "dcf_fusion_gather_bwd": (c_int, [c_int, P, P, P, c_int, c_int, c_int, c_int, c_float, c_float, c_float, c_float, P, P, c_int, P, P, P, P, P]),
     "dcf_fusion_invert_workspace_bytes": (c_size_t, [c_int, c_int]),
     "dcf_fusion_invert": (c_int, [P, c_int, c_int, c_int, P, P, P, P, P]),
+    "dcf_fusion_invert_counted": (c_int, [P, c_int, c_int, c_int, P, P, P, P, c_int, P]),
     "dcf_fusion_gather_bwd_pts": (c_int, [c_int, P, P, P, c_int, P, P, c_int, c_int, c_int, c_int, c_float, c_float, c_float, c_float, P, P, c_int, P, P, P, P, P]),
     "dcf_fusion_gather_bwd_workspace_bytes": (c_size_t, [c_int]),
     "dcf_fusion_gather_bwd_direct_workspace_bytes": (c_size_t, [c_int, c_int, c_int]),
diff --git a/deep_continuous_fusion_for_multi-sensor_3d_object_detection_amd/csrc/geometry.hip b/deep_continuous_fusion_for_multi-sensor_3d_object_detection_amd/csrc/geometry.hip
--- a/deep_continuous_fusion_for_multi-sensor_3d_object_detection_amd/csrc/geometry.hip
+++ b/deep_continuous_fusion_for_multi-sensor_3d_object_detection_amd/csrc/geometry.hip
@@ -484,10 +484,15 @@
     int nscan[DCF_MAX_KNN_SITES], nsb[DCF_MAX_KNN_SITES];
     int pkey_off[DCF_MAX_KNN_SITES], sorted_off[DCF_MAX_KNN_SITES];
     int n, B;
+    int *inv_cnt; int inv_n;
 };
 
 __global__ void __launch_bounds__(256) k_knn_zero_ms(KnnSortSites S)
 {
+    if (S.inv_cnt) {
+        const int nt = gridDim.x * gridDim.y * blockDim.x;
+        for (int i = (blockIdx.y * gridDim.x + blockIdx.x) * blockDim.x + threadIdx.x; i < S.inv_n; i += nt) S.inv_cnt[i] = 0;
+    }
     const int site = blockIdx.y / S.B, frame = blockIdx.y - site * S.B;
     int *p = S.ws[site] + (size_t)frame * S.g[site].fs_ws;
     const int n = S.nscan[site], n4 = n >> 2;
@@ -640,6 +645,19 @@
     }
 };
 
+struct InvRun { int head, len; };
+__device__ __forceinline__ InvRun inv_run(int key, int lane)
+{
+    const int prev = __shfl_up(key, 1, 64);
+    const unsigned long long heads = __ballot(lane == 0 || key != prev);
+    const unsigned long long below = heads & ((2ull << lane) - 1ull);
+    InvRun r;
+    r.head = 63 - __clzll(below);
+    const unsigned long long above = lane == 63 ? 0ull : (heads >> (lane + 1));
+    r.len = (above ? lane + 1 + (__ffsll((long long)above) - 1) : 64) - r.head;
+    return r;
+}
+
 #ifdef KNN_STAMP
 #define KNN_STAMP_TILES 4096
 __device__ long long g_knn_stamps[KNN_STAMP_TILES][16];
@@ -653,9 +671,27 @@
 #endif
 
 constexpr int KNN_MERGE_POINTS = 256;
-template <int K, int NW>
+constexpr int KNN_STAGE_POINTS = 256;
+struct KnnStage {
+    float x[KNN_STAGE_POINTS], y[KNN_STAGE_POINTS];
+    int id[KNN_STAGE_POINTS];
+    int cell[148];
+};
+union KnnWaveLds {
+    KnnStage stage;
+    unsigned long long keys[8][64];
+};
+template <int WPB>
+__device__ __forceinline__ KnnWaveLds *knn_wave_lds()
+{
+    __shared__ KnnWaveLds s_wave[WPB];
+    return s_wave;
+}
+
+template <int K, int NW, int WPB>
 __device__ __forceinline__ void knn_search_tile(const int *count, int n_max, const KnnGrid &g, const int *cellstart,
-                                                const float4 *sorted, float rmax2, int *out, const int tile, const int wv)
+                                                const float4 *sorted, float rmax2, int *out, const int tile, const int wv,
+                                                const int own, int *inv_cnt = nullptr)
 {
     count += blockIdx.y * g.fs_cnt; cellstart += (size_t)blockIdx.y * g.fs_ws; out += (size_t)blockIdx.y * g.fs_out;
     sorted = reinterpret_cast<const float4 *>(reinterpret_cast<const int *>(sorted) + (size_t)blockIdx.y * g.fs_ws);
@@ -663,7 +699,7 @@
     const int TI = tile / g.w8, TJ = tile - TI * g.w8;
     const int i = TI * 8 + (lane >> 3), j = TJ * 8 + (lane & 7);
     const bool inside = (i < g.h) && (j < g.w);
-    __shared__ unsigned long long s_keys[NW][K][64];
+    KnnWaveLds *const s_wave = knn_wave_lds<WPB>();
     const float s = (float)g.stride;
     const float X = __fdiv_rn(__fsub_rn(__fmul_rn((float)i + 0.5f, s), g.xo), g.xs);
     const float Y = __fdiv_rn(__fsub_rn(__fmul_rn((float)j + 0.5f, s), g.yo), g.ys);
@@ -699,12 +735,12 @@
     auto merge = [&]() {
         if constexpr (NW > 1) {
 #pragma unroll
-            for (int q = 0; q < K; ++q) s_keys[wv][q][lane] = TopK<K>::key(top.d[q], top.id[q]);
+            for (int q = 0; q < K; ++q) s_wave[wv].keys[q][lane] = TopK<K>::key(top.d[q], top.id[q]);
             __syncthreads();
 #pragma unroll
             for (int o = 1; o < NW; ++o) {
 #pragma unroll
-                for (int q = 0; q < K; ++q) top.insert_unique(s_keys[(wv + o) % NW][q][lane]);
+                for (int q = 0; q < K; ++q) top.insert_unique(s_wave[(wv + o) % NW].keys[q][lane]);
             }
             __syncthreads();
         }
@@ -732,6 +768,18 @@
                 ps = cellstart[cell_key(ci, c0, g)];
                 pe = cellstart[cell_key(ci, c1, g) + 1];
             }
+            int cc[3] = {0, 0, 0};
+            if (own && lane < 48) {
+                const int wi = TI * 8 - 2 + (lane >> 2);
+#pragma unroll
+                for (int k = 0; k < 3; ++k) {
+                    const int wj = TJ * 8 - 2 + (lane & 3) * 3 + k;
+                    if (wi >= 0 && wi <= H8 - 1 && wj >= 0 && wj <= W8 - 1) {
+                        const int key = cell_key(wi, wj, g);
+                        cc[k] = cellstart[key + 1] - cellstart[key];
+                    }
+                }
+            }
             const int len = pe - ps;
             int inc = len;
 #ifdef KNN_STAMP
@@ -746,6 +794,20 @@
             const int total = __builtin_amdgcn_readlane(inc, 63);
             const int exc = inc - len;
             KNN_ST(2, (long long)total);
+            const bool stage = own && total <= KNN_STAGE_POINTS;
+            KnnStage &sg = s_wave[__builtin_amdgcn_readfirstlane(threadIdx.x >> 6)].stage;
+            if (stage && total > 0) {
+                const int c3 = cc[0] + cc[1] + cc[2];
+                int cinc = c3;
+#pragma unroll
+                for (int o = 1; o < 64; o <<= 1) {
+                    const int v = __shfl_up(cinc, o, 64);
+                    if (lane >= o) cinc += v;
+                }
+                const int cex = cinc - c3;
+                if (lane < 48) { sg.cell[3 * lane] = cex; sg.cell[3 * lane + 1] = cex + cc[0]; sg.cell[3 * lane + 2] = cex + cc[0] + cc[1]; }
+                else if (lane == 48) sg.cell[144] = cex;
+            }
             for (int base = 0; base < total; base += 64) {
                 const int t = base + lane;
                 int lo = 0, hi = 63;
@@ -766,7 +828,42 @@
                     KNN_T(11);
                 }
 #endif
-                offer(mine, n, !done);
+                if (!stage) offer(mine, n, !done);
+                else if (lane < n) { sg.x[t] = mine.x; sg.y[t] = mine.y; sg.id[t] = __float_as_int(mine.z); }
+            }
+            if (stage && total > 0) {
+                __builtin_amdgcn_fence(__ATOMIC_RELEASE, "wavefront");
+                __builtin_amdgcn_wave_barrier();
+                __builtin_amdgcn_fence(__ATOMIC_ACQUIRE, "wavefront");
+                const int pi = lane >> 3, pj = lane & 7;
+                int off[5], end[5], cnt = 0;
+#pragma unroll
+                for (int r = 0; r < 5; ++r) {
+                    const int a = sg.cell[(pi + r) * 12 + pj], b = sg.cell[(pi + r) * 12 + pj + 5];
+                    off[r] = a - cnt;
+                    cnt += b - a;
+                    end[r] = cnt;
+                }
+                if (done) cnt = 0;
+                int maxc = cnt;
+#pragma unroll
+                for (int o = 32; o >= 1; o >>= 1) maxc = max(maxc, __shfl_xor(maxc, o, 64));
+                maxc = __builtin_amdgcn_readfirstlane(maxc);
+                KNN_ST(7, (long long)maxc);
+                for (int t0 = wv; t0 < maxc; t0 += 4 * NW) {
+#pragma unroll
+                    for (int v = 0; v < 4; ++v) {
+                        const int t = t0 + NW * v;
+                        const int o = t < end[0] ? off[0] : (t < end[1] ? off[1] : (t < end[2] ? off[2] : (t < end[3] ? off[3] : off[4])));
+                        const int a = min(t + o, KNN_STAGE_POINTS - 1);
+                        const float qx = sg.x[a], qy = sg.y[a];
+                        const int qi = sg.id[a];
+                        const float lim = t < cnt ? d2lim : -1.0f;
+                        const float dx = __fsub_rn(qx, X), dy = __fsub_rn(qy, Y);
+                        const float d2 = __fadd_rn(__fmul_rn(dx, dx), __fmul_rn(dy, dy));
+                        top.insert(d2 <= lim ? d2 : __int_as_float(0x7f800000), qi);
+                    }
+                }
             }
         }
         merge();
@@ -836,13 +933,21 @@
 #pragma unroll
         for (int q = 0; q < K; ++q) out[q * hw + pix] = top.id[q] != 0x7fffffff ? top.id[q] : -1;
     }
+    if (inv_cnt && wv == 0) {
+#pragma unroll
+        for (int q = 0; q < K; ++q) {
+            const int key = (inside && top.id[q] >= 0 && top.id[q] < n_max) ? top.id[q] : -1;
+            const InvRun r = inv_run(key, lane);
+            if (key >= 0 && r.head == lane) atomicAdd(&inv_cnt[key], r.len);
+        }
+    }
 }
 
 template <int K, int NW>
 __global__ void __launch_bounds__(64 * NW) k_knn_search(const int *count, int n_max, KnnGrid g, const int *cellstart,
-                                                       const float4 *sorted, float rmax2, int *out)
-{
-    knn_search_tile<K, NW>(count, n_max, g, cellstart, sorted, rmax2, out, blockIdx.x, __builtin_amdgcn_readfirstlane(threadIdx.x >> 6));
+                                                       const float4 *sorted, float rmax2, int *out, int own)
+{
+    knn_search_tile<K, NW, NW>(count, n_max, g, cellstart, sorted, rmax2, out, blockIdx.x, __builtin_amdgcn_readfirstlane(threadIdx.x >> 6), own);
 }
 
 template <int K>
@@ -872,7 +977,7 @@
 
 template <int K>
 __device__ __forceinline__ void knn_search_wave(const int *count, int n_max, const KnnGrid &g, const int *cellstart,
-                                                const float4 *sorted, float rmax2, int *out, const int bx)
+                                                const float4 *sorted, float rmax2, int *out, const int bx, int *inv_cnt = nullptr)
 {
     count += blockIdx.y * g.fs_cnt; cellstart += (size_t)blockIdx.y * g.fs_ws; out += (size_t)blockIdx.y * g.fs_out;
     sorted = reinterpret_cast<const float4 *>(reinterpret_cast<const int *>(sorted) + (size_t)blockIdx.y * g.fs_ws);
@@ -982,6 +1087,11 @@
     if (lane == 0) {
 #pragma unroll
         for (int q = 0; q < K; ++q) out[q * hw + pix] = (q < gcnt) ? gi[q] : -1;
+        if (inv_cnt) {
+#pragma unroll
+            for (int q = 0; q < K; ++q)
+                if (q < gcnt && gi[q] >= 0 && gi[q] < n_max) atomicAdd(&inv_cnt[gi[q]], 1);
+        }
     }
 }
 
@@ -1008,7 +1118,7 @@
 template <int K>
 __device__ __forceinline__ void knn_search_fine(const int *count, int n_max, const KnnGrid &g, const KnnGrid &gf, const int *cellstart_c,
                                                 const float4 *sorted_c, const int *cellstart, const float4 *sorted, float rmax2,
-                                                int *out, int dense_min, const int bx)
+                                                int *out, int dense_min, const int bx, int *inv_cnt = nullptr)
 {
     count += blockIdx.y * g.fs_cnt; out += (size_t)blockIdx.y * g.fs_out;
     cellstart_c += (size_t)blockIdx.y * g.fs_ws;
@@ -1151,6 +1261,11 @@
     if (lane == 0) {
 #pragma unroll
         for (int q = 0; q < K; ++q) out[q * hw + pix] = (q < gcnt) ? gi[q] : -1;
+        if (inv_cnt) {
+#pragma unroll
+            for (int q = 0; q < K; ++q)
+                if (q < gcnt && gi[q] >= 0 && gi[q] < n_max) atomicAdd(&inv_cnt[gi[q]], 1);
+        }
     }
 }
 
@@ -1170,6 +1285,9 @@
     int kind[DCF_MAX_KNN_SITES];
     int first[DCF_MAX_KNN_SITES + 1];
     int n, dense_min;
+    int *inv_cnt;
+    int B;
+    int own;
 };
 
 template <int K>
@@ -1182,16 +1300,17 @@
     const int wave = __builtin_amdgcn_readfirstlane(threadIdx.x >> 6);
     const KnnGrid &g = S.g[i];
     const int kind = S.kind[i];
+    int *const inv = S.inv_cnt ? S.inv_cnt + (size_t)(i * S.B + (int)blockIdx.y) * (n_max + 1) : nullptr;
     if (kind == 0) {
         const int tile = lb * 4 + wave;
         if (tile >= g.h8 * g.w8) return;
-        knn_search_tile<K, 1>(count, n_max, g, S.cellstart[i], S.sorted[i], rmax2, S.out[i], tile, 0);
+        knn_search_tile<K, 1, 4>(count, n_max, g, S.cellstart[i], S.sorted[i], rmax2, S.out[i], tile, 0, S.own, inv);
     } else if (kind == 1) {
-        knn_search_tile<K, 4>(count, n_max, g, S.cellstart[i], S.sorted[i], rmax2, S.out[i], lb, wave);
+        knn_search_tile<K, 4, 4>(count, n_max, g, S.cellstart[i], S.sorted[i], rmax2, S.out[i], lb, wave, S.own, inv);
     } else if (kind == 2) {
-        knn_search_wave<K>(count, n_max, g, S.cellstart[i], S.sorted[i], rmax2, S.out[i], lb);
+        knn_search_wave<K>(count, n_max, g, S.cellstart[i], S.sorted[i], rmax2, S.out[i], lb, inv);
     } else {
-        knn_search_fine<K>(count, n_max, g, S.gf[i], S.cellstart[i], S.sorted[i], S.cellstart_f[i], S.sorted_f[i], rmax2, S.out[i], S.dense_min, lb);
+        knn_search_fine<K>(count, n_max, g, S.gf[i], S.cellstart[i], S.sorted[i], S.cellstart_f[i], S.sorted_f[i], rmax2, S.out[i], S.dense_min, lb, inv);
     }
 }
 
@@ -1208,19 +1327,6 @@
 #pragma unroll
     for (int i = 1; i < DCF_MAX_KNN_MAPS; ++i) g += (i < m.n && e >= m.first[i]);
     return g;
-}
-
-struct InvRun { int head, len; };
-__device__ __forceinline__ InvRun inv_run(int key, int lane)
-{
-    const int prev = __shfl_up(key, 1, 64);
-    const unsigned long long heads = __ballot(lane == 0 || key != prev);
-    const unsigned long long below = heads & ((2ull << lane) - 1ull);
-    InvRun r;
-    r.head = 63 - __clzll(below);
-    const unsigned long long above = lane == 63 ? 0ull : (heads >> (lane + 1));
-    r.len = (above ? lane + 1 + (__ffsll((long long)above) - 1) : 64) - r.head;
-    return r;
 }
 
 __global__ void __launch_bounds__(256) k_zero_rows(int *p, int n, int64_t stride)
@@ -1458,6 +1564,12 @@
     int tile_waves, dense_min;
 };
 
+static int knn_window_own()
+{
+    static DcfOpt win_o("KNN_WINDOW"); const char *win = win_o.str();
+    return !(win && win[0] == 't');
+}
+
 static KnnSearchPlan knn_search_plan(const KnnGrid &g, int B, int n_max, int K, const int *cellstart, const float4 *sorted, const KnnFine *fine, bool merged)
 {
     KnnSearchPlan pl;
@@ -1534,6 +1646,7 @@
     const KnnSearchPlan pl = knn_search_plan(g, B, n_max, K, cellstart, sorted, fine, defer != nullptr);
     if (defer) { *defer = pl; return DCF_OK; }
     const int nbp = g.h8 * g.w8;
+    const int own = knn_window_own();
     const int nbw = cdiv(h * w, 4);
     if (pl.kind == 3) {
 #define KNN_FCASE(KK)                                                                                                                       \
@@ -1555,13 +1668,13 @@
                                                                 cellstart, sorted, rmax2, idx_out));                     \
         else if (pl.tile_waves == 4)                                                                                     \
             DCF_LAUNCH_B("knn_search", fB * ((double)h * w * K * 4.0 + (double)n_max * 16.0), s, hipLaunchKernelGGL((k_knn_search<KK, 4>), dim3(nbp, B), dim3(256), 0, s, count_dev, n_max, g, \
-                                                           cellstart, sorted, rmax2, idx_out));                          \
+                                                           cellstart, sorted, rmax2, idx_out, own));                     \
         else if (pl.tile_waves == 2)                                                                                     \
             DCF_LAUNCH_B("knn_search", fB * ((double)h * w * K * 4.0 + (double)n_max * 16.0), s, hipLaunchKernelGGL((k_knn_search<KK, 2>), dim3(nbp, B), dim3(128), 0, s, count_dev, n_max, g, \
-                                                           cellstart, sorted, rmax2, idx_out));                          \
+                                                           cellstart, sorted, rmax2, idx_out, own));                     \
         else                                                                                                             \
             DCF_LAUNCH_B("knn_search", fB * ((double)h * w * K * 4.0 + (double)n_max * 16.0), s, hipLaunchKernelGGL((k_knn_search<KK, 1>), dim3(nbp, B), dim3(64), 0, s, count_dev, n_max, g, \
-                                                           cellstart, sorted, rmax2, idx_out));                          \
+                                                           cellstart, sorted, rmax2, idx_out, own));                     \
         break;
     switch (K) {
         KNN_CASE(1) KNN_CASE(2) KNN_CASE(3) KNN_CASE(4) KNN_CASE(5) KNN_CASE(6) KNN_CASE(7) KNN_CASE(8)
@@ -1599,15 +1712,20 @@
     return knn_bev_impl(who, xyz, count_dev, B, n_max, K, h, w, stride, xs, xo, ys, yo, rmax2, idx_out, ws, ws_stride_bytes, S(stream), &fine);
 }
 
-extern "C" int dcf_knn_bev_sites(const float *xyz, const int32_t *count_dev, int B, int n_max, int K, const dcf_knn_site *sites, int nsites,
-                                 float xs, float xo, float ys, float yo, float rmax2, dcf_stream_t stream)
-{
-    const char *who = "dcf_knn_bev_sites";
+static bool knn_count_inv()
+{
+    static DcfOpt ci_o("KNN_COUNT_INV"); const char *ci = ci_o.str();
+    return !(ci && ci[0] == '0');
+}
+
+static int knn_bev_sites_impl(const char *who, const float *xyz, const int32_t *count_dev, int B, int n_max, int K, const dcf_knn_site *sites, int nsites,
+                              float xs, float xo, float ys, float yo, float rmax2, int32_t *inv_cnt, dcf_stream_t stream)
+{
     DCF_REQUIRE(xyz && count_dev && sites && nsites >= 1 && nsites <= DCF_MAX_KNN_SITES, "%s: 1..%d sites", who, DCF_MAX_KNN_SITES);
     DCF_REQUIRE(K >= 1 && K <= 8 && n_max >= 0 && B >= 1 && B * nsites <= 65535, "%s: bad dims", who);
     hipStream_t s = S(stream);
     KnnSortSites ss;
-    ss.n = nsites; ss.B = B;
+    ss.n = nsites; ss.B = B; ss.inv_cnt = inv_cnt; ss.inv_n = nsites * B * (n_max + 1);
     int max_nsb = 1, max_nscan = 1;
     for (int i = 0; i < DCF_MAX_KNN_SITES; ++i) {
         const dcf_knn_site &t = sites[i < nsites ? i : 0];
@@ -1639,9 +1757,9 @@
     if (n_max > 0)
         DCF_LAUNCH_B("knn_fill", (double)gy * n_max * (12.0 + 4.0 + 16.0), s, hipLaunchKernelGGL(k_knn_fill_ms, dim3(cdiv(n_max, 256), gy), dim3(256), 0, s, xyz, count_dev, n_max, ss));
     static DcfOpt ms_o("KNN_MERGED_SEARCH"); const char *ms = ms_o.str();
-    const bool merged = !(ms && ms[0] == '0');
+    const bool merged = inv_cnt || !(ms && ms[0] == '0');
     KnnSearchSites S;
-    S.n = nsites; S.dense_min = KNN_FINE_MIN_POINTS;
+    S.n = nsites; S.dense_min = KNN_FINE_MIN_POINTS; S.own = knn_window_own(); S.inv_cnt = inv_cnt; S.B = B;
     int blocks = 0;
     double bytes = 0.0;
     for (int i = 0; i < nsites; ++i) {
@@ -1682,14 +1800,28 @@
     return DCF_OK;
 }
 
+extern "C" int dcf_knn_bev_sites(const float *xyz, const int32_t *count_dev, int B, int n_max, int K, const dcf_knn_site *sites, int nsites,
+                                 float xs, float xo, float ys, float yo, float rmax2, dcf_stream_t stream)
+{
+    return knn_bev_sites_impl("dcf_knn_bev_sites", xyz, count_dev, B, n_max, K, sites, nsites, xs, xo, ys, yo, rmax2, nullptr, stream);
+}
+
+extern "C" int dcf_knn_bev_sites_counted(const float *xyz, const int32_t *count_dev, int B, int n_max, int K, const dcf_knn_site *sites, int nsites,
+                                         float xs, float xo, float ys, float yo, float rmax2, int32_t *inv_cnt, dcf_stream_t stream)
+{
+    DCF_REQUIRE(!inv_cnt || (int64_t)nsites * B * ((int64_t)n_max + 1) < (1ll << 31), "dcf_knn_bev_sites_counted: too many counts");
+    return knn_bev_sites_impl("dcf_knn_bev_sites_counted", xyz, count_dev, B, n_max, K, sites, nsites, xs, xo, ys, yo, rmax2,
+                              knn_count_inv() ? inv_cnt : nullptr, stream);
+}
+
 extern "C" size_t dcf_fusion_invert_workspace_bytes(int n_max, int nmaps)
 {
     const size_t nscan = (size_t)nmaps * (n_max + 1);
     return sizeof(int) * (2 * nscan + (size_t)cdiv(nscan, CP_TILE) + 8);
 }
 
-extern "C" int dcf_fusion_invert(const dcf_knn_map *maps, int nmaps, int K, int n_max, int32_t *start, int32_t *ent_pix, int32_t *ent_pt,
-                                 void *ws, dcf_stream_t stream)
+static int fusion_invert_impl(const dcf_knn_map *maps, int nmaps, int K, int n_max, int32_t *start, int32_t *ent_pix, int32_t *ent_pt,
+                              void *ws, bool counts_ready, dcf_stream_t stream)
 {
     DCF_REQUIRE(maps && start && ent_pix && ent_pt && ws && K >= 1 && n_max >= 1, "dcf_fusion_invert: bad arguments");
     DCF_REQUIRE(nmaps >= 1 && nmaps <= DCF_MAX_KNN_MAPS, "dcf_fusion_invert: 1..%d maps per call", DCF_MAX_KNN_MAPS);
@@ -1711,8 +1843,10 @@
     hipStream_t s = S(stream);
     const int total = (int)tot, nscan = nmaps * (n_max + 1), nsb = cdiv(nscan, CP_TILE);
     int *cnt = (int *)ws, *cursor = cnt + nscan, *blocksum = cursor + nscan, *totp = blocksum + nsb;
-    DCF_HIP(hipMemsetAsync(cnt, 0, sizeof(int) * (size_t)nscan, s));
-    DCF_LAUNCH_B("inv_hist", (double)total * 4.0, s, hipLaunchKernelGGL(k_inv_hist, dim3(cdiv(total, 256)), dim3(256), 0, s, m, n_max, cnt));
+    if (!counts_ready) {
+        DCF_HIP(hipMemsetAsync(cnt, 0, sizeof(int) * (size_t)nscan, s));
+        DCF_LAUNCH_B("inv_hist", (double)total * 4.0, s, hipLaunchKernelGGL(k_inv_hist, dim3(cdiv(total, 256)), dim3(256), 0, s, m, n_max, cnt));
+    }
     DCF_LAUNCH("scan_blocksum", s, hipLaunchKernelGGL(k_scan_blocksum, dim3(nsb), dim3(CP_THREADS), 0, s, cnt, nscan, blocksum));
     DCF_LAUNCH("compact_scan", s, hipLaunchKernelGGL(k_compact_scan, dim3(1), dim3(CP_THREADS), 0, s, blocksum, nsb, totp));
     DCF_LAUNCH("scan_apply", s, hipLaunchKernelGGL(k_scan_apply, dim3(nsb), dim3(CP_THREADS), 0, s, cnt, nscan, blocksum, start, cursor));
@@ -1720,6 +1854,18 @@
     return DCF_OK;
 }
 
+extern "C" int dcf_fusion_invert(const dcf_knn_map *maps, int nmaps, int K, int n_max, int32_t *start, int32_t *ent_pix, int32_t *ent_pt,
+                                 void *ws, dcf_stream_t stream)
+{
+    return fusion_invert_impl(maps, nmaps, K, n_max, start, ent_pix, ent_pt, ws, false, stream);
+}
+
+extern "C" int dcf_fusion_invert_counted(const dcf_knn_map *maps, int nmaps, int K, int n_max, int32_t *start, int32_t *ent_pix, int32_t *ent_pt,
+                                         void *ws, int counts_ready, dcf_stream_t stream)
+{
+    return fusion_invert_impl(maps, nmaps, K, n_max, start, ent_pix, ent_pt, ws, counts_ready != 0 && knn_count_inv(), stream);
+}
+
 #ifdef KNN_STAMP
 extern "C" int dcf_knn_stamps_read(long long *dst, int *dims)
 {
diff --git a/deep_continuous_fusion_for_multi-sensor_3d_object_detection_amd/model.py b/deep_continuous_fusion_for_multi-sensor_3d_object_detection_amd/model.py
--- a/deep_continuous_fusion_for_multi-sensor_3d_object_detection_amd/model.py
+++ b/deep_continuous_fusion_for_multi-sensor_3d_object_detection_amd/model.py
@@ -438,8 +438,14 @@
                 if first is None:
                     first = si - 1
                 sites.append((h, w, s, fine, ws, out))
-            idx = ops.knn_bev_sites(points, cnt, self.K, sites, self._grid.aff, self.r_max)
-            return dict(xyz=points.contiguous(), uv=uv.contiguous(), cnt=cnt, idx=idx, aff=self._grid.aff)
+            from .engine import FUSION_INV
+            inv = bufs.get("inv") if (bufs is not None and FUSION_INV != "0") else None
+            counted = inv is not None and inv[0].numel() == len(sites) * B * (points.shape[1] + 1)
+            idx = ops.knn_bev_sites(points, cnt, self.K, sites, self._grid.aff, self.r_max, inv_ws=inv[2] if counted else None)
+            geom = dict(xyz=points.contiguous(), uv=uv.contiguous(), cnt=cnt, idx=idx, aff=self._grid.aff)
+            if counted:
+                geom["inv_counted"] = inv[2]
+            return geom
         fine = None
         for si in range(1, 5):
             s = 2 ** si
@@ -493,13 +499,14 @@
             return geom
         n_max = geom["xyz"].shape[1]
         maps = [t[b] for t in geom["idx"] for b in range(t.shape[0])]
+        ready = bufs is not None and geom.get("inv_counted") is bufs["inv"][2]
         if self.deterministic:
             geom["inv"] = ops.fusion_invert_sorted(maps, n_max, out=None if bufs is None else bufs["inv"],
-                                                   scratch=None if bufs is None else bufs["inv_scratch"])
+                                                   scratch=None if bufs is None else bufs["inv_scratch"], counts_ready=ready)
             Hf, Wf = self._cam_hw()
             geom["cam_inv"] = ops.cam_invert(geom["uv"], geom["cnt"], n_max, Hf, Wf, out=None if bufs is None else bufs["cam"])
         else:
-            geom["inv"] = ops.fusion_invert(maps, n_max, out=None if bufs is None else bufs["inv"])
+            geom["inv"] = ops.fusion_invert(maps, n_max, out=None if bufs is None else bufs["inv"], counts_ready=ready)
         geom["inv_nmax"] = n_max
         return geom
 
diff --git a/deep_continuous_fusion_for_multi-sensor_3d_object_detection_amd/ops.py b/deep_continuous_fusion_for_multi-sensor_3d_object_detection_amd/ops.py
--- a/deep_continuous_fusion_for_multi-sensor_3d_object_detection_amd/ops.py
+++ b/deep_continuous_fusion_for_multi-sensor_3d_object_detection_amd/ops.py
@@ -445,7 +445,7 @@
     return idx
 
 
-def knn_bev_sites(xyz, cnt, K, sites, aff, rmax=None):
+def knn_bev_sites(xyz, cnt, K, sites, aff, rmax=None, inv_ws=None):
     B, n_max = xyz.shape[0], xyz.shape[1]
     arr = (H.KnnSite * len(sites))()
     for i, (h, w, stride, fine, ws, out) in enumerate(sites):
@@ -456,6 +456,12 @@
             raise H.DcfError("knn_bev_sites: site %d: out must be a contiguous int32 [B, K, h, w]" % i)
         arr[i] = H.KnnSite(h, w, stride, fine, out.data_ptr(), ws.data_ptr(), st)
     r2 = -1.0 if rmax is None else float(np.float32(rmax) * np.float32(rmax))
+    if inv_ws is not None:
+        if inv_ws.dtype != torch.uint8 or inv_ws.numel() < H.lib().dcf_fusion_invert_workspace_bytes(n_max, len(sites) * B):
+            raise H.DcfError("knn_bev_sites: inv_ws must be the uint8 workspace of fusion_invert_sizes() for sites x B maps")
+        H.call("dcf_knn_bev_sites_counted", _chk(xyz, "xyz"), _chk(cnt, "cnt"), B, n_max, K, ctypes.addressof(arr), len(sites), float(aff[0]),
+               float(aff[1]), float(aff[2]), float(aff[3]), r2, inv_ws, H.stream_ptr())
+        return [t[5] for t in sites]
     H.call("dcf_knn_bev_sites", _chk(xyz, "xyz"), _chk(cnt, "cnt"), B, n_max, K, ctypes.addressof(arr), len(sites), float(aff[0]), float(aff[1]),
            float(aff[2]), float(aff[3]), r2, H.stream_ptr())
     return [t[5] for t in sites]
@@ -551,7 +557,7 @@
     return len(maps) * (n_max + 1), sum(t.numel() for t in maps), H.lib().dcf_fusion_invert_workspace_bytes(n_max, len(maps))
 
 
-def fusion_invert(maps, n_max, out=None):
+def fusion_invert(maps, n_max, out=None, counts_ready=False):
     K = maps[0].shape[0]
     dev = maps[0].device
     tab = (H.KnnMap * len(maps))()
@@ -566,6 +572,11 @@
         start = torch.empty((len(maps) * (n_max + 1),), dtype=torch.int32, device=dev)
         ent = torch.empty((2, total), dtype=torch.int32, device=dev)
         ws = torch.empty((H.lib().dcf_fusion_invert_workspace_bytes(n_max, len(maps)),), dtype=torch.uint8, device=dev)
+    if counts_ready:
+        if out is None:
+            raise H.DcfError("fusion_invert: counts_ready needs the workspace the counts were written to (out)")
+        H.call("dcf_fusion_invert_counted", ctypes.addressof(tab), len(maps), K, n_max, start, ent[0], ent[1], ws, 1, H.stream_ptr())
+        return start, ent
     H.call("dcf_fusion_invert", ctypes.addressof(tab), len(maps), K, n_max, start, ent[0], ent[1], ws, H.stream_ptr())
     return start, ent
 
@@ -619,8 +630,8 @@
     return keys
 
 
-def fusion_invert_sorted(maps, n_max, out=None, scratch=None):
-    start, ent = fusion_invert(maps, n_max, out=out)
+def fusion_invert_sorted(maps, n_max, out=None, scratch=None, counts_ready=False):
+    start, ent = fusion_invert(maps, n_max, out=out, counts_ready=counts_ready)
     inv_sort_segments(start, ent[0], scratch)
     return start, ent
 
diff --git a/include/dcf_hip.h b/include/dcf_hip.h
--- a/include/dcf_hip.h
+++ b/include/dcf_hip.h
@@ -61,12 +61,16 @@
 typedef struct { int32_t h, w, stride, fine; int32_t *idx_out; void *ws; size_t ws_stride_bytes; } dcf_knn_site;
 int dcf_knn_bev_sites(const float *xyz, const int32_t *count_dev, int B, int n_max, int K, const dcf_knn_site *sites, int nsites,
                       float xs, float xo, float ys, float yo, float rmax2, dcf_stream_t stream);
+int dcf_knn_bev_sites_counted(const float *xyz, const int32_t *count_dev, int B, int n_max, int K, const dcf_knn_site *sites, int nsites,
+                              float xs, float xo, float ys, float yo, float rmax2, int32_t *inv_cnt, dcf_stream_t stream);
 
 #define DCF_MAX_KNN_MAPS 32
 typedef struct { const int32_t *idx; int32_t h, w; } dcf_knn_map;
 size_t dcf_fusion_invert_workspace_bytes(int n_max, int nmaps);
 int dcf_fusion_invert(const dcf_knn_map *maps, int nmaps, int K, int n_max, int32_t *start, int32_t *ent_pix, int32_t *ent_pt,
                       void *ws, dcf_stream_t stream);
+int dcf_fusion_invert_counted(const dcf_knn_map *maps, int nmaps, int K, int n_max, int32_t *start, int32_t *ent_pix, int32_t *ent_pt,
+                              void *ws, int counts_ready, dcf_stream_t stream);
 
 int dcf_nchw_to_nhwc(int dtype, const float *x, void *y, int B, int C, int H, int W, dcf_stream_t stream);
 int dcf_nhwc_to_nchw(int dtype, const void *x, float *y, int B, int C, int H, int W, dcf_stream_t stream);
```

New measurement: 339.1 frames/s. 7.2% lower.
